# antonbaumann/MIMO-Unet

Hardware: AMD Instinct MI355X
Metric: train images/sec at 256x256, S=2, fbc=30 (higher is better)
Workload: dtype f32 (split into 16-bit hi/lo pairs on the MFMA; weight gradient: activation as one fp16 value); 1 GPU; cfg3: SEN12TP-shape synthetic 2->1 ch, 256x256, S=2, fbc=30, laplace_nll, batch 32 global; global_batch=32, per_gpu_batch=32, scaling=strong, labels=U[0,1) (SURVEY 8d); same batch every step, parallelism=dp1, world_size=1, weak_per_gpu_batch=32, strong_global_batch=32, optimizer=adam(lr=1e-3) fused, inputs=resident in HBM

## Files before the change

mimo_unet_amd/csrc/common.h:

```cpp
#pragma once
#include <hip/hip_runtime.h>
#include <stdint.h>

#include "../../include/mimo_hip.h"
#include "tile_sched.h"

namespace mimo {

void set_error(const char* fmt, ...);

#define MIMO_HIP_CHECK(expr)                                                                          \
  do {                                                                                                \
    hipError_t e_ = (expr);                                                                           \
    if (e_ != hipSuccess) {                                                                           \
      ::mimo::set_error("%s failed: %s (%s:%d)", #expr, hipGetErrorString(e_), __FILE__, __LINE__);   \
      return MIMO_ERR_HIP;                                                                            \
    }                                                                                                 \
  } while (0)
#define MIMO_KERNEL_CHECK() MIMO_HIP_CHECK(hipGetLastError())
#define MIMO_TRY(expr)            \
  do {                            \
    int rc_ = (expr);             \
    if (rc_ != MIMO_OK) return rc_; \
  } while (0)

static inline int ceil_div(int a, int b) { return (a + b - 1) / b; }
static inline int round_up(int a, int b) { return ceil_div(a, b) * b; }
static inline int64_t ceil_div64(int64_t a, int64_t b) { return (a + b - 1) / b; }

static inline int pad_channels(int c) { return round_up(c, 8); }

constexpr int kWave = 64;

enum StoreType { ST_F32 = 0, ST_BF16 = 1, ST_F16 = 2 };
static inline int store_bytes(int dt) { return dt == ST_F32 ? 4 : 2; }

__device__ __forceinline__ int xcd_virtual_index(int linear, int total) {
  return sched::xcd_virtual_index(linear, total);
}

__host__ __device__ __forceinline__ float w16_scale(unsigned wmax_bits, bool inverse) { return sched::w16_scale(wmax_bits, inverse); }

constexpr int kFinSlack = 32;
struct ConvLaunch {
  const float* x;
  float* y;
  const float* w;
  const void* wpk = nullptr;
  const float* bias;
  float* stats;
  int N, Hi, Wi, ldx, cin_p;
  int Ho, Wo, ldy, cout_pad, cout_store;
  int off;
  const float* ep_scale = nullptr;
  const float* ep_shift = nullptr;
  const float* ep_mask = nullptr;
  int ep_mask_ld = 0;
  int* status = nullptr;
  int pair = 0;
  int wide = 0;
  const float* in_scale = nullptr;
  const float* in_shift = nullptr;
  const unsigned* wmax = nullptr;
  int ksplit = 1;
};
int conv3x3_ksplit(int mode, int N, int cin_p, int cout_pad, int Ho, int Wo);
int conv3x3_bf16x3_launch_k(const ConvLaunch& a, int mode, int* rows, hipStream_t stream, float* kpart, size_t kpart_floats);
size_t conv3x3_ksplit_scratch(int mode, int N, int cin_p, int cout_pad, int Ho, int Wo, int ldy);
int conv3x3_split_fuses_input(int mode, int wide, int Ho, int Wo);
int conv3x3_launch(const ConvLaunch& a, int* rows, hipStream_t stream);
int conv3x3_thin_ok(int cin, int cout_p);
int conv3x3_thin_launch(const ConvLaunch& a, int cin, int* rows, hipStream_t stream);
size_t wgrad_thin_scratch(int cin, int cout_p);
int wgrad_thin_ok(int cin, int cout_p, int N, int H, int W);
int wgrad_thin_launch(const float* x, int ldx, const float* dz, int lddz, int N, int H, int W, int cin, int cout, int cout_p,
                      float* partial, float* dw, hipStream_t stream);
int conv3x3_bf16x3_launch(const ConvLaunch& a, int mode, int* rows, hipStream_t stream);
int pack_weights_bf16x3_launch(const float* w, void* dst, int f16, int cout, int cin, int rows_pad, int cols,
                               const int* row_map, const int* col_map, int transposed, hipStream_t stream, int pair = 0);
int conv3x3_pair_tail(int mode, int cin_p, int Ho, int Wo);
int conv3x3_wide_rows(int mode, int N, int cin_p, int rows, int Ho, int Wo);
size_t conv3x3_wide_weight_elems(int cin_p, int rows_pad);
int conv3x3_wide_stat_rows();
int conv3x3_wide_launch(const ConvLaunch& a, int mode, int* rows, hipStream_t stream);
int pack_weights_wide_launch(const float* w, void* dst, int f16, int cout, int cin, int rows_pad, int cols,
                             const int* row_map, const int* col_map, int nrows_map, int transposed, hipStream_t stream,
                             int single = 0);
int conv3x3_pick_nfrag(int cout);
int conv3x3_cout_pad(int cout);
int conv3x3_stat_rows(int N, int Ho, int Wo);
int conv3x3_ws_stat_rows(int N, int Ho, int Wo);

static __device__ __attribute__((aligned(256))) float kZeroPage[64];

struct WgradLaunch {
  const float* x;
  const float* dz;
  float* partial;
  int N, H, W, ldx, lddz;
  int cin_p, cout_p;
  int cin_pad, cout_pad;
  int splits;
  int np = 3;
  const float* dz_absmax = nullptr;
  int dz_absmax_n = 0;
  int store = 0;
  const float* in_scale = nullptr;
  const float* in_shift = nullptr;
};
constexpr int kDzMaxSlots = 2048 * 2;
__host__ __device__ __forceinline__ float wg_dz_scale(unsigned absmax_bits, bool inverse) { return sched::wg_dz_scale(absmax_bits, inverse); }
#if defined(__HIPCC__)
__device__ __forceinline__ float wg_dz_absmax(const float* __restrict__ slots, int n) {
  float m = 0.f;
  for (int i = (int)(threadIdx.x & 63); i < n; i += 64) m = fmaxf(m, slots[i]);
#pragma unroll
  for (int d = 1; d < 64; d <<= 1) m = fmaxf(m, __shfl_xor(m, d));
  return m;
}
#endif
int wgrad_launch(const WgradLaunch& a, hipStream_t stream);
int wgrad_split_has_np2(int cin_p, int cout_p);
int wgrad_split_fuses_input(int cin_p, int cout_p, int store, int np);
void wgrad_split_tiles(int cin_p, int cout_p, int* CI, int* CO);
int wgrad_split_pick_splits(int N, int H, int W, int cin_pad, int cout_pad, int CI, int CO, int store = 0, int cus = 256);
int wgrad_split_launch(const WgradLaunch& a, hipStream_t stream);
int wgrad_pick_splits(int N, int H, int W, int cin_pad, int cout_pad);
size_t wgrad_reduce_scratch(int splits, int cin_pad, int cout_pad);
int wgrad_reduce_launch(const float* partial, int splits, int cin_pad, int cout_pad, const int* cin_map,
                        int cin_p, int cin, int cout, float* dw, hipStream_t stream, const float* dz_absmax = nullptr,
                        int dz_absmax_n = 0, hipEvent_t done = nullptr);

struct PackJob {
  int64_t w_off, bias_off;
  void* dst;
  float* bias_dst;
  const int *row_map, *col_map;
  int kind, cout, cin, rows_pad, cols, transposed, total, bias_n;
  int pair;
  int map_rows;
  unsigned* wmax;
};
int pack_jobs_launch(const PackJob* jobs_dev, int njobs, int max_total, const float* params, hipStream_t stream);
int wabsmax_jobs_launch(const PackJob* jobs_dev, int njobs, int max_total, const float* params, hipStream_t stream,
                        int* status = nullptr);

int pack_weights_launch(const float* w, float* dst, int cout, int cin, int rows_pad, int cols,
                        const int* row_map, const int* col_map, int transposed, hipStream_t stream);

}
```

mimo_unet_amd/csrc/conv_bf16x3.hip:

```cpp
#include <cstdlib>
#include <type_traits>

#include "common.h"

namespace mimo {

template <bool F16>
struct Elem;
template <>
struct Elem<false> {
  typedef __bf16 T;
  typedef __attribute__((ext_vector_type(8))) __bf16 V8;
  typedef __attribute__((ext_vector_type(4))) __bf16 V4;
};
template <>
struct Elem<true> {
  typedef _Float16 T;
  typedef __attribute__((ext_vector_type(8))) _Float16 V8;
  typedef __attribute__((ext_vector_type(4))) _Float16 V4;
};
typedef float f32x4_ __attribute__((ext_vector_type(4)));
__device__ __forceinline__ f32x4_ mfma16(Elem<false>::V8 a, Elem<false>::V8 b, f32x4_ c) {
  return __builtin_amdgcn_mfma_f32_16x16x32_bf16(a, b, c, 0, 0, 0);
}
// ... 206 lines not shown
            }
            acc[m][nf] = mfma16(ah, bh[nf], acc[m][nf]);
          }
        }
      }
      if (!last) {
        MIMO_STORE_W((r + 1) % 3, buf ^ 1)
      }
      if (r == 2 && c + 1 < nchunks) {
        __syncthreads();
        MIMO_STORE_X()
      }
      __syncthreads();
      buf ^= 1;
    }
  }

  float bv[NF], s1[NF], s2[NF], esc[NF], esh[NF], emk[NF];
#pragma unroll
  for (int nf = 0; nf < NF; ++nf) {
    bv[nf] = a.bias ? a.bias[co0 + nf * 16 + lr] : 0.f;
    s1[nf] = 0.f;
    s2[nf] = 0.f;
    esc[nf] = a.ep_scale ? a.ep_scale[co0 + nf * 16 + lr] : 1.f;
    esh[nf] = a.ep_scale ? a.ep_shift[co0 + nf * 16 + lr] : 0.f;
    emk[nf] = (a.ep_mask && co0 + nf * 16 + lr < a.ep_mask_ld) ? a.ep_mask[(size_t)n * a.ep_mask_ld + co0 + nf * 16 + lr] : 1.f;
  }
  typedef typename std::conditional<OUT16, ET, float>::type OT;
  OT* yimg = reinterpret_cast<OT*>(a.y) + (size_t)n * a.Ho * a.Wo * a.ldy;
  const float winv = !F16 ? 1.f : a.wmax ? w16_scale(*a.wmax, true) : 1.f / kF16WeightScale;
#pragma unroll
  for (int m = 0; m < MF; ++m) {
#pragma unroll
    for (int r4 = 0; r4 < 4; ++r4) {
      const int idx = (wave * MF + m) * 16 + g * 4 + r4;
      const int orow = idx / TC, ocol = idx - orow * TC;
      const int oy = y0 + orow, ox = x0 + ocol;
      if (idx < npix_out && oy < a.Ho && ox < a.Wo) {
        OT* yp = yimg + ((size_t)oy * a.Wo + ox) * a.ldy + co0 + lr;
#pragma unroll
        for (int nf = 0; nf < NF; ++nf) {
          float v = acc[m][nf][r4] * winv + bv[nf];
          if (a.ep_scale) {
            if (a.status && !isfinite(v)) atomicOr(a.status, 1);
            v = fmaxf(fmaf(v, esc[nf], esh[nf]), 0.f) * emk[nf];
          }
          if (co0 + nf * 16 + lr < a.cout_store) yp[nf * 16] = (OT)v;
          s1[nf] += v;
          s2[nf] += v * v;
        }
      }
    }
  }
  if (a.stats) {
#pragma unroll
    for (int nf = 0; nf < NF; ++nf) {
      s1[nf] += __shfl_xor(s1[nf], 16);
      s1[nf] += __shfl_xor(s1[nf], 32);
      s2[nf] += __shfl_xor(s2[nf], 16);
      s2[nf] += __shfl_xor(s2[nf], 32);
    }
    float* red = reinterpret_cast<float*>(ws);
    if (g == 0) {
#pragma unroll
      for (int nf = 0; nf < NF; ++nf) {
        red[(wave * 2 + 0) * NB + nf * 16 + lr] = s1[nf];
        red[(wave * 2 + 1) * NB + nf * 16 + lr] = s2[nf];
      }
    }
    __syncthreads();
    if (tid < 2 * NB) {
      const int which = tid / NB, c = tid - which * NB;
      float v = 0.f;
#pragma unroll
      for (int w = 0; w < 8; ++w) v += red[(w * 2 + which) * NB + c];
      a.stats[((size_t)blockIdx.x * 2 + which) * a.cout_pad + co0 + c] = v;
    }
  }
}

#undef MIMO_LOAD_X
#undef MIMO_STORE_X
#undef MIMO_LOAD_W
#undef MIMO_STORE_W

template <int MF>
struct WsTile {
  static constexpr int NPIX = 64 * MF;
  static constexpr int MAXPIX = MF == 4 ? 360 : 180;
};
constexpr int kWsMaxMF = 4;

template <int NF, int MODE, int MF_, bool PAIR = false, bool FIN = false>
__global__ __launch_bounds__(512, (MF_ == 2 && NF <= 2) ? 4 : 2) void conv3x3_ws_kernel(ConvLaunch a, int TR, int TC,
                                                                                          int tilesY, int tilesX,
                                                                                          int numTiles, int xcd_order,
                                                                                          int gx, int coTiles) {
  MIMO_CONV_MODE_CONSTANTS
  static_assert(!PAIR || (NP == 3 && !IN16), "tap pairing: split16 modes");
  static_assert(!FIN || MODE == 1, "fused input BatchNorm + ReLU: the split16 forward");
  typedef typename Elem<F16>::T ET;
  typedef typename Elem<F16>::V8 bf16x8;
  typedef typename Elem<F16>::V4 bf16x4;
  typedef typename std::conditional<OUT16, ET, float>::type OT;
  constexpr int NB = NF * 16;
  constexpr int MF = MF_;
  constexpr int kWsMaxPix = WsTile<MF>::MAXPIX;
  constexpr int UPP = IN16 ? 4 : 8, UPPS = IN16 ? 2 : 3;
  constexpr int XU = (kWsMaxPix * UPP + 255) / 256;
  constexpr int XP = XU / 3;
  static_assert(XU % 3 == 0, "input tile staged in three equal parts");
  constexpr int WUNITS = 3 * NB * 8;
  constexpr int WU = (WUNITS + 255) / 256;
  constexpr int PITCH = kPitchB;
  constexpr int WPITCH = 128;
  constexpr int XBYTES = kWsMaxPix * PITCH, WROWB = 3 * NB * WPITCH;
  __shared__ __attribute__((aligned(128))) unsigned char xs[2 * XBYTES];
  __shared__ __attribute__((aligned(128))) unsigned char ws[2 * WROWB];

  const int tid = threadIdx.x;
  const int lane = tid & 63, wave = tid >> 6;
  const int TCP = TC + 2, TRP = TR + 2;
  const int npix_lds = TRP * TCP, npix_out = TR * TC;
  const int nchunks = (a.cin_p + 31) / 32;
  const int ksplit = a.ksplit > 1 ? a.ksplit : 1;
  const int v_ = xcd_order ? xcd_virtual_index((int)blockIdx.x, gx * coTiles * ksplit) : (int)blockIdx.x;
  const int vks_ = v_ / coTiles;
  const int vbx = vks_ / ksplit, ks = vks_ - vbx * ksplit;
  const int co0 = (v_ - vks_ * coTiles) * NB;
  const int cpk_ = (nchunks + ksplit - 1) / ksplit;
  const int ck0 = ks * cpk_, nck = min(cpk_, nchunks - ck0);
  const int ntiles_mine = vbx < numTiles ? (numTiles - 1 - vbx) / gx + 1 : 0;
  const int nstages = ntiles_mine * nck;

  if (wave >= 4) {
    const int ptid = tid - 256;
    f32x4 xreg[XU];
    const unsigned ws_lds = (unsigned)(size_t)(__attribute__((address_space(3))) unsigned char*)ws;
    int wsrc[WU];
#pragma unroll
    for (int k = 0; k < WU; ++k) {
      const int u = min(ptid + k * 256, WUNITS - 1), row = u >> 3;
      wsrc[k] = ((row / NB) * a.cout_pad + row % NB) * 8 + ((u & 7) ^ (row & 7));
    }
    int u_rc[XU], u_off[XU];
#pragma unroll
    for (int k = 0; k < XU; ++k) {
      const int p = min((ptid + k * 256) >> UPPS, npix_lds - 1);
      const int tr = p / TCP, tc = p - tr * TCP;
      u_rc[k] = (tr << 16) | tc;
      u_off[k] = ((tr * a.Wi + tc) * a.ldx + 4 * ((ptid + k * 256) & 7)) * 4;
    }
    const u32x4* wpk = reinterpret_cast<const u32x4*>(a.wpk);
    f32x4 in_sc = f32x4{0.f, 0.f, 0.f, 0.f}, in_sh = in_sc, in_sc_n = in_sc, in_sh_n = in_sc;
#define WS_LOAD_SS(SC, SH, STAGE)                                                                    \
  if (FIN) {                                                                                         \
    const int c_ = (ck0 + (STAGE) % nck) * 32 + 4 * (ptid & 7);                                      \
     \
    SC = *reinterpret_cast<const f32x4*>(a.in_scale + c_);                                           \
    SH = *reinterpret_cast<const f32x4*>(a.in_shift + c_);                                           \
  }
#define WS_LOAD_X(K0, K1, STAGE)                                                                     \
  {                                                                                                  \
    const int st_ = (STAGE);                                                                         \
    const int ti_ = st_ / nck, ck_ = ck0 + st_ - ti_ * nck;                                          \
    int t_ = vbx + ti_ * gx;                                                                         \
    const int tx_ = t_ % tilesX;                                                                     \
    t_ /= tilesX;                                                                                    \
    const int ty_ = t_ % tilesY;                                                                     \
    const int n_ = t_ / tilesY;                                                                      \
    const int y0_ = ty_ * TR - a.off, x0_ = tx_ * TC - a.off;                                        \
    const float* ximg_ = a.x + (size_t)n_ * a.Hi * a.Wi * a.ldx;                                     \
    const unsigned short* ximg16_ = reinterpret_cast<const unsigned short*>(a.x) + (size_t)n_ * a.Hi * a.Wi * a.ldx; \
                                                                         \
    if (!CVT && !IN16 && y0_ >= 0 && y0_ + TRP <= a.Hi && x0_ >= 0 && x0_ + TCP <= a.Wi && ck_ * 32 + 32 <= a.cin_p) { \
      const char* tb_ = reinterpret_cast<const char*>(ximg_ + ((size_t)y0_ * a.Wi + x0_) * a.ldx) + ck_ * 128; \
      _Pragma("unroll") for (int k_ = (K0); k_ < (K1); ++k_)                                         \
        xreg[k_] = *reinterpret_cast<const f32x4*>(tb_ + u_off[k_]);                                 \
    } else {                                                                                         \
    _Pragma("unroll") for (int k_ = (K0); k_ < (K1); ++k_) {                                         \
      int iy_ = y0_ + (u_rc[k_] >> 16), ix_ = x0_ + (u_rc[k_] & 0xffff);                             \
      bool in_ = true;                                                                               \
      if (a.off == 1) {                                                       \
        iy_ = max(iy_, -iy_);                                                                        \
        iy_ = max(min(iy_, 2 * a.Hi - 2 - iy_), 0);                                                  \
        ix_ = max(ix_, -ix_);                                                                        \
        ix_ = max(min(ix_, 2 * a.Wi - 2 - ix_), 0);                                                  \
      } else {                                            \
        in_ = iy_ >= 0 && iy_ < a.Hi && ix_ >= 0 && ix_ < a.Wi;                                      \
      }                                                                                              \
      const int q_ = (ptid + k_ * 256) & (UPP - 1);                                                  \
      const int o_ = in_ ? (iy_ * a.Wi + ix_) * a.ldx : 0;                                           \
      if (IN16) {                          \
        const int rc_ = min(32, a.cin_p - ck_ * 32);                                                 \
        const bool ok_ = in_ && 8 * q_ < rc_;                                                        \
        xreg[k_] = *reinterpret_cast<const f32x4*>(                                                  \
            ok_ ? reinterpret_cast<const float*>(ximg16_ + o_ + ck_ * 32 + 8 * q_) : kZeroPage);     \
      } else if (CVT) {                                                                              \
        const int ch_ = ck_ * 32 + 4 * q_;                                                           \
        const bool ok_ = in_ && ch_ < a.cin_p;                                                       \
        xreg[k_] = *reinterpret_cast<const f32x4*>(ok_ ? ximg_ + o_ + ch_ : kZeroPage);              \
      } else {                                                                                       \
        const int rc_ = min(32, a.cin_p - ck_ * 32);                                                 \
        const bool ok_ = in_ && 8 * (q_ & 3) < rc_;                                                  \
        const unsigned short* s_ = reinterpret_cast<const unsigned short*>(ximg_ + o_) +             \
                                   (ck_ * 64 + (q_ >> 2) * rc_ + 8 * (q_ & 3));                      \
        xreg[k_] = *reinterpret_cast<const f32x4*>(ok_ ? reinterpret_cast<const float*>(s_) : kZeroPage); \
      }                                                                                              \
    }                                                                                                \
    }                                                                                                \
  }
#define WS_STORE_X(K0, K1, BUF)                                                                      \
  _Pragma("unroll") for (int k_ = (K0); k_ < (K1); ++k_) {                                           \
    const int u_ = ptid + k_ * 256;                                                                  \
    const int p_ = u_ >> UPPS, q_ = u_ & (UPP - 1);                                                  \
    if (p_ < npix_lds) {                                                                             \
      f32x4 v_ = xreg[k_];                                                                           \
      if (FIN) {                                                                                     \
        v_[0] = fmaxf(fmaf(v_[0], in_sc[0], in_sh[0]), 0.f);                                         \
        v_[1] = fmaxf(fmaf(v_[1], in_sc[1], in_sh[1]), 0.f);                                         \
        v_[2] = fmaxf(fmaf(v_[2], in_sc[2], in_sh[2]), 0.f);                                         \
        v_[3] = fmaxf(fmaf(v_[3], in_sc[3], in_sh[3]), 0.f);                                         \
      }                                                                                              \
      unsigned char* row_ = xs + (BUF) * XBYTES + p_ * PITCH;                                        \
      const int sx_ = 0;                                                                             \
      if (CVT) {                                                                                     \
        bf16x4 hi_, lo_;                                                                             \
        hi_[0] = (ET)v_[0];                                                                          \
        hi_[1] = (ET)v_[1];                                                                          \
        hi_[2] = (ET)v_[2];                                                                          \
        hi_[3] = (ET)v_[3];                                                                          \
        lo_[0] = (ET)(v_[0] - (float)hi_[0]);                                                        \
        lo_[1] = (ET)(v_[1] - (float)hi_[1]);                                                        \
        lo_[2] = (ET)(v_[2] - (float)hi_[2]);                                                        \
        lo_[3] = (ET)(v_[3] - (float)hi_[3]);                                                        \
        *reinterpret_cast<bf16x4*>(row_ + (((q_ >> 1) ^ sx_) << 4) + (q_ & 1) * 8) = hi_;            \
        if (NP == 3) *reinterpret_cast<bf16x4*>(row_ + ((((q_ >> 1) + 4) ^ sx_) << 4) + (q_ & 1) * 8) = lo_; \
      } else {                                                                                       \
        *reinterpret_cast<f32x4*>(row_ + ((q_ ^ sx_) << 4)) = v_;                                    \
      }                                                                                              \
    }                                                                                                \
  }
#define WS_DMA_W(BUF, PH)                                                                            \
  {                                                                                                  \
    const int phw_ = (PH);                                                                           \
    const int ck_ = ck0 + (phw_ / 3) % nck, r_ = phw_ % 3;                                           \
    const u32x4* src_ = wpk + ((size_t)(ck_ * 9 + r_ * 3) * a.cout_pad + co0) * 8;                   \
    _Pragma("unroll") for (int k_ = 0; k_ < WU; ++k_) {                                              \
      if (ptid + k_ * 256 < WUNITS) {                      \
         \
        const unsigned dst_ = __builtin_amdgcn_readfirstlane(                                        \
            ws_lds + (unsigned)((BUF) * WROWB + (k_ * 256 + (ptid & ~63)) * 16));                    \
        unsigned keep_;                                                                              \
        asm volatile("s_mov_b32 %0, m0\n\ts_mov_b32 m0, %2\n\ts_nop 0\n\tglobal_load_lds_dwordx4 %1, off\n\ts_mov_b32 m0, %0" \
                     : "=&s"(keep_) : "v"(src_ + wsrc[k_]), "s"(dst_) : "memory");                   \
      }                                                                                              \
    }                                                                                                \
  }
#define WS_DMA_WAIT(N) asm volatile("s_waitcnt vmcnt(%0)\n\ts_waitcnt lgkmcnt(0)\n\ts_barrier" ::"n"(N) : "memory");
    const int nphases = 3 * nstages;
    WS_LOAD_SS(in_sc, in_sh, 0)
    WS_LOAD_X(0, XU, 0)
    WS_DMA_W(0, 0)
    WS_STORE_X(0, XU, 0)
    WS_LOAD_SS(in_sc_n, in_sh_n, min(1, nstages - 1))
    WS_LOAD_X(0, XU, min(1, nstages - 1))
    WS_DMA_WAIT(XU)
    for (int j = 0; j < nstages; ++j) {
      const int xb = (j + 1) & 1;
      if (FIN) {
        in_sc = in_sc_n;
        in_sh = in_sh_n;
      }
#define WS_PHASE(R)                                                                                  \
  {                                                                                                  \
          \
    const int ph_ = 3 * j + (R);                                                                     \
    if ((R) == 0) {                                                                                  \
      WS_LOAD_SS(in_sc_n, in_sh_n, min(j + 2, nstages - 1))  \
    }                                                                                                \
    WS_STORE_X((R) * XP, ((R) + 1) * XP, xb)                                                         \
    WS_DMA_W((ph_ + 1) & 1, min(ph_ + 1, nphases - 1))                                               \
    WS_LOAD_X((R) * XP, ((R) + 1) * XP, min(j + 2, nstages - 1))                                     \
    WS_DMA_WAIT(XP)                                                                                  \
  }
      WS_PHASE(0)
      WS_PHASE(1)
      WS_PHASE(2)
#undef WS_PHASE
    }
#undef WS_LOAD_SS
#undef WS_LOAD_X
#undef WS_STORE_X
#undef WS_DMA_W
#undef WS_DMA_WAIT
    if (FWD && a.stats) __syncthreads();
    return;
  }

  const int lr = lane & 15, g = lane >> 4;
  int pbase[kWsMaxMF];
#pragma unroll
  for (int m = 0; m < MF; ++m) {
    int idx = (wave * MF + m) * 16 + lr;
    if (idx >= npix_out) idx = 0;
    const int r = idx / TC, c = idx - r * TC;
    pbase[m] = (r * TCP + c) * PITCH + g * 16;
  }
  const int pair_d = g >= 2 ? TCP * PITCH - 32 : 0, pair_d2 = g >= 2 ? -32 : 0;
  const int wbase = lr * WPITCH + ((g ^ (lr & 7)) << 4);
  const int wlo = (wbase ^ 64) - wbase;
  f32x4 bv[NF];
#pragma unroll
  for (int nf = 0; nf < NF; ++nf)
    bv[nf] = (FWD && a.bias) ? *reinterpret_cast<const f32x4*>(a.bias + co0 + nf * 16 + g * 4) : f32x4{0.f, 0.f, 0.f, 0.f};
  const float winv = !F16 ? 1.f : a.wmax ? w16_scale(*a.wmax, true) : 1.f / kF16WeightScale;
  (void)winv;
  int prc[kWsMaxMF];
#pragma unroll
  for (int m = 0; m < MF; ++m) {
    const int idx = (wave * MF + m) * 16 + lr;
    const int r = idx / TC, c = idx - r * TC;
    prc[m] = idx < npix_out ? (r << 16) | c : (0x4000 << 16);
  }
  const int nphases = 3 * nstages;
  f32x4 s1[NF], s2[NF];
#pragma unroll
  for (int nf = 0; nf < NF; ++nf) {
    s1[nf] = f32x4{0.f, 0.f, 0.f, 0.f};
    s2[nf] = f32x4{0.f, 0.f, 0.f, 0.f};
  }

  f32x4 acc[kWsMaxMF][NF];
#pragma unroll
  for (int m = 0; m < MF; ++m)
#pragma unroll
    for (int nf = 0; nf < NF; ++nf) acc[m][nf] = f32x4{0.f, 0.f, 0.f, 0.f};
  constexpr bool PINNED = !CVT;
  constexpr int RA = NP == 3 ? 2 : 1, RB = NF * RA;
  bf16x8 ah[2], al[2], bh[2][NF], bl[2][NF];

#define C_READ_B(BS, KW)                                                                             \
// ... 38 lines not shown
    }                                                                                                \
    if (!(LAST)) {                                                                                   \
      C_READ_A(0, (KW) + 1, 0)                                                                       \
      C_MFMA(1, BS, MF - 1)                                                                          \
      C_PIN(RA)                                                                                      \
    }                                                                                                \
  }
#define C_EPILOGUE(TI)                                                                               \
  {                                                                                                  \
    int t_ = vbx + (TI) * gx;                                                                        \
    const int tx_ = t_ % tilesX;                                                                     \
    t_ /= tilesX;                                                                                    \
    const int ty_ = t_ % tilesY;                                                                     \
    const int n_ = t_ / tilesY;                                                                      \
    const int y0_ = ty_ * TR, x0_ = tx_ * TC;                                                        \
    OT* yimg = reinterpret_cast<OT*>(a.y) + ((size_t)ks * a.N + n_) * a.Ho * a.Wo * a.ldy + co0 + g * 4; \
    _Pragma("unroll") for (int m = 0; m < MF; ++m) {                                                 \
      const int oy = y0_ + (prc[m] >> 16), ox = x0_ + (prc[m] & 0xffff);                             \
      if (oy < a.Ho && ox < a.Wo) {                                                                  \
        OT* yp = yimg + ((size_t)oy * a.Wo + ox) * a.ldy;                                            \
        _Pragma("unroll") for (int nf = 0; nf < NF; ++nf) {                                          \
                                                   \
          f32x4 v = acc[m][nf];                                                                      \
          if (F16) v = v * winv;                                                                     \
          if (FWD) v = v + bv[nf];                                                                   \
          const int c_ = co0 + nf * 16 + g * 4;                                                      \
          if (FWD && a.ep_scale) {                                                                   \
            if (a.status && !(isfinite(v[0]) && isfinite(v[1]) && isfinite(v[2]) && isfinite(v[3]))) atomicOr(a.status, 1); \
            const f32x4 esc_ = *reinterpret_cast<const f32x4*>(a.ep_scale + c_);                     \
            const f32x4 esh_ = *reinterpret_cast<const f32x4*>(a.ep_shift + c_);                     \
            _Pragma("unroll") for (int i_ = 0; i_ < 4; ++i_) {                                       \
              const float mk_ = (a.ep_mask && c_ + i_ < a.ep_mask_ld)                                \
                                    ? a.ep_mask[(size_t)n_ * a.ep_mask_ld + c_ + i_] : 1.f;          \
              v[i_] = fmaxf(fmaf(v[i_], esc_[i_], esh_[i_]), 0.f) * mk_;                             \
            }                                                                                        \
          }                                                                                          \
          if (c_ < a.cout_store) {                                                                   \
            if (OUT16) {                                                                             \
              bf16x4 o_;                                                                             \
              o_[0] = (ET)v[0];                                                                      \
              o_[1] = (ET)v[1];                                                                      \
              o_[2] = (ET)v[2];                                                                      \
              o_[3] = (ET)v[3];                                                                      \
              *reinterpret_cast<bf16x4*>(yp + nf * 16) = o_;                                         \
            } else {                                                                                 \
              *reinterpret_cast<f32x4*>(yp + nf * 16) = v;                                           \
            }                                                                                        \
          }                                                                                          \
          if (FWD) {                                                                                 \
            s1[nf] += v;                                                                             \
            s2[nf] += v * v;                                                                         \
          }                                                                                          \
        }                                                                                            \
      }                                                                                              \
    }                                                                                                \
    _Pragma("unroll") for (int m = 0; m < MF; ++m)                                                   \
      _Pragma("unroll") for (int nf = 0; nf < NF; ++nf) acc[m][nf] = f32x4{0.f, 0.f, 0.f, 0.f};      \
  }
#define C_PHASE(P, FIRST)                                                                            \
  {                                                                                                  \
    const int j_ = ph / 3, r_ = ph - 3 * j_;                                                         \
    const unsigned char* xb_ = xs + (j_ & 1) * XBYTES;                                               \
    const unsigned char* wb_ = ws + (ph & 1) * WROWB + wbase;                                        \
    const bool pc_ = PAIR && (j_ + 1) % nchunks == 0;        \
    const int ro_ = pc_ ? 2 * r_ : r_;                                                               \
    const int pd_ = pc_ ? (r_ == 0 ? pair_d : pair_d2) : 0;                                          \
    __syncthreads();         \
    C_READ_B((P) ^ 1, 0)                                                                             \
    C_READ_A(0, 0, 0)                                                                                \
    if (!(FIRST)) {                                                                                  \
      C_MFMA(1, P, MF - 1)                                                                           \
      C_PIN(RA + RB)                                                                                 \
      if (tile_done) {                                                                               \
        C_EPILOGUE(ti)                                                                               \
        ++ti;                                                                                        \
      }                                                                                              \
    }                                                                                                \
    C_TAP(0, (P) ^ 1, false)                                                                         \
    C_TAP(1, P, false)                                                                               \
    C_TAP(2, (P) ^ 1, true)                                                                          \
    tile_done = r_ == (PAIR ? 1 : 2) && (j_ + 1) % nck == 0;                                         \
    ++ph;                                                                                            \
    if (PAIR) {                              \
      if (ph < nphases && ph % 3 == 2 && (ph / 3 + 1) % nchunks == 0) {                              \
        __syncthreads();                                                                             \
        ++ph;                                                                                        \
      }                                                                                              \
    }                                                                                                \
  }

  int ph = 0, ti = 0;
  bool tile_done = false;
  C_PHASE(1, true)
  while (ph + (PAIR ? 2 : 1) < nphases) {
    C_PHASE(0, false)
    C_PHASE(1, false)
  }
  if (ph < nphases) {
    C_PHASE(0, false)
    C_MFMA(1, 1, MF - 1)
  } else {
    C_MFMA(1, 0, MF - 1)
  }
  C_EPILOGUE(ti)
  __syncthreads();
  if (FWD && a.stats) {
    float* red = reinterpret_cast<float*>(xs);
#pragma unroll
    for (int nf = 0; nf < NF; ++nf) {
#pragma unroll
      for (int i = 0; i < 4; ++i) {
#pragma unroll
        for (int d = 1; d < 16; d <<= 1) {
          s1[nf][i] += __shfl_xor(s1[nf][i], d);
          s2[nf][i] += __shfl_xor(s2[nf][i], d);
        }
      }
      if (lr == 0) {
        *reinterpret_cast<f32x4*>(red + (wave * 2 + 0) * NB + nf * 16 + g * 4) = s1[nf];
        *reinterpret_cast<f32x4*>(red + (wave * 2 + 1) * NB + nf * 16 + g * 4) = s2[nf];
      }
    }
    __syncthreads();
    if (tid < 2 * NB) {
      const int which = tid / NB, c = tid - which * NB;
      const float v = (red[(0 * 2 + which) * NB + c] + red[(1 * 2 + which) * NB + c]) +
                      (red[(2 * 2 + which) * NB + c] + red[(3 * 2 + which) * NB + c]);
      a.stats[((size_t)vbx * 2 + which) * a.cout_pad + co0 + c] = v;
    }
  }
#undef C_READ_A
#undef C_READ_B
#undef C_TAP
#undef C_MFMA
#undef C_PIN
#undef C_EPILOGUE
#undef C_PHASE
}

static bool conv_ws_enabled() {
  static const bool on = !(getenv("MIMO_CONV_WS") && atoi(getenv("MIMO_CONV_WS")) == 0);
  return on;
}

int conv3x3_ws_stat_rows(int, int, int) { return 512 * 4; }

int conv3x3_pair_tail(int mode, int cin_p, int Ho, int Wo) {
  if (mode < 0 || mode > 1 || !conv_ws_enabled() || Ho * Wo < 256) return 0;
  const int tail = cin_p - 32 * (ceil_div(cin_p, 32) - 1);
  return tail <= 16 ? 1 : 0;
}

template <int NF, int MODE, int MF>
static int launch_ws(const ConvLaunch& a, int* rows, hipStream_t stream) {
  int TR, TC;
  pick_tile_n(a.Ho, a.Wo, WsTile<MF>::NPIX, WsTile<MF>::MAXPIX, &TR, &TC);
  const int tilesY = ceil_div(a.Ho, TR), tilesX = ceil_div(a.Wo, TC);
  const int numTiles = a.N * tilesY * tilesX;
  const int coTiles = a.cout_pad / (NF * 16);
  constexpr int kWgPerCU = (MF == 2 && NF <= 2) ? 2 : 1;
  const int ksplit = a.ksplit > 1 ? a.ksplit : 1;
  if (ksplit > 1) {
    const int nchunks = ceil_div(a.cin_p, 32), cpk = ceil_div(nchunks, ksplit);
    if (MODE > 1 || a.pair || a.bias || a.stats || a.ep_scale || a.cin_p % 32 != 0 || cpk * (ksplit - 1) >= nchunks) {
      set_error("conv3x3 split: K split %d needs a split16 launch without bias / stats / epilogue, whole 32-channel chunks "
                "and at least one chunk per split (cin_p %d)", ksplit, a.cin_p);
      return MIMO_ERR_INVALID;
    }
  }
  int gx = max(1, 256 * kWgPerCU / (coTiles * ksplit));
  if (gx > numTiles) gx = numTiles;
  const int per = ceil_div(numTiles, gx);
  gx = ceil_div(numTiles, per);
  if (rows) *rows = gx;
  dim3 grid(gx * coTiles * ksplit);
  const int xcd = 1;
  if (a.in_scale) {
    if constexpr (MODE == 1) {
      if (a.ep_scale || !a.in_shift || (a.pair && a.pair != conv3x3_pair_tail(MODE, a.cin_p, a.Ho, a.Wo))) {
        set_error("conv3x3 split: the input BatchNorm + ReLU can be fused into the split16 training forward only");
        return MIMO_ERR_INVALID;
      }
      if (a.pair)
        hipLaunchKernelGGL((conv3x3_ws_kernel<NF, MODE, MF, true, true>), grid, dim3(512), 0, stream, a, TR, TC, tilesY, tilesX, numTiles, xcd, gx, coTiles);
      else
        hipLaunchKernelGGL((conv3x3_ws_kernel<NF, MODE, MF, false, true>), grid, dim3(512), 0, stream, a, TR, TC, tilesY, tilesX, numTiles, xcd, gx, coTiles);
      MIMO_KERNEL_CHECK();
      return MIMO_OK;
    } else {
      set_error("conv3x3 split: the input BatchNorm + ReLU can be fused into the split16 forward only");
      return MIMO_ERR_INVALID;
    }
  }
  if (a.pair) {
    if constexpr (MODE <= 1) {
      if (a.pair != conv3x3_pair_tail(MODE, a.cin_p, a.Ho, a.Wo)) {
        set_error("conv3x3 split: weights packed for tap pairing, launch is not");
        return MIMO_ERR_INVALID;
      }
      hipLaunchKernelGGL((conv3x3_ws_kernel<NF, MODE, MF, true>), grid, dim3(512), 0, stream, a, TR, TC, tilesY, tilesX, numTiles, xcd, gx, coTiles);
    } else {
      set_error("conv3x3 split: tap pairing exists for the split16 modes only");
      return MIMO_ERR_INVALID;
    }
  } else
    hipLaunchKernelGGL((conv3x3_ws_kernel<NF, MODE, MF>), grid, dim3(512), 0, stream, a, TR, TC, tilesY, tilesX, numTiles, xcd, gx, coTiles);
  MIMO_KERNEL_CHECK();
  return MIMO_OK;
}

template <int MF, int NF, int MODE>
static int launch_bf16x3(const ConvLaunch& a, int* rows, hipStream_t stream) {
  int TR, TC;
  pick_tile_n(a.Ho, a.Wo, TileCfg<MF>::NPIX, TileCfg<MF>::MAXPIX, &TR, &TC);
  const int tilesY = ceil_div(a.Ho, TR), tilesX = ceil_div(a.Wo, TC);
  if (rows) *rows = a.N * tilesY * tilesX;
  dim3 grid(a.N * tilesY * tilesX, a.cout_pad / (NF * 16));
  hipLaunchKernelGGL((conv3x3_bf16x3_kernel<MF, NF, MODE>), grid, dim3(512), 0, stream, a, TR, TC, tilesY, tilesX);
  MIMO_KERNEL_CHECK();
  return MIMO_OK;
}

static bool use_big_tile(int Ho, int Wo) { return Ho * Wo >= 1024; }

int conv3x3_split_fuses_input(int mode, int wide, int Ho, int Wo) {
  return mode == 1 && (wide != 0 || (conv_ws_enabled() && Ho * Wo >= 256)) ? 1 : 0;
}

template <int MODE>
static int conv3x3_split_dispatch(const ConvLaunch& a, int* rows, hipStream_t stream) {
  if (a.in_scale && !conv3x3_split_fuses_input(MODE, 0, a.Ho, a.Wo)) {
    set_error("conv3x3 split: this launch cannot apply the input BatchNorm + ReLU in its loader (conv3x3_split_fuses_input)");
    return MIMO_ERR_INVALID;
  }
  const int nfr = a.cout_pad / 16;
  int nf = 4;
  while (nfr % nf != 0) --nf;
  if (conv_ws_enabled() && a.Ho * a.Wo >= 256) {
    if (a.ksplit <= 1) {
      int TR, TC;
      pick_tile_n(a.Ho, a.Wo, WsTile<4>::NPIX, WsTile<4>::MAXPIX, &TR, &TC);
      const int numTiles = a.N * ceil_div(a.Ho, TR) * ceil_div(a.Wo, TC);
      long best = -1;
      for (int c = 4; c >= 1; --c) {
        if (nfr % c) continue;
        const int gx = max(1, min(numTiles, 256 / (nfr / c)));
        const long cost = (long)ceil_div(numTiles, gx) * (1 + c);
        if (best < 0 || cost < best) best = cost, nf = c;
      }
    }
    const bool mf2 = (MODE == 1 || MODE == 2 || MODE == 4 || MODE == 6);
    switch (nf) {
      case 4: return launch_ws<4, MODE, 4>(a, rows, stream);
      case 3: return launch_ws<3, MODE, 4>(a, rows, stream);
      case 2: return mf2 ? launch_ws<2, MODE, 2>(a, rows, stream) : launch_ws<2, MODE, 4>(a, rows, stream);
      default: return mf2 ? launch_ws<1, MODE, 2>(a, rows, stream) : launch_ws<1, MODE, 4>(a, rows, stream);
    }
  }
  if (a.pair) {
    set_error("conv3x3 split: weights packed for tap pairing, launch is not");
    return MIMO_ERR_INVALID;
  }
  if (use_big_tile(a.Ho, a.Wo) && nf >= 3) {
    switch (nf) {
      case 4: return launch_bf16x3<4, 4, MODE>(a, rows, stream);
      case 3: return launch_bf16x3<4, 3, MODE>(a, rows, stream);
      case 2: return launch_bf16x3<4, 2, MODE>(a, rows, stream);
      default: return launch_bf16x3<4, 1, MODE>(a, rows, stream);
    }
  }
  switch (nf) {
    case 4: return launch_bf16x3<2, 4, MODE>(a, rows, stream);
    case 3: return launch_bf16x3<2, 3, MODE>(a, rows, stream);
    case 2: return launch_bf16x3<2, 2, MODE>(a, rows, stream);
    default: return launch_bf16x3<2, 1, MODE>(a, rows, stream);
  }
}

constexpr int kKsplitReduceUnits = 14;
int conv3x3_ksplit(int mode, int N, int cin_p, int cout_pad, int Ho, int Wo) {
  static const int force = [] { const char* e = getenv("MIMO_CONV_KSPLIT"); return e ? atoi(e) : -1; }();
  if (force == 0 || (mode != 0 && mode != 1) || !conv_ws_enabled() || Ho * Wo < 256 || cin_p % 32 != 0 ||
      cout_pad % 16 != 0)
    return 1;
  const int nchunks = cin_p / 32;
  if (nchunks < 2) return 1;
  auto legal = [&](int ks) { return ks >= 2 && ceil_div(nchunks, ks) * (ks - 1) < nchunks; };
  if (force >= 2) {
    int ks = min(force, nchunks);
    while (ks >= 2 && !legal(ks)) --ks;
    return ks >= 2 ? ks : 1;
  }
  int TR, TC;
  pick_tile_n(Ho, Wo, WsTile<4>::NPIX, WsTile<4>::MAXPIX, &TR, &TC);
  const int numTiles = N * ceil_div(Ho, TR) * ceil_div(Wo, TC);
  const int nfr = cout_pad / 16;
  long unsplit = -1;
  for (int c = 4; c >= 1; --c) {
    if (nfr % c) continue;
    const int gx = max(1, min(numTiles, 256 / (nfr / c)));
    const long cost = (long)ceil_div(numTiles, gx) * (1 + c) * nchunks * 3;
    if (unsplit < 0 || cost < unsplit) unsplit = cost;
  }
  int nf = 4;
  while (nfr % nf != 0) --nf;
  const int coTiles = nfr / nf;
  int best = 1;
  long best_cost = -1;
  for (int ks = 2; ks <= 8 && ks <= nchunks; ++ks) {
    if (!legal(ks) || coTiles * ks > 256) continue;
    const int gx = max(1, min(numTiles, 256 / (coTiles * ks)));
    const long cost = (long)ceil_div(numTiles, gx) * (1 + nf) * ceil_div(nchunks, ks) * 3 + kKsplitReduceUnits;
    if (best_cost < 0 || cost < best_cost) best_cost = cost, best = ks;
  }
  return (best_cost >= 0 && best_cost * 100 < unsplit * 85) ? best : 1;
}

size_t conv3x3_ksplit_scratch(int mode, int N, int cin_p, int cout_pad, int Ho, int Wo, int ldy) {
  const int ks = conv3x3_ksplit(mode, N, cin_p, cout_pad, Ho, Wo);
  return ks > 1 ? (size_t)ks * N * Ho * Wo * ldy : 0;
}

__global__ __launch_bounds__(256) void conv_ksplit_reduce_kernel(const float* __restrict__ part, int ksplit, int P, int ld, int Cv,
                                                                 const float* __restrict__ bias, float* __restrict__ out,
                                                                 int ldo, float* __restrict__ stats, int cout_pad) {
  __shared__ f32x4 red[2][256];
  const int QB = Cv < 256 ? Cv : 256, PPI = 256 / QB;
  const int ql = threadIdx.x % QB, pl = threadIdx.x / QB;
  const int q = blockIdx.y * QB + ql;
  const bool active = pl < PPI && q < Cv;
  f32x4 s1 = f32x4{0.f, 0.f, 0.f, 0.f}, s2 = s1;
  if (active) {
    const f32x4 b = bias ? *reinterpret_cast<const f32x4*>(bias + 4 * q) : f32x4{0.f, 0.f, 0.f, 0.f};
    const size_t slab = (size_t)P * ld;
    for (int p = blockIdx.x * PPI + pl; p < P; p += gridDim.x * PPI) {
      const float* src = part + (size_t)p * ld + 4 * q;
      f32x4 v = *reinterpret_cast<const f32x4*>(src);
      for (int k = 1; k < ksplit; ++k) v += *reinterpret_cast<const f32x4*>(src + k * slab);
      v += b;
      *reinterpret_cast<f32x4*>(out + (size_t)p * ldo + 4 * q) = v;
      s1 += v;
      s2 += v * v;
    }
  }
  if (!stats) return;
  red[0][threadIdx.x] = s1;
  red[1][threadIdx.x] = s2;
  __syncthreads();
  if (pl == 0 && q < Cv) {
    for (int i = 1; i < PPI; ++i) {
      s1 += red[0][i * QB + ql];
      s2 += red[1][i * QB + ql];
    }
    float* row = stats + (size_t)blockIdx.x * 2 * cout_pad;
    *reinterpret_cast<f32x4*>(row + 4 * q) = s1;
    *reinterpret_cast<f32x4*>(row + cout_pad + 4 * q) = s2;
  }
}

int conv3x3_bf16x3_launch_k(const ConvLaunch& a, int mode, int* rows, hipStream_t stream, float* kpart, size_t kpart_floats) {
  const int ks = (a.wide || a.ep_scale || !kpart) ? 1 : conv3x3_ksplit(mode, a.N, a.cin_p, a.cout_pad, a.Ho, a.Wo);
  const size_t need = (size_t)ks * a.N * a.Ho * a.Wo * a.ldy;
  if (ks <= 1 || a.pair || need > kpart_floats || a.cout_store % 4 != 0 || a.ldy % 4 != 0 || (size_t)a.N * a.Ho * a.Wo > (1u << 30))
    return conv3x3_bf16x3_launch(a, mode, rows, stream);
  ConvLaunch p = a;
  p.y = kpart;
  p.bias = nullptr;
  p.stats = nullptr;
  p.ksplit = ks;
  MIMO_TRY(conv3x3_bf16x3_launch(p, mode, nullptr, stream));
  const int P = a.N * a.Ho * a.Wo, Cv = a.cout_store / 4;
  const int QB = Cv < 256 ? Cv : 256, PPI = 256 / QB;
  const int gx = max(1, min(ceil_div(P, PPI * 2), 256));
  if (rows) *rows = gx;
  hipLaunchKernelGGL(conv_ksplit_reduce_kernel, dim3(gx, ceil_div(Cv, QB)), dim3(256), 0, stream, kpart, ks, P, a.ldy, Cv, a.bias,
                     a.y, a.ldy, a.stats, a.cout_pad);
  MIMO_KERNEL_CHECK();
  return MIMO_OK;
}

int conv3x3_bf16x3_launch(const ConvLaunch& a, int mode, int* rows, hipStream_t stream) {
  if (a.wide) return conv3x3_wide_launch(a, mode, rows, stream);
  if (!a.wpk || a.ldx % 4 != 0 || a.cout_pad % 16 != 0 || a.Hi < 2 || a.Wi < 2 || mode < 0 || mode > 7 ||
      (mode >= 4 && (a.ldx % 8 != 0 || a.cin_p % 8 != 0 || a.ldy % 4 != 0))) {
    set_error("conv3x3 split: bad geometry or mode");
    return MIMO_ERR_INVALID;
  }
  switch (mode) {
    case 0: return conv3x3_split_dispatch<0>(a, rows, stream);
    case 1: return conv3x3_split_dispatch<1>(a, rows, stream);
    case 2: return conv3x3_split_dispatch<2>(a, rows, stream);
    case 3: return conv3x3_split_dispatch<3>(a, rows, stream);
    case 4: return conv3x3_split_dispatch<4>(a, rows, stream);
    case 5: return conv3x3_split_dispatch<5>(a, rows, stream);
    case 6: return conv3x3_split_dispatch<6>(a, rows, stream);
    default: return conv3x3_split_dispatch<7>(a, rows, stream);
  }
}

__device__ __forceinline__ void pair_slot(int tap, int k, int* slot, int* kk) {
  const int row = tap / 3, kw = tap - 3 * row;
  *slot = row == 2 ? 3 + kw : kw;
  *kk = k + (row == 1 ? 16 : 0);
}

template <bool F16>
__global__ void pack_weights_bf16x3_kernel(const float* __restrict__ w, typename Elem<F16>::T* __restrict__ dst, int cout,
                                           int cin, int rows_pad, int cols, int nchunks, const int* __restrict__ row_map,
                                           const int* __restrict__ col_map, int transposed, int pair) {
  typedef typename Elem<F16>::T ET;
  const int total = nchunks * 9 * rows_pad * 32;
  for (int i = blockIdx.x * blockDim.x + threadIdx.x; i < total; i += gridDim.x * blockDim.x) {
    const int k = i & 31;
    int rest = i >> 5;
    const int row = rest % rows_pad;
    rest /= rows_pad;
    const int tap = rest % 9, chunk = rest / 9;
    const int col = chunk * 32 + k;
    float v = 0.f;
    if (col < cols) {
      const int rm = row_map[row], cm = col_map[col];
      if (rm >= 0 && cm >= 0) {
        const int co = transposed ? cm : rm, ci = transposed ? rm : cm;
        const int kh = transposed ? 2 - tap / 3 : tap / 3, kw = transposed ? 2 - tap % 3 : tap % 3;
        v = w[(((size_t)co * cin + ci) * 3 + kh) * 3 + kw];
      }
    }
    if (F16) v *= kF16WeightScale;
    const ET hi = (ET)v;
    const ET lo = (ET)(v - (float)hi);
    int slot = tap, kk = k;
    if (pair && chunk == nchunks - 1) {
      if (k >= 16) continue;
      pair_slot(tap, k, &slot, &kk);
    }
    ET* d = dst + (((size_t)chunk * 9 + slot) * rows_pad + row) * 64;
    d[kk] = hi;
    d[32 + kk] = lo;
  }
}

__global__ void pack_jobs_kernel(const PackJob* __restrict__ jobs, const float* __restrict__ params) {
  const PackJob j = jobs[blockIdx.y];
  const float* w = params + j.w_off;
  const float wscale = j.wmax ? w16_scale(*j.wmax, false) : kF16WeightScale;
  if (blockIdx.x == 0 && j.bias_n > 0)
    for (int i = threadIdx.x; i < j.bias_n; i += blockDim.x) j.bias_dst[i] = params[j.bias_off + i];
  const int per_tap = j.total / 9;
  for (int i = blockIdx.x * blockDim.x + threadIdx.x; i < per_tap; i += gridDim.x * blockDim.x) {
    int row, col, k = 0, chunk = 0;
    if (j.kind == 0) {
      col = i % j.cols;
      row = i / j.cols;
    } else if (j.kind >= 5) {
      k = i & 31;
      const int rest = i >> 5;
      row = rest % j.rows_pad;
      chunk = rest / j.rows_pad;
      col = chunk * 32 + k;
    } else if (j.kind >= 3) {
      k = i & 15;
      const int rest = i >> 4;
      row = rest % j.rows_pad;
      chunk = rest / j.rows_pad;
      col = chunk * 16 + k;
    } else {
      k = i & 31;
      const int rest = i >> 5;
      row = rest % j.rows_pad;
      chunk = rest / j.rows_pad;
      col = chunk * 32 + k;
    }
    float v[9];
#pragma unroll
    for (int t = 0; t < 9; ++t) v[t] = 0.f;
    if (col < j.cols && (j.kind < 3 || row < j.map_rows)) {
      const int rm = j.row_map[row], cm = j.col_map[col];
      if (rm >= 0 && cm >= 0) {
        const int co = j.transposed ? cm : rm, ci = j.transposed ? rm : cm;
        const float* src = w + ((size_t)co * j.cin + ci) * 9;
#pragma unroll
        for (int t = 0; t < 9; ++t) v[t] = src[j.transposed ? 8 - t : t];
      }
    }
    const bool paired = (j.kind == 1 || j.kind == 2) && j.pair && chunk == (j.cols + 31) / 32 - 1;
    if (paired && k >= 16) continue;
#pragma unroll
    for (int tap = 0; tap < 9; ++tap) {
      const float x = v[tap];
      int slot = tap, kk = k;
      if (paired) pair_slot(tap, k, &slot, &kk);
      if (j.kind == 0) {
        reinterpret_cast<float*>(j.dst)[((size_t)tap * j.rows_pad + row) * j.cols + col] = x;
      } else if (j.kind == 5) {
        reinterpret_cast<_Float16*>(j.dst)[(((size_t)chunk * 9 + tap) * j.rows_pad + row) * 32 + k] = (_Float16)(x * wscale);
      } else if (j.kind == 6) {
        reinterpret_cast<__bf16*>(j.dst)[(((size_t)chunk * 9 + tap) * j.rows_pad + row) * 32 + k] = (__bf16)x;
      } else if (j.kind == 3) {
        const float xs = x * wscale;
        const _Float16 hi = (_Float16)xs, lo = (_Float16)(xs - (float)hi);
        _Float16* d = reinterpret_cast<_Float16*>(j.dst) + (((size_t)chunk * 9 + tap) * j.rows_pad + row) * 32;
        d[k] = hi;
        d[16 + k] = lo;
      } else if (j.kind == 4) {
        const __bf16 hi = (__bf16)x, lo = (__bf16)(x - (float)hi);
        __bf16* d = reinterpret_cast<__bf16*>(j.dst) + (((size_t)chunk * 9 + tap) * j.rows_pad + row) * 32;
        d[k] = hi;
        d[16 + k] = lo;
      } else if (j.kind == 1) {
        const float xs = x * wscale;
        const _Float16 hi = (_Float16)xs, lo = (_Float16)(xs - (float)hi);
        _Float16* d = reinterpret_cast<_Float16*>(j.dst) + (((size_t)chunk * 9 + slot) * j.rows_pad + row) * 64;
        d[kk] = hi;
        d[32 + kk] = lo;
// ... 66 lines not shown
```

mimo_unet_amd/csrc/conv_wide.hip:

```cpp
#include <cstdlib>
#include <type_traits>

#include "common.h"
#include "tile_sched.h"

namespace mimo {

namespace {

typedef float f32x4 __attribute__((ext_vector_type(4)));
typedef float f32x2 __attribute__((ext_vector_type(2)));
typedef float f32x16 __attribute__((ext_vector_type(16)));
typedef unsigned int u32x4 __attribute__((ext_vector_type(4)));
typedef __attribute__((ext_vector_type(8))) __bf16 bf16x8_t;
typedef __attribute__((ext_vector_type(8))) _Float16 f16x8_t;
typedef __attribute__((ext_vector_type(4))) _Float16 f16x4_t;

__device__ __forceinline__ f32x16 mfma32(bf16x8_t a, bf16x8_t b, f32x16 c) {
  return __builtin_amdgcn_mfma_f32_32x32x16_bf16(a, b, c, 0, 0, 0);
}
__device__ __forceinline__ f32x16 mfma32(f16x8_t a, f16x8_t b, f32x16 c) {
  return __builtin_amdgcn_mfma_f32_32x32x16_f16(a, b, c, 0, 0, 0);
}
__device__ __forceinline__ float dpp_xor1(float x) {
  return __builtin_bit_cast(float, __builtin_amdgcn_update_dpp(0, __builtin_bit_cast(int, x), 0xB1, 0xF, 0xF, true));
}

constexpr float kWideF16Scale = 256.f;

constexpr int kXPitch = 80;
constexpr int kMaxPix = sched::kWideMaxPix;
constexpr int kXBytes = kMaxPix * kXPitch;

}

template <int NF, int MODE, int TPP, bool EPI, bool FIN = false>
__global__ __launch_bounds__(512, 2) void conv3x3_wide_kernel(ConvLaunch a, int TR, int TC, int tilesY, int tilesX,
                                                                int numTiles, int gx, int coTiles) {
  static_assert(MODE == 0 || MODE == 1 || (MODE >= 4 && MODE <= 7), "split16 and 16-bit storage modes");
  static_assert(!FIN || (MODE == 1 && !EPI), "fused input BatchNorm + ReLU: the split16 forward with statistics");
  static_assert((NF == 2 && TPP == 3) || (NF == 1 && TPP == 9), "instances: 64 channels x tap rows, 32 channels x chunks");
  constexpr bool FWD = MODE == 1 || MODE == 4 || MODE == 6;
  constexpr bool S16 = MODE >= 4;
  constexpr bool F16 = MODE == 1 || MODE >= 6;
  constexpr bool CVT = MODE == 1;
  constexpr int CKC = S16 ? 32 : 16;
  constexpr bool STATS = FWD && !EPI;
  static_assert(FWD || !EPI, "the inference epilogue belongs to the forward");
  typedef typename std::conditional<F16, f16x8_t, bf16x8_t>::type V8;
  typedef typename std::conditional<F16, _Float16, __bf16>::type ET;
  constexpr int NB = NF * 32;
  constexpr int MF = 4;
  constexpr int SM = NF == 1 ? 2 : 1;
  constexpr int NSLOT = MF / SM;
  constexpr int PARTS = 9 / TPP;
  constexpr int XU = 10;
#define XK0(R) (PARTS == 1 ? ((R) <= 0 ? 0 : XU) : ((R) <= 0 ? 0 : (R) == 1 ? 4 : (R) == 2 ? 8 : XU))
#define XKN(R) (XK0((R) + 1) - XK0(R))
  constexpr int WUNITS = TPP * NB * 4;
  constexpr int WU = (WUNITS + 255) / 256;
  constexpr int WPHB = WU * 256 * 16;
  constexpr int NWB = TPP == 3 ? 3 : 2;
  constexpr int EPIB = FWD ? 3 * NB * 4 : 0;
  constexpr bool DEFER = NF == 1 && MODE == 0 && !EPI;
  constexpr int SUMB = (DEFER && FWD) ? 4 * 2 * 256 * 8 : 0;
  static_assert(2 * kXBytes + NWB * WPHB + EPIB + SUMB <= 160 * 1024, "LDS budget");
  __shared__ __attribute__((aligned(1024))) unsigned char lds[2 * kXBytes + NWB * WPHB + EPIB + SUMB];
  unsigned char* const xs = lds;
  unsigned char* const ws = lds + 2 * kXBytes;
  float* const epi = reinterpret_cast<float*>(lds + 2 * kXBytes + NWB * WPHB);

  const int tid = threadIdx.x;
  const int lane = tid & 63, wave = tid >> 6;
  const int TCP = TC + 2, TRP = TR + 2;
  const int npix_lds = TRP * TCP, npix_out = TR * TC;
  const int nchunks = (a.cin_p + CKC - 1) / CKC;
  const int v_ = xcd_virtual_index((int)blockIdx.x, gx * coTiles);
  const int vbx = v_ / coTiles;
  const int co0 = (v_ - vbx * coTiles) * NB;
  const int ntiles_mine = vbx < numTiles ? (numTiles - 1 - vbx) / gx + 1 : 0;
  const int nstages = ntiles_mine * nchunks;
  const int nphases = PARTS * nstages;
  const int rows_pad = coTiles * NB;

  if (FWD) {
    if (tid < NB) {
      const int c = co0 + tid;
      epi[tid] = c < a.cout_pad ? a.bias[c] : 0.f;
      if (EPI) {
        epi[NB + tid] = c < a.cout_store ? a.ep_scale[c] : 0.f;
        epi[2 * NB + tid] = c < a.cout_store ? a.ep_shift[c] : 0.f;
      }
    }
    __syncthreads();
  }

  if (wave >= 4) {
    const int ptid = tid - 256;
    f32x4 xreg[XU];
    const unsigned ws_lds = (unsigned)(size_t)(__attribute__((address_space(3))) unsigned char*)ws;
    int wsrc[WU];
#pragma unroll
    for (int k = 0; k < WU; ++k) {
      const int u = min(ptid + k * 256, WUNITS - 1), row = u >> 2;
      const int tp = row / NB, ch = row - tp * NB;
      wsrc[k] = ((tp * rows_pad + ch) * 4 + ((u & 3) ^ ((ch >> 2) & 3))) * 16;
    }
    const unsigned wdst0 = __builtin_amdgcn_readfirstlane(ws_lds + (unsigned)((ptid & ~63) * 16));
    int u_rc[XU];
    int u_off[XU];
    unsigned u_val = 0;
#pragma unroll
    for (int k = 0; k < XU; ++k) {
      const int p = min((ptid + k * 256) >> 2, npix_lds - 1);
      const int tr = p / TCP, tc = p - tr * TCP;
      u_rc[k] = (tr << 16) | tc;
      u_off[k] = 0;
    }
    const int uq = ptid & 3;
    const int uq_off = (CVT || S16) ? 16 * uq : (uq >> 1) * 64 + (uq & 1) * 16;
    const int esz = S16 ? 2 : 4;
    const char* const wpk = reinterpret_cast<const char*>(a.wpk) + (size_t)co0 * 64;
    const int wph_bytes = TPP * rows_pad * 64;
    int l_stage = 0, l_ck = 0, l_ti = 0;
    const char* l_img = nullptr;
    int l_y0 = 0, l_x0 = 0;
    bool l_new = true;
    f32x4 in_sc = f32x4{0.f, 0.f, 0.f, 0.f}, in_sh = in_sc, in_sc_n = in_sc, in_sh_n = in_sc;
#define WD_LOAD_SS(SC, SH, CK)                                                                       \
  if (FIN) {                                                                                         \
    const int c_ = (CK) * CKC + 4 * uq;                                                              \
     \
    SC = *reinterpret_cast<const f32x4*>(a.in_scale + c_);                                           \
    SH = *reinterpret_cast<const f32x4*>(a.in_shift + c_);                                           \
  }
#define WD_TILE(TI)                                                                                  \
  {                                                                                                  \
    int t_ = vbx + (TI) * gx;                                                                        \
    const int tx_ = t_ % tilesX;                                                                     \
    t_ /= tilesX;                                                                                    \
    const int ty_ = t_ % tilesY;                                                                     \
    const int n_ = t_ / tilesY;                                                                      \
    l_y0 = ty_ * TR - a.off;                                                                         \
    l_x0 = tx_ * TC - a.off;                                                                         \
    l_img = reinterpret_cast<const char*>(a.x) + (size_t)n_ * a.Hi * a.Wi * a.ldx * esz;             \
  }
#define WD_OFFS(K0, K1)                                                                              \
  _Pragma("unroll") for (int k_ = (K0); k_ < (K1); ++k_) {                                           \
    int iy_ = l_y0 + (u_rc[k_] >> 16), ix_ = l_x0 + (u_rc[k_] & 0xffff);                             \
    if (FWD) {                                                                  \
      iy_ = max(iy_, -iy_);                                                                          \
      iy_ = max(min(iy_, 2 * a.Hi - 2 - iy_), 0);                                                    \
      ix_ = max(ix_, -ix_);                                                                          \
      ix_ = max(min(ix_, 2 * a.Wi - 2 - ix_), 0);                                                    \
    } else {                                    \
      const bool in_ = iy_ >= 0 && iy_ < a.Hi && ix_ >= 0 && ix_ < a.Wi;                             \
      u_val = in_ ? u_val | (1u << k_) : u_val & ~(1u << k_);                                        \
      iy_ = in_ ? iy_ : 0;                                                                           \
      ix_ = in_ ? ix_ : 0;                                                                           \
    }                                                                                                \
    u_off[k_] = (iy_ * a.Wi + ix_) * a.ldx * esz + uq_off;                                           \
  }
#define WD_LOAD_X(K0, K1)                                                                            \
  {                                                                                                  \
    if (l_new) {                                                                                     \
      WD_OFFS(K0, K1)                                                                                \
    }                                                                                                \
    const int rc_ = min(32, a.cin_p - (l_ck >> 1) * 32);  \
                                  \
    const bool full_ = (CVT || S16) ? l_ck * CKC + CKC <= a.cin_p : rc_ == 32;                       \
    const char* b_ = l_img + ((CVT || S16) ? l_ck * 64 : (l_ck >> 1) * 128 + (l_ck & 1) * 32);       \
    if (full_) {                                                                                     \
      _Pragma("unroll") for (int k_ = (K0); k_ < (K1); ++k_) {                                       \
        if (FWD)                                                                                     \
          xreg[k_] = *reinterpret_cast<const f32x4*>(b_ + u_off[k_]);                                \
        else                                                                                         \
          xreg[k_] = *reinterpret_cast<const f32x4*>(                                                \
              (u_val >> k_) & 1 ? b_ + u_off[k_] : reinterpret_cast<const char*>(kZeroPage));        \
      }                                                                                              \
    } else {                                                                                         \
      _Pragma("unroll") for (int k_ = (K0); k_ < (K1); ++k_) {                                       \
        if (CVT || S16) {                                                                            \
          const bool ok_ = (FWD || ((u_val >> k_) & 1)) && l_ck * CKC + (CKC / 4) * uq < a.cin_p;    \
          xreg[k_] = *reinterpret_cast<const f32x4*>(ok_ ? b_ + u_off[k_] : reinterpret_cast<const char*>(kZeroPage)); \
        } else {  \
          const int e_ = (l_ck & 1) * 16 + (uq & 1) * 8;                                             \
          const bool ok_ = ((u_val >> k_) & 1) && e_ < rc_;                                          \
          xreg[k_] = *reinterpret_cast<const f32x4*>(                                                \
              ok_ ? b_ + u_off[k_] + (uq >> 1) * (rc_ - 32) * 2 : reinterpret_cast<const char*>(kZeroPage)); \
        }                                                                                            \
      }                                                                                              \
    }                                                                                                \
  }
#define WD_NEXT_STAGE()                                                                              \
  {                                                                                                  \
    l_new = false;                                                                                   \
    if (l_stage + 1 < nstages) {                                                                     \
      ++l_stage;                                                                                     \
      if (++l_ck == nchunks) {                                                                       \
        l_ck = 0;                                                                                    \
        ++l_ti;                                                                                      \
        l_new = true;                                                                                \
        WD_TILE(l_ti)                                                                                \
      }                                                                                              \
    }                                                                                                \
  }
#define WD_STORE_X(K0, K1, BUF)                                                                      \
  _Pragma("unroll") for (int k_ = (K0); k_ < (K1); ++k_) {                                           \
    const int p_ = (ptid + k_ * 256) >> 2;                                                           \
                                  \
    {                                                                                                \
      f32x4 v_ = xreg[k_];                                                                           \
      if (FIN) {                                                                                     \
        v_[0] = fmaxf(fmaf(v_[0], in_sc[0], in_sh[0]), 0.f);                                         \
        v_[1] = fmaxf(fmaf(v_[1], in_sc[1], in_sh[1]), 0.f);                                         \
        v_[2] = fmaxf(fmaf(v_[2], in_sc[2], in_sh[2]), 0.f);                                         \
        v_[3] = fmaxf(fmaf(v_[3], in_sc[3], in_sh[3]), 0.f);                                         \
      }                                                                                              \
      unsigned char* row_ = xs + (BUF) * kXBytes + p_ * kXPitch;                                     \
      if (CVT) {                                                                                     \
        f16x4_t hi_, lo_;                                                                            \
        hi_[0] = (_Float16)v_[0];                                                                    \
        hi_[1] = (_Float16)v_[1];                                                                    \
        hi_[2] = (_Float16)v_[2];                                                                    \
        hi_[3] = (_Float16)v_[3];                                                                    \
        lo_[0] = (_Float16)(v_[0] - (float)hi_[0]);                                                  \
        lo_[1] = (_Float16)(v_[1] - (float)hi_[1]);                                                  \
        lo_[2] = (_Float16)(v_[2] - (float)hi_[2]);                                                  \
        lo_[3] = (_Float16)(v_[3] - (float)hi_[3]);                                                  \
        *reinterpret_cast<f16x4_t*>(row_ + uq * 8) = hi_;                                            \
        *reinterpret_cast<f16x4_t*>(row_ + 32 + uq * 8) = lo_;                                       \
      } else {                                                                                       \
        *reinterpret_cast<f32x4*>(row_ + uq * 16) = v_;                                              \
      }                                                                                              \
    }                                                                                                \
  }
    int w_ph = 0, w_pht = 0;
    const char* w_src = wpk;
    const int pht_n = PARTS * nchunks;
#define WD_DMA_W(BUF)                                                                                \
  {                                                                                                  \
    _Pragma("unroll") for (int k_ = 0; k_ < WU; ++k_) {                                              \
      const unsigned dst_ = wdst0 + (unsigned)((BUF) * WPHB + k_ * 4096);                            \
      unsigned keep_;                                                                                \
      asm volatile("s_mov_b32 %0, m0\n\ts_mov_b32 m0, %2\n\ts_nop 0\n\tglobal_load_lds_dwordx4 %1, off\n\ts_mov_b32 m0, %0" \
                   : "=&s"(keep_) : "v"(w_src + wsrc[k_]), "s"(dst_) : "memory");                    \
    }                                                                                                \
    if (w_ph + 1 < nphases) {  \
      ++w_ph;                                                                                        \
      w_src += wph_bytes;                                                                            \
      if (++w_pht == pht_n) {                                                                        \
        w_pht = 0;                                                                                   \
        w_src = wpk;                                                                                 \
      }                                                                                              \
    }                                                                                                \
  }
#define WD_WAIT_BAR(N) asm volatile("s_waitcnt vmcnt(%0)\n\ts_waitcnt lgkmcnt(0)\n\ts_barrier" ::"n"(N) : "memory");

    WD_TILE(0)
    WD_LOAD_SS(in_sc, in_sh, 0)
    WD_LOAD_X(0, XU)
    WD_DMA_W(0)
    if (NWB == 3) {
      WD_DMA_W(1)
    }
    WD_STORE_X(0, XU, 0)
    WD_NEXT_STAGE()
    WD_LOAD_SS(in_sc_n, in_sh_n, l_ck)
    WD_LOAD_X(0, XU)
    _Pragma("unroll") for (int k_ = 0; k_ < XU; ++k_) asm volatile("" ::"v"(xreg[k_]));
    WD_WAIT_BAR(0)
    int wslot = NWB == 3 ? 2 : 1;
    for (int j = 0; j < nstages; ++j) {
      const int xb = (j + 1) & 1;
      if (FIN) {
        in_sc = in_sc_n;
        in_sh = in_sh_n;
      }
      WD_NEXT_STAGE()
#define WD_PHASE(R)                                                                                  \
  {                                                                                                  \
    if ((R) == 0) {                                                                                  \
      WD_LOAD_SS(in_sc_n, in_sh_n, l_ck)           \
    }                                                                                                \
    WD_STORE_X(XK0(R), XK0((R) + 1), xb)                                                             \
    WD_DMA_W(wslot)                                                                                  \
    wslot = wslot + 1 == NWB ? 0 : wslot + 1;                                                        \
    WD_LOAD_X(XK0(R), XK0((R) + 1))                                                                  \
                                \
    WD_WAIT_BAR(NWB == 3 ? XKN(((R) + 2) % 3) + WU + XKN(R) + ((FIN && (R) == 0) ? 2 : 0) : XKN(R))  \
  }
      WD_PHASE(0)
      if (PARTS == 3) {
        WD_PHASE(1)
        WD_PHASE(2)
      }
#undef WD_PHASE
    }
#undef WD_LOAD_SS
#undef WD_TILE
#undef WD_OFFS
#undef WD_NEXT_STAGE
#undef WD_LOAD_X
#undef WD_STORE_X
#undef WD_DMA_W
#undef WD_WAIT_BAR
#undef XK0
#undef XKN
    asm volatile("s_waitcnt vmcnt(0)" ::: "memory");
// ... 199 lines not shown
    __builtin_amdgcn_sched_group_barrier(0x002, 5, 0);                                               \
  }                                                                                                  \
  __builtin_amdgcn_sched_group_barrier(0x040, 1, 0);
#define WC_BODY(P, FIRST, PIECES)                                                                    \
  _Pragma("unroll") for (int t = 0; t < TPP; ++t)                                                    \
    _Pragma("unroll") for (int s = 0; s < NSLOT; ++s) {                                              \
      const int g_ = t * NSLOT + s;                                                                  \
      const int ws_ = (t & 1) ? (P) : ((P) ^ 1);                                                     \
      if (!(t == TPP - 1 && s == NSLOT - 1)) {                                                       \
        if (s + 1 < NSLOT) {                                                                         \
          WC_READ_A((g_ + 1) & 1, t, s + 1)                                                          \
        } else {                                                                                     \
          WC_READ_W(ws_ ^ 1, t + 1)                                                                  \
          WC_READ_A((g_ + 1) & 1, t + 1, 0)                                                          \
        }                                                                                            \
        WC_MFMA_Z(g_ & 1, ws_, s, (PIECES) && t == 0)                                                \
        const bool piece_ = (PIECES) && g_ < 4 * MF;                                                 \
        if (piece_) {                                                                                \
          WC_PIECE(g_)                                                                               \
        }                                                                                            \
                                  \
        if (piece_) {                                                  \
          if (s + 1 < NSLOT) {                                                                       \
            WC_PIN_P(2 * SM + (FWD ? 1 : 0))                                                         \
          } else {                                                                                   \
            WC_PIN_P(2 * NF + 2 * SM + (FWD ? 1 : 0))                                                \
          }                                                                                          \
        } else if ((FIRST) && g_ == 0) {  \
          WC_PIN(2 * NF + 2 * SM + 2 * SM)                                                           \
        } else if (s + 1 < NSLOT) {                                                                  \
          WC_PIN(2 * SM)                                                                             \
        } else {                                                                                     \
          WC_PIN(2 * NF + 2 * SM)                                                                    \
        }                                                                                            \
      }                                                                                              \
    }
#define WC_PHASE(P, FIRST)                                                                           \
  {                                                                                                  \
    const int j_ = ph / PARTS, r_ = ph - PARTS * j_;                                                 \
    const unsigned char* xb_ = xs + (j_ & 1) * kXBytes;                                              \
    const unsigned char* wb_ = ws + wslot * WPHB;                                                    \
    const int ro_ = r_ * row1;                                                                       \
    (void)ro_;                                                                                       \
    __syncthreads();         \
    WC_READ_W((P) ^ 1, 0)                                                                            \
    WC_READ_A(0, 0, 0)                                                                               \
    bool pieces_ = false;                                                                            \
    if (!(FIRST)) {                                                                                  \
      WC_MFMA(1, P, NSLOT - 1)                                                                       \
      WC_PIN(2 * NF + 2 * SM)                                                                        \
      if (tile_done) {                                                                               \
        if (DEFER) {                                                                                 \
          WC_SNAPSHOT(ti)                                                                            \
          pieces_ = true;                                                                            \
        } else {                                                                                     \
          WC_EPILOGUE(ti)                                                                            \
        }                                                                                            \
        ++ti;                                                                                        \
      }                                                                                              \
    }                                                                                                \
    if (DEFER && pieces_) {                                                                          \
      WC_BODY(P, FIRST, true)                                                                        \
    } else {                                                                                         \
      WC_BODY(P, FIRST, false)                                                                       \
    }                                                                                                \
    tile_done = r_ == PARTS - 1 && (j_ + 1) % nchunks == 0;                                          \
    ++ph;                                                                                            \
    wslot = wslot + 1 == NWB ? 0 : wslot + 1;                                                        \
  }
#define WC_FINAL_EPILOGUE(TI)                                                                        \
  if (DEFER) {                                                                                       \
    WC_SNAPSHOT(TI)                                                                                  \
    _Pragma("unroll") for (int k_ = 0; k_ < 4 * MF; ++k_) {                                          \
      WC_PIECE(k_)                                                                                   \
    }                                                                                                \
  } else {                                                                                           \
    WC_EPILOGUE(TI)                                                                                  \
  }

  int ph = 0, ti = 0, wslot = 0;
  bool tile_done = false;
  if (nphases > 0) {
    WC_PHASE(1, true)
    while (ph + 1 < nphases) {
      WC_PHASE(0, false)
      WC_PHASE(1, false)
    }
    if (ph < nphases) {
      WC_PHASE(0, false)
      WC_MFMA(1, 1, NSLOT - 1)
    } else {
      WC_MFMA(1, 0, NSLOT - 1)
    }
    WC_FINAL_EPILOGUE(ti)
  }
  if (SUMB) {
#pragma unroll
    for (int j = 0; j < 4; ++j) {
      s1[0][j] = lsum[(2 * j) * 256];
      s2[0][j] = lsum[(2 * j + 1) * 256];
    }
  }
  __syncthreads();
  if (STATS) {
    float* red = reinterpret_cast<float*>(xs);
#pragma unroll
    for (int nf = 0; nf < NF; ++nf)
#pragma unroll
      for (int j = 0; j < 4; ++j) {
#pragma unroll
        for (int i = 0; i < 2; ++i)
#pragma unroll
          for (int d = 2; d < 32; d <<= 1) {
            s1[nf][j][i] += __shfl_xor(s1[nf][j][i], d);
            s2[nf][j][i] += __shfl_xor(s2[nf][j][i], d);
          }
        if (px < 2) {
          const int c = nf * 32 + 8 * j + 4 * h + 2 * px;
          *reinterpret_cast<f32x2*>(red + (wave * 2 + 0) * NB + c) = s1[nf][j];
          *reinterpret_cast<f32x2*>(red + (wave * 2 + 1) * NB + c) = s2[nf][j];
        }
      }
    __syncthreads();
    if (tid < 2 * NB) {
      const int which = tid / NB, c = tid - which * NB;
      const float v = (red[(0 * 2 + which) * NB + c] + red[(1 * 2 + which) * NB + c]) +
                      (red[(2 * 2 + which) * NB + c] + red[(3 * 2 + which) * NB + c]);
      if (a.stats && co0 + c < a.cout_pad) a.stats[((size_t)vbx * 2 + which) * a.cout_pad + co0 + c] = v;
    }
  }
#undef WC_READ_W
#undef WC_READ_A
#undef WC_MFMA
#undef WC_EPILOGUE
#undef WC_FINAL_EPILOGUE
#undef WC_SNAPSHOT
#undef WC_PIECE
#undef WC_PIN_P
#undef WC_BODY
#undef WC_MFMA_Z
#undef WC_PIN
#undef WC_PHASE
}

static int wide_force() {
  static const int f = [] {
    const char* e = getenv("MIMO_CONV_WIDE");
    const int v = e ? atoi(e) : 1;
    return v == 0 ? -1 : v >= 2 ? 1 : 0;
  }();
  return f;
}

int conv3x3_wide_rows(int mode, int N, int cin_p, int rows, int Ho, int Wo) {
  return sched::wide_config(mode, N, cin_p, rows, Ho, Wo, wide_force()).rows_pad;
}
size_t conv3x3_wide_weight_elems(int cin_p, int rows_pad) { return (size_t)ceil_div(cin_p, 16) * 9 * rows_pad * 32; }
int conv3x3_wide_stat_rows() { return 256; }

int conv3x3_wide_launch(const ConvLaunch& a, int mode, int* rows, hipStream_t stream) {
  const sched::WideCfg c = sched::wide_config(mode, a.N, a.cin_p, a.cout_store, a.Ho, a.Wo, 1);
  if (!a.wpk || c.nf == 0 || c.rows_pad != a.wide || a.ldx % 4 != 0 || a.ldy % 4 != 0 || a.Hi < 2 || a.Wi < 2) {
    set_error("conv3x3 wide: weights packed for %d rows, launch geometry gives %d (nf %d)", a.wide, c.rows_pad, c.nf);
    return MIMO_ERR_INVALID;
  }
  if (mode == 0 && a.cout_store % 8 != 0) {
    set_error("conv3x3 wide data gradient: %d stored channels (a multiple of 8 is needed)", a.cout_store);
    return MIMO_ERR_INVALID;
  }
  if ((int64_t)a.Ho * a.Wo * a.ldy * 4 >= (int64_t)0x7fff0000) {
    set_error("conv3x3 wide: output image of %d x %d x %d exceeds the kernel's 32-bit offsets", a.Ho, a.Wo, a.ldy);
    return MIMO_ERR_INVALID;
  }
  if ((int64_t)a.Hi * a.Wi * a.ldx * 4 > (int64_t)INT32_MAX) {
    set_error("conv3x3 wide: input image of %d x %d x %d exceeds the kernel's 32-bit offsets", a.Hi, a.Wi, a.ldx);
    return MIMO_ERR_INVALID;
  }
  const int tilesY = ceil_div(a.Ho, c.TR), tilesX = ceil_div(a.Wo, c.TC);
  const int numTiles = a.N * tilesY * tilesX;
  const int coTiles = c.rows_pad / (c.nf * 32);
  const int gx = sched::wide_grid_x(numTiles, coTiles);
  if (rows) *rows = gx;
  dim3 grid(gx * coTiles);
#define WIDE_LAUNCH(NF_, MODE_, TPP_, EPI_)                                                                        \
  hipLaunchKernelGGL((conv3x3_wide_kernel<NF_, MODE_, TPP_, EPI_>), grid, dim3(512), 0, stream, a, c.TR, c.TC, tilesY, \
                     tilesX, numTiles, gx, coTiles)
  const bool fwd = mode == 1 || mode == 4 || mode == 6;
  if (fwd && (!a.bias || (a.ep_scale && (a.stats || !a.ep_shift)))) {
    set_error("conv3x3 wide forward: needs the bias; statistics rows and the inference epilogue exclude each other");
    return MIMO_ERR_INVALID;
  }
  if (mode >= 4 && (a.ldx % 8 != 0 || a.cin_p % 8 != 0)) {
    set_error("conv3x3 wide, 16-bit storage: channel counts must be multiples of 8");
    return MIMO_ERR_INVALID;
  }
  if (a.in_scale && (mode != 1 || a.ep_scale || !a.in_shift)) {
    set_error("conv3x3 wide: the input BatchNorm + ReLU can be fused into the split16 training forward only");
    return MIMO_ERR_INVALID;
  }
  if (a.in_scale) {
    if (c.nf == 2)
      hipLaunchKernelGGL((conv3x3_wide_kernel<2, 1, 3, false, true>), grid, dim3(512), 0, stream, a, c.TR, c.TC, tilesY, tilesX,
                         numTiles, gx, coTiles);
    else
      hipLaunchKernelGGL((conv3x3_wide_kernel<1, 1, 9, false, true>), grid, dim3(512), 0, stream, a, c.TR, c.TC, tilesY, tilesX,
                         numTiles, gx, coTiles);
    MIMO_KERNEL_CHECK();
    return MIMO_OK;
  }
#define WIDE_FWD(MODE_)            \
  if (a.ep_scale) {                \
    if (c.nf == 2)                 \
      WIDE_LAUNCH(2, MODE_, 3, true);  \
    else                           \
      WIDE_LAUNCH(1, MODE_, 9, true);  \
  } else {                         \
    if (c.nf == 2)                 \
      WIDE_LAUNCH(2, MODE_, 3, false); \
    else                           \
      WIDE_LAUNCH(1, MODE_, 9, false); \
  }
#define WIDE_DG(MODE_)             \
  if (c.nf == 2)                   \
    WIDE_LAUNCH(2, MODE_, 3, false);   \
  else                             \
    WIDE_LAUNCH(1, MODE_, 9, false);
  switch (mode) {
    case 1: WIDE_FWD(1) break;
    case 4: WIDE_FWD(4) break;
    case 6: WIDE_FWD(6) break;
    case 0: WIDE_DG(0) break;
    case 5: WIDE_DG(5) break;
    default: WIDE_DG(7) break;
  }
#undef WIDE_FWD
#undef WIDE_DG
#undef WIDE_LAUNCH
  MIMO_KERNEL_CHECK();
  return MIMO_OK;
}

template <bool F16, bool SINGLE>
__global__ void pack_weights_wide_kernel(const float* __restrict__ w, void* __restrict__ dstv, int cout, int cin,
                                         int rows_pad, int cols, int nchunks, const int* __restrict__ row_map,
                                         const int* __restrict__ col_map, int nrows_map, int transposed) {
  typedef typename std::conditional<F16, _Float16, __bf16>::type ET;
  constexpr int CK = SINGLE ? 32 : 16;
  ET* dst = reinterpret_cast<ET*>(dstv);
  const int total = nchunks * 9 * rows_pad * CK;
  for (int i = blockIdx.x * blockDim.x + threadIdx.x; i < total; i += gridDim.x * blockDim.x) {
    const int k = i % CK;
    int rest = i / CK;
    const int row = rest % rows_pad;
    rest /= rows_pad;
    const int tap = rest % 9, chunk = rest / 9;
    const int col = chunk * CK + k;
    float v = 0.f;
    if (col < cols && row < nrows_map) {
      const int rm = row_map[row], cm = col_map[col];
      if (rm >= 0 && cm >= 0) {
        const int co = transposed ? cm : rm, ci = transposed ? rm : cm;
        const int kh = transposed ? 2 - tap / 3 : tap / 3, kw = transposed ? 2 - tap % 3 : tap % 3;
        v = w[(((size_t)co * cin + ci) * 3 + kh) * 3 + kw];
      }
    }
    if (F16) v *= kWideF16Scale;
    const ET hi = (ET)v;
    ET* d = dst + (((size_t)chunk * 9 + tap) * rows_pad + row) * 32;
    d[k] = hi;
    if (!SINGLE) d[16 + k] = (ET)(v - (float)hi);
  }
}

int pack_weights_wide_launch(const float* w, void* dst, int f16, int cout, int cin, int rows_pad, int cols,
                             const int* row_map, const int* col_map, int nrows_map, int transposed, hipStream_t stream,
                             int single) {
  const int nchunks = ceil_div(cols, single ? 32 : 16);
  const int total = nchunks * 9 * rows_pad * (single ? 32 : 16);
  const int blocks = min(ceil_div(total, 256), 4096);
#define PW_LAUNCH(F_, S_)                                                                                              \
  hipLaunchKernelGGL((pack_weights_wide_kernel<F_, S_>), dim3(blocks), dim3(256), 0, stream, w, dst, cout, cin, rows_pad, \
                     cols, nchunks, row_map, col_map, nrows_map, transposed)
  if (f16) {
    if (single)
      PW_LAUNCH(true, true);
    else
      PW_LAUNCH(true, false);
  } else {
    if (single)
      PW_LAUNCH(false, true);
    else
      PW_LAUNCH(false, false);
  }
#undef PW_LAUNCH
  MIMO_KERNEL_CHECK();
  return MIMO_OK;
}

}
```

mimo_unet_amd/csrc/ops_api.hip:

```cpp
#include <algorithm>
#include <vector>

#include "elementwise.h"

using namespace mimo;

namespace {

struct Temp {
  std::vector<void*> ptrs;
  ~Temp() {
    for (void* p : ptrs) (void)hipFree(p);
  }
  template <typename T>
  T* get(size_t count) {
    void* q = nullptr;
    if (hipMalloc(&q, std::max<size_t>(count, 1) * sizeof(T)) != hipSuccess) return nullptr;
    (void)hipMemset(q, 0, std::max<size_t>(count, 1) * sizeof(T));
    ptrs.push_back(q);
    return static_cast<T*>(q);
  }
  int* ints(const std::vector<int>& v) {
    int* p = get<int>(v.size());
    if (p) (void)hipMemcpy(p, v.data(), v.size() * sizeof(int), hipMemcpyHostToDevice);
// ... 19 lines not shown
    __syncthreads();
  }
  if (threadIdx.x == 0 && c < C) out[c] = (float)red[0];
}

__global__ void sums_to_stats_kernel(const double* __restrict__ sums, int chunks, int cout_pad, int cout,
                                     double* __restrict__ stats) {
  const int c = blockIdx.x * blockDim.x + threadIdx.x;
  if (c >= cout) return;
  double s1 = 0.0, s2 = 0.0;
  for (int k = 0; k < chunks; ++k) {
    s1 += sums[(size_t)k * 2 * cout_pad + c];
    s2 += sums[(size_t)k * 2 * cout_pad + cout_pad + c];
  }
  stats[c] = s1;
  stats[cout + c] = s2;
}

template <typename T>
__global__ void to16_kernel(const float* __restrict__ s, T* __restrict__ d, int64_t n) {
  for (int64_t i = (int64_t)blockIdx.x * blockDim.x + threadIdx.x; i < n; i += (int64_t)gridDim.x * blockDim.x) d[i] = (T)s[i];
}
template <typename T>
__global__ void from16_kernel(const T* __restrict__ s, float* __restrict__ d, int64_t n) {
  for (int64_t i = (int64_t)blockIdx.x * blockDim.x + threadIdx.x; i < n; i += (int64_t)gridDim.x * blockDim.x) d[i] = (float)s[i];
}
int to16(const float* s, void* d, int64_t n, bool f16, hipStream_t st) {
  const int blocks = (int)std::min<int64_t>((n + 255) / 256, 4096);
  if (f16)
    hipLaunchKernelGGL(to16_kernel<_Float16>, dim3(blocks), dim3(256), 0, st, s, (_Float16*)d, n);
  else
    hipLaunchKernelGGL(to16_kernel<__bf16>, dim3(blocks), dim3(256), 0, st, s, (__bf16*)d, n);
  MIMO_KERNEL_CHECK();
  return MIMO_OK;
}
int from16(const void* s, float* d, int64_t n, bool f16, hipStream_t st) {
  const int blocks = (int)std::min<int64_t>((n + 255) / 256, 4096);
  if (f16)
    hipLaunchKernelGGL(from16_kernel<_Float16>, dim3(blocks), dim3(256), 0, st, (const _Float16*)s, d, n);
  else
    hipLaunchKernelGGL(from16_kernel<__bf16>, dim3(blocks), dim3(256), 0, st, (const __bf16*)s, d, n);
  MIMO_KERNEL_CHECK();
  return MIMO_OK;
}
bool is_mixed(int precision) { return precision == MIMO_PREC_BF16_MIXED || precision == MIMO_PREC_FP16_MIXED; }

}

extern "C" {

int mimo_op_conv3x3_forward(const float* x, const float* w, const float* bias, float* z, double* stats, int32_t n,
                            int32_t h, int32_t wd, int32_t cin, int32_t cin_p, int32_t cout, int32_t cout_p,
                            int32_t precision, mimo_stream stream) {
  hipStream_t st = (hipStream_t)stream;
  Temp t;
  const int cout_pad = conv3x3_cout_pad(cout);
  const bool mixed = is_mixed(precision), f16s = precision == MIMO_PREC_FP16_MIXED;
  const bool split = precision == MIMO_PREC_SPLIT16 || precision == MIMO_PREC_BF16 || mixed;
  const bool bf16 = precision == MIMO_PREC_BF16 || precision == MIMO_PREC_BF16_MIXED;
  float* wf = t.get<float>((size_t)9 * cout_pad * cin_p);
  void* wpk = t.get<uint16_t>((size_t)ceil_div(cin_p, 32) * 9 * cout_pad * 64);
  float* bp = t.get<float>(cout_pad);
  int* rm = t.ints(ident_map(cout_pad, cout));
  int* cm = t.ints(ident_map(cin_p, cin));
  const int rows_cap = std::max(std::max(conv3x3_stat_rows(n, h, wd), conv3x3_ws_stat_rows(n, h, wd)), 2048);
  float* partial = t.get<float>((size_t)rows_cap * 2 * cout_pad);
  double* sums = t.get<double>((size_t)kMaxChunks * 2 * cout_pad);
  if (!wf || !bp || !rm || !cm || !partial || !sums) {
    set_error("mimo_op_conv3x3_forward: allocation failed");
    return MIMO_ERR_HIP;
  }
  MIMO_TRY(pack_weights_launch(w, wf, cout, cin, cout_pad, cin_p, rm, cm, 0, st));
  const int fmode = mixed ? (f16s ? 6 : 4) : (bf16 ? 2 : 1);
  const int wide = (precision == MIMO_PREC_SPLIT16 || mixed) ? conv3x3_wide_rows(fmode, n, cin_p, cout_p, h, wd) : 0;
  const int pair = (split && !wide) ? conv3x3_pair_tail(fmode, cin_p, h, wd) : 0;
  if (wide) {
    wpk = t.get<uint16_t>(conv3x3_wide_weight_elems(cin_p, wide));
    if (!wpk) {
      set_error("mimo_op_conv3x3_forward: allocation failed");
      return MIMO_ERR_HIP;
    }
    MIMO_TRY(pack_weights_wide_launch(w, wpk, bf16 ? 0 : 1, cout, cin, wide, cin_p, rm, cm, cout_pad, 0, st, mixed ? 1 : 0));
  } else if (split)
    MIMO_TRY(pack_weights_bf16x3_launch(w, wpk, bf16 ? 0 : 1, cout, cin, cout_pad, cin_p, rm, cm, 0, st, pair));
  if (bias) MIMO_HIP_CHECK(hipMemcpyAsync(bp, bias, cout * sizeof(float), hipMemcpyDeviceToDevice, st));
  const int64_t nx = (int64_t)n * h * wd * cin_p, nz = (int64_t)n * h * wd * cout_p;
  uint16_t *x16 = nullptr, *z16 = nullptr;
  if (mixed) {
    x16 = t.get<uint16_t>(nx);
    z16 = t.get<uint16_t>(nz);
    if (!x16 || !z16) {
      set_error("mimo_op_conv3x3_forward: allocation failed");
      return MIMO_ERR_HIP;
    }
    MIMO_TRY(to16(x, x16, nx, f16s, st));
  }
  ConvLaunch a;
  a.x = mixed ? reinterpret_cast<const float*>(x16) : x;
  a.y = mixed ? reinterpret_cast<float*>(z16) : z;
  a.w = wf;
  a.bias = bp;
  a.stats = stats ? partial : nullptr;
  a.N = n;
  a.Hi = a.Ho = h;
  a.Wi = a.Wo = wd;
  a.ldx = cin_p;
  a.cin_p = cin_p;
  a.ldy = cout_p;
  a.cout_pad = cout_pad;
  a.cout_store = cout_p;
  a.off = 1;
  a.wpk = wpk;
  a.pair = pair;
  a.wide = wide;
  int rows = 0;
  if (!mixed && cin_p < 16 && conv3x3_thin_ok(cin, cout_p))
    MIMO_TRY(conv3x3_thin_launch(a, cin, &rows, st));
  else if (split) {
    const size_t kfl = (mixed || wide) ? 0 : conv3x3_ksplit_scratch(fmode, n, cin_p, cout_pad, h, wd, cout_p);
    float* kpart = kfl ? t.get<float>(kfl) : nullptr;
    MIMO_TRY(conv3x3_bf16x3_launch_k(a, fmode, &rows, st, kpart, kfl));
  } else
    MIMO_TRY(conv3x3_launch(a, &rows, st));
  if (mixed) MIMO_TRY(from16(z16, z, nz, f16s, st));
  if (stats) {
    int chunks = 0;
    MIMO_TRY(rowsum_launch(partial, rows, 2 * cout_pad, sums, &chunks, st));
    hipLaunchKernelGGL(sums_to_stats_kernel, dim3(ceil_div(cout, 64)), dim3(64), 0, st, sums, chunks, cout_pad, cout, stats);
    MIMO_KERNEL_CHECK();
  }
  MIMO_HIP_CHECK(hipStreamSynchronize(st));
  return MIMO_OK;
}

int mimo_op_conv3x3_dgrad(const float* dz, const float* w, float* dx, int32_t n, int32_t h, int32_t wd, int32_t cin,
                          int32_t cin_p, int32_t cout, int32_t cout_p, int32_t precision, mimo_stream stream) {
  hipStream_t st = (hipStream_t)stream;
  Temp t;
  const int rows_pad = conv3x3_cout_pad(cin_p);
  const bool mixed = is_mixed(precision), f16s = precision == MIMO_PREC_FP16_MIXED;
  const bool split = precision == MIMO_PREC_SPLIT16 || precision == MIMO_PREC_BF16 || mixed;
  const bool bf16 = precision == MIMO_PREC_BF16;
  float* wdp = t.get<float>((size_t)9 * rows_pad * cout_p);
  void* wpk = t.get<uint16_t>((size_t)ceil_div(cout_p, 32) * 9 * rows_pad * 64);
  int* rm = t.ints(ident_map(rows_pad, cin));
  int* cm = t.ints(ident_map(cout_p, cout));
  float* dxpad = t.get<float>((size_t)n * (h + 2) * (wd + 2) * cin_p);
  if (!wdp || !rm || !cm || !dxpad) {
    set_error("mimo_op_conv3x3_dgrad: allocation failed");
    return MIMO_ERR_HIP;
  }
  MIMO_TRY(pack_weights_launch(w, wdp, cout, cin, rows_pad, cout_p, rm, cm, 1, st));
  const int dmode = mixed ? (f16s ? 7 : 5) : (bf16 ? 3 : 0);
  const int wide = (precision == MIMO_PREC_SPLIT16 || mixed) ? conv3x3_wide_rows(dmode, n, cout_p, cin_p, h + 2, wd + 2) : 0;
  const int pair = (split && !wide) ? conv3x3_pair_tail(dmode, cout_p, h + 2, wd + 2) : 0;
  if (wide) {
    wpk = t.get<uint16_t>(conv3x3_wide_weight_elems(cout_p, wide));
    if (!wpk) {
      set_error("mimo_op_conv3x3_dgrad: allocation failed");
      return MIMO_ERR_HIP;
    }
    MIMO_TRY(pack_weights_wide_launch(w, wpk, f16s ? 1 : 0, cout, cin, wide, cout_p, rm, cm, rows_pad, 1, st, mixed ? 1 : 0));
  } else if (split)
    MIMO_TRY(pack_weights_bf16x3_launch(w, wpk, f16s ? 1 : 0, cout, cin, rows_pad, cout_p, rm, cm, 1, st, pair));
  const float* dz_in = dz;
  const int64_t ndz = (int64_t)n * h * wd * cout_p, ndx = (int64_t)n * h * wd * cin_p;
  uint16_t* dx16 = nullptr;
  if (mixed) {
    uint16_t* dz16 = t.get<uint16_t>(ndz);
    dx16 = t.get<uint16_t>(ndx);
    if (!dz16 || !dx16) {
      set_error("mimo_op_conv3x3_dgrad: allocation failed");
      return MIMO_ERR_HIP;
    }
    MIMO_TRY(to16(dz, dz16, ndz, f16s, st));
    dz_in = reinterpret_cast<const float*>(dz16);
  } else if (split) {
    float* dzs = t.get<float>((size_t)n * h * wd * cout_p);
    if (!dzs) {
      set_error("mimo_op_conv3x3_dgrad: allocation failed");
      return MIMO_ERR_HIP;
    }
    MIMO_TRY(split_pairs_launch(dz, dzs, (int64_t)n * h * wd, cout_p, st));
    dz_in = dzs;
  }
  ConvLaunch a;
  a.x = dz_in;
  a.y = dxpad;
  a.w = wdp;
  a.bias = nullptr;
  a.stats = nullptr;
  a.N = n;
  a.Hi = h;
  a.Wi = wd;
  a.ldx = cout_p;
  a.cin_p = cout_p;
  a.Ho = h + 2;
  a.Wo = wd + 2;
  a.ldy = cin_p;
  a.cout_pad = rows_pad;
  a.cout_store = cin_p;
  a.off = 2;
  a.wpk = wpk;
  a.pair = pair;
  a.wide = wide;
  if (split) {
    const size_t kfl = (mixed || wide) ? 0 : conv3x3_ksplit_scratch(dmode, n, cout_p, rows_pad, h + 2, wd + 2, cin_p);
    float* kpart = kfl ? t.get<float>(kfl) : nullptr;
    MIMO_TRY(conv3x3_bf16x3_launch_k(a, dmode, nullptr, st, kpart, kfl));
  } else
    MIMO_TRY(conv3x3_launch(a, nullptr, st));
  if (mixed) {
    MIMO_TRY(fold_slice_launch(dxpad, f16s ? ST_F16 : ST_BF16, cin_p, 0, dx16, cin_p, n, h, wd, cin_p, 0, st));
    MIMO_TRY(from16(dx16, dx, ndx, f16s, st));
  } else {
    MIMO_TRY(fold_slice_launch(dxpad, ST_F32, cin_p, 0, dx, cin_p, n, h, wd, cin_p, 0, st));
  }
  MIMO_HIP_CHECK(hipStreamSynchronize(st));
  return MIMO_OK;
}

int mimo_op_conv3x3_wgrad(const float* x, const float* dz, float* dw, float* dbias, int32_t n, int32_t h, int32_t wd,
                          int32_t cin, int32_t cin_p, int32_t cout, int32_t cout_p, int32_t precision,
                          mimo_stream stream) {
  hipStream_t st = (hipStream_t)stream;
  Temp t;
  const bool mixed = is_mixed(precision), f16s = precision == MIMO_PREC_FP16_MIXED;
  const bool split = precision == MIMO_PREC_SPLIT16 || precision == MIMO_PREC_BF16 || mixed;
  const bool bf16 = precision == MIMO_PREC_BF16;
  if (!mixed && cin_p < 16 && wgrad_thin_ok(cin, cout_p, n, h, wd)) {
    float* part = t.get<float>(wgrad_thin_scratch(cin, cout_p));
    if (!part) {
      set_error("mimo_op_conv3x3_wgrad: allocation failed");
      return MIMO_ERR_HIP;
    }
    MIMO_TRY(wgrad_thin_launch(x, cin_p, dz, cout_p, n, h, wd, cin, cout, cout_p, part, dw, st));
    if (dbias) {
      hipLaunchKernelGGL(colsum_naive_kernel, dim3(cout), dim3(256), 0, st, dz, (int64_t)n * h * wd, cout_p, cout, dbias);
      MIMO_KERNEL_CHECK();
    }
    MIMO_HIP_CHECK(hipStreamSynchronize(st));
    return MIMO_OK;
  }
  WgradLaunch a;
  a.x = x;
  a.dz = dz;
  a.N = n;
  a.H = h;
  a.W = wd;
  a.ldx = cin_p;
  a.lddz = cout_p;
  a.cin_p = cin_p;
  a.cout_p = cout_p;
  if (split) {
    int CI, CO;
    wgrad_split_tiles(cin_p, cout_p, &CI, &CO);
    a.cin_pad = round_up(cin_p, CI);
    a.cout_pad = round_up(cout_p, CO);
    a.splits = wgrad_split_pick_splits(n, h, wd, a.cin_pad, a.cout_pad, CI, CO, mixed ? (f16s ? 2 : 1) : 0);
  } else {
    a.cin_pad = round_up(cin_p, 32);
    a.cout_pad = round_up(cout_p, 32);
    a.splits = wgrad_pick_splits(n, h, wd, a.cin_pad, a.cout_pad);
  }
  a.partial = t.get<float>((size_t)(a.splits + a.splits / 8 + 2) * 9 * a.cin_pad * a.cout_pad);
  int* cm = t.ints(ident_map(cin_p, cin));
  if (!a.partial || !cm) {
    set_error("mimo_op_conv3x3_wgrad: allocation failed");
    return MIMO_ERR_HIP;
  }
  if (mixed) {
    const int64_t nx = (int64_t)n * h * wd * cin_p, ndz = (int64_t)n * h * wd * cout_p;
    uint16_t *x16 = t.get<uint16_t>(nx), *dz16 = t.get<uint16_t>(ndz);
    if (!x16 || !dz16) {
      set_error("mimo_op_conv3x3_wgrad: allocation failed");
      return MIMO_ERR_HIP;
    }
    MIMO_TRY(to16(x, x16, nx, f16s, st));
    MIMO_TRY(to16(dz, dz16, ndz, f16s, st));
    a.x = reinterpret_cast<const float*>(x16);
    a.dz = reinterpret_cast<const float*>(dz16);
    a.np = 1;
    a.store = f16s ? 2 : 1;
    MIMO_TRY(wgrad_split_launch(a, st));
  } else if (split) {
    float* dzs = t.get<float>((size_t)n * h * wd * cout_p);
    if (!dzs) {
      set_error("mimo_op_conv3x3_wgrad: allocation failed");
      return MIMO_ERR_HIP;
    }
    float* amax = (!bf16 && wgrad_split_has_np2(cin_p, cout_p)) ? t.get<float>(kDzMaxSlots) : nullptr;
    int amax_n = 0;
    MIMO_TRY(split_pairs_launch(dz, dzs, (int64_t)n * h * wd, cout_p, st, amax, &amax_n));
    a.dz = dzs;
    a.np = bf16 ? 1 : amax ? 2 : 3;
    a.dz_absmax = amax;
    a.dz_absmax_n = amax_n;
    MIMO_TRY(wgrad_split_launch(a, st));
  } else {
    MIMO_TRY(wgrad_launch(a, st));
  }
  MIMO_TRY(wgrad_reduce_launch(a.partial, a.splits, a.cin_pad, a.cout_pad, cm, cin_p, cin, cout, dw, st, a.dz_absmax, a.dz_absmax_n));
  if (dbias) {
    hipLaunchKernelGGL(colsum_naive_kernel, dim3(cout), dim3(256), 0, st, dz, (int64_t)n * h * wd, cout_p, cout, dbias);
    MIMO_KERNEL_CHECK();
  }
  MIMO_HIP_CHECK(hipStreamSynchronize(st));
  return MIMO_OK;
}

int mimo_op_maxpool2x2(const float* x, float* y, int32_t n, int32_t h, int32_t w, int32_t c_p, mimo_stream stream) {
  MIMO_TRY(maxpool_fwd_launch(x, ST_F32, c_p, n, h, w, c_p, y, c_p, (hipStream_t)stream));
  return MIMO_OK;
}

int mimo_op_upsample_cat(const float* skip, const float* low, float* out, int32_t n, int32_t hs, int32_t ws, int32_t cs_p,
                         int32_t hl, int32_t wl, int32_t cl_p, mimo_stream stream) {
  MIMO_TRY(upcat_fwd_launch(skip, ST_F32, cs_p, cs_p, low, cl_p, cl_p, n, hs, ws, hl, wl, out, (hipStream_t)stream));
  return MIMO_OK;
}

}
```

mimo_unet_amd/csrc/plan.hip:

```cpp
#include <algorithm>
#include <cstdarg>
#include <cstdio>
#include <cstdlib>
#include <cstring>
#include <memory>
#include <string>
#include <vector>

#include "elementwise.h"

namespace mimo {

static thread_local char g_error[512] = "";
void set_error(const char* fmt, ...) {
  va_list ap;
  va_start(ap, fmt);
  vsnprintf(g_error, sizeof(g_error), fmt, ap);
  va_end(ap);
}
const char* last_error() { return g_error; }

namespace {

struct TensorInfo {
  std::string name;
  int ndim;
  int64_t shape[4];
  int kind;
  int64_t offset;
};

struct Act {
  float* a = nullptr;
  int ld = 0;
  float* da = nullptr;
  int ldda = 0;
  int Cp = 0, C = 0;
  int N = 0, H = 0, W = 0;
  std::vector<int> chmap;
  int grad_writes = 0;
  const float* skipgrad = nullptr;
  int skipgrad_ld = 0;
  const float* poolgrad = nullptr;
  int poolgrad_ld = 0;
  Act* parent = nullptr;
  int parent_choff = 0;
  const float *z = nullptr, *z_scale = nullptr, *z_shift = nullptr;
  int z_ld = 0;
  bool z_live = false;
};

struct ConvBN {
  std::string conv_name, bn_name;
  int Cin = 0, Cout = 0, cin_p = 0, cout_p = 0;
  int cout_pad = 0;
  int dg_rows = 0;
  int wg_cin_pad = 0, wg_cout_pad = 0, wg_splits = 1;
  int N = 0, H = 0, W = 0;
  int64_t off_w = 0, off_b = 0, off_gamma = 0, off_beta = 0, off_rm = 0, off_rv = 0;
  float *wf = nullptr, *wd = nullptr, *bias_p = nullptr;
  void *wf16 = nullptr, *wd16 = nullptr;
  bool fwd_split = false, dg_split = false, wg_split = false;
  unsigned* wmax = nullptr;
  bool wg_np2 = false;
  bool thin = false;
  int fwd_wide = 0, dg_wide = 0;
  int *cin_map = nullptr, *fwd_row_map = nullptr, *dg_row_map = nullptr, *dg_col_map = nullptr;
  float* z = nullptr;
  int dtz = ST_F32;
  float *mean = nullptr, *invstd = nullptr, *scale = nullptr, *shift = nullptr, *c1 = nullptr, *c2 = nullptr;
  const float* in = nullptr;
  int ld_in = 0;
  float* a = nullptr;
  int ld_a = 0;
  float* pool_out = nullptr;
  int pool_ld = 0;
  bool fuse_in = false, act_elided = false;
  const float* in_z = nullptr;
  int ld_in_z = 0;
  const float *in_scale = nullptr, *in_shift = nullptr;
};

enum InputKind { IN_IMAGE = 0, IN_POOL = 1, IN_UPCAT = 2 };

struct DoubleConv {
  std::string prefix;
  ConvBN c1, c2;
  InputKind kind = IN_IMAGE;
  int subnet = -1;
  Act* src0 = nullptr;
  Act* src1 = nullptr;
  float* in_buf = nullptr;
  int in_ld = 0;
  bool pool_fused = false;
  float* dxpad_own = nullptr;
  float* mid = nullptr;
  Act out;
  float drop_p = 0.f;
  const float* mask = nullptr;
  int64_t p_begin = 0, p_end = 0;
};

struct Head {
  int s = 0;
  int64_t off_w = 0, off_b = 0;
};

}
}

using namespace mimo;

struct mimo_plan {
  mimo_config cfg;
  int S, f, N, H, W, Ci, Co, Ci_p;
  bool mixed = false, f16 = false;
  int st = ST_F32, esz = 4;
  float* eoff(float* p, size_t elems) const { return reinterpret_cast<float*>(reinterpret_cast<char*>(p) + elems * esz); }
  int alloc_act(float** p, size_t elems, int dt) {
    return dalloc(p, (elems * store_bytes(dt) + 3) / 4);
  }
  int fwd_mode() const {
    return cfg.precision == MIMO_PREC_BF16 ? 2 : cfg.precision == MIMO_PREC_BF16_MIXED ? 4 : cfg.precision == MIMO_PREC_FP16_MIXED ? 6 : 1;
  }
  int dgrad_mode() const {
    return cfg.precision == MIMO_PREC_BF16 ? 3 : cfg.precision == MIMO_PREC_BF16_MIXED ? 5 : cfg.precision == MIMO_PREC_FP16_MIXED ? 7 : 0;
  }
  std::vector<TensorInfo> tensors;
  int64_t param_floats = 0, buffer_floats = 0;
  float *params = nullptr, *grads = nullptr, *bnbuf = nullptr;
  std::vector<void*> allocs;
  size_t bytes = 0;

  std::vector<std::unique_ptr<DoubleConv>> dcs;
  std::vector<DoubleConv*> enc_in, down1, up4;
  DoubleConv *down2 = nullptr, *down3 = nullptr, *down4 = nullptr, *up1 = nullptr, *up2 = nullptr, *up3 = nullptr;
  Act x2cat;
  std::vector<Head> heads;

  float *s_dz = nullptr, *s_dxpadA = nullptr, *s_dxpadB = nullptr, *s_wslab = nullptr,
        *s_partial = nullptr, *s_losspart = nullptr;
  float* s_headpart = nullptr;
  int head_rows = 0;
  double* s_sums = nullptr;
  int* s_tickets = nullptr;
  ColsumScratch colsum() const { return ColsumScratch{s_sums, s_tickets, d_status}; }
  int* d_status = nullptr;
  size_t cap_act = 0, cap_pad = 0, cap_slab = 0, cap_partial = 0, cap_sums = 0;
  float* s_kpart = nullptr;
  size_t cap_kpart = 0;

  bool wg_async = false;
  int wg_cus = 256;
  int wg_delay_us = 0;
  bool fuse_bwd_src = false;
  bool fuse_bwd_pool = false, fuse_bwd_head = false;
  hipStream_t wg_stream = nullptr;
#ifndef MIMO_DZ_BUFS
#define MIMO_DZ_BUFS 4
#endif
  static constexpr int kDzBufs = MIMO_DZ_BUFS;
  static constexpr int wg_bufs = kDzBufs;
  hipEvent_t ev_dz[kDzBufs] = {}, ev_wg[kDzBufs] = {}, ev_join = nullptr, ev_stage = nullptr;
  bool wg_pending[kDzBufs] = {};
  float* s_dz2[kDzBufs] = {};
  float* s_dzmax2[kDzBufs] = {};
  float* s_dzs2[kDzBufs] = {};
  bool any_mixed_dz = false;
  int dz_idx = 0;

  struct ProfRec {
    hipEvent_t a, b;
    int kind, tier;
  };
  int cur_tier = 0;
  double prof_kind_tier_ms[MIMO_PROF_KINDS][5] = {};
  bool prof_on = false;
  std::vector<ProfRec> prof_recs;
  std::vector<std::pair<hipEvent_t, hipEvent_t>> prof_pool;
  double prof_ms[MIMO_PROF_KINDS] = {}, prof_flops[MIMO_PROF_KINDS] = {}, prof_bytes[MIMO_PROF_KINDS] = {};
  int64_t prof_launches[MIMO_PROF_KINDS] = {};

  static constexpr int kProfTierBase = 100, kProfTiers = 5;
  double prof_tier_ms[2 * kProfTiers] = {};
  int tier_of(int h) const {
    int t = 0, hh = H;
    while (t < kProfTiers - 1 && hh > h) {
      hh /= 2;
      ++t;
    }
    return t;
  }
  int prof_begin(int kind, hipStream_t st) {
    if (!prof_on) return -1;
    ProfRec r;
    if (!prof_pool.empty()) {
      r.a = prof_pool.back().first;
      r.b = prof_pool.back().second;
      prof_pool.pop_back();
    } else {
      (void)hipEventCreate(&r.a);
      (void)hipEventCreate(&r.b);
    }
    r.kind = kind;
    if (kind >= kProfTierBase) cur_tier = (kind - kProfTierBase) / 2;
    r.tier = cur_tier;
    (void)hipEventRecord(r.a, st);
    prof_recs.push_back(r);
    return (int)prof_recs.size() - 1;
  }
  void prof_end(int idx, double flops, double bytes, hipStream_t st) {
    if (idx < 0 || !prof_on) return;
    (void)hipEventRecord(prof_recs[idx].b, st);
    const int kind = prof_recs[idx].kind;
    if (kind >= kProfTierBase) return;
    prof_flops[kind] += flops;
    prof_bytes[kind] += bytes;
    prof_launches[kind] += 1;
  }
  int prof_collect() {
    for (auto& r : prof_recs) {
      MIMO_HIP_CHECK(hipEventSynchronize(r.b));
      float ms = 0.f;
      MIMO_HIP_CHECK(hipEventElapsedTime(&ms, r.a, r.b));
      if (r.kind >= kProfTierBase)
        prof_tier_ms[r.kind - kProfTierBase] += ms;
      else {
        prof_ms[r.kind] += ms;
        prof_kind_tier_ms[r.kind][r.tier] += ms;
      }
      prof_pool.emplace_back(r.a, r.b);
    }
    prof_recs.clear();
    return MIMO_OK;
  }

  bool graph_enabled = true;
  hipStream_t cap_stream = nullptr;
  hipGraphExec_t graph_exec = nullptr;
  uint64_t graph_key = 0;
  bool train_graph = false;
  hipGraphExec_t tg_fwd = nullptr;
  uint64_t tg_fwd_key = 0, tg_fwd_seen = 0;
  static constexpr int kBwdGraphs = 9;
  hipGraphExec_t tg_bwd[kBwdGraphs] = {};
  uint64_t tg_bwd_key = 0, tg_bwd_seen = 0;
  bool tg_bwd_live = false;
  static constexpr int kMaxTrainCaptures = 24;
  int tg_captures = 0;
  bool fwd_graphed = false;
  bool loss_staged = false;
  int64_t last_x_rows = 0;
  const int64_t* last_perm_arg = nullptr;
  float *g_label = nullptr, *g_lmask = nullptr, *g_dloss = nullptr;
  int64_t* g_lperm = nullptr;
  void drop_train_graphs() {
    if (tg_fwd) (void)hipGraphExecDestroy(tg_fwd);
    tg_fwd = nullptr;
    tg_fwd_key = tg_fwd_seen = 0;
    for (auto& e : tg_bwd) {
      if (e) (void)hipGraphExecDestroy(e);
      e = nullptr;
    }
    tg_bwd_key = tg_bwd_seen = 0;
  }
  void drop_graphs() {
    if (graph_exec) (void)hipGraphExecDestroy(graph_exec);
    graph_exec = nullptr;
    drop_train_graphs();
  }
  float *g_x = nullptr, *g_out = nullptr;
  int64_t* g_perm = nullptr;
  std::vector<float*> g_masks;
  std::vector<const float*> g_mask_ptrs;
  Dropout2dSite* d_sites = nullptr;
  int max_site_count = 0;
  uint64_t rng_seed = 0, rng_offset = 0;
  std::vector<char> elem_rng_on;
  std::vector<const float*> eff_masks;
  float elem_rate(int j) const { return j == 0 ? cfg.center_dropout_rate : cfg.final_dropout_rate; }
  ElemRng elem_rng(int j) const { return ElemRng{rng_seed, rng_offset, (int)dcs.size() + j, elem_rate(j)}; }

  bool capturing = false;

  static constexpr int kMaxWmaxWords = 128;
  unsigned* wmax_pool = nullptr;
  int wmax_used = 0;
  PackJob* pack_jobs = nullptr;
  int n_fwd_jobs = 0, n_all_jobs = 0, pack_max_total = 0;

  bool fwd_done = false, fwd_training = false, had_perm = false, loss_done = false;
  int bwd_next_stage = 0;
  bool fwd_no_grad = false;
  int64_t derived_version = -1;
  bool derived_dgrad = false;
  bool need_derive = true;
  int64_t encoder_param_floats = 0;
  float* out = nullptr;
  const float *label = nullptr, *lmask = nullptr;
  std::vector<const float*> elem_masks;
  const int64_t* lperm = nullptr;

  ~mimo_plan() {
    for (void* p : allocs) (void)hipFree(p);
    for (auto& r : prof_recs) {
      (void)hipEventDestroy(r.a);
      (void)hipEventDestroy(r.b);
    }
    for (auto& e : prof_pool) {
      (void)hipEventDestroy(e.first);
      (void)hipEventDestroy(e.second);
    }
    drop_graphs();
    if (cap_stream) (void)hipStreamDestroy(cap_stream);
    if (wg_stream) (void)hipStreamDestroy(wg_stream);
    for (int i = 0; i < kDzBufs; ++i)
      for (hipEvent_t e : {ev_dz[i], ev_wg[i]})
        if (e) (void)hipEventDestroy(e);
    if (ev_join) (void)hipEventDestroy(ev_join);
    if (ev_stage) (void)hipEventDestroy(ev_stage);
  }

  template <typename T>
  int dalloc(T** p, size_t count) {
    void* q = nullptr;
    const size_t nbytes = std::max<size_t>(count, 1) * sizeof(T);
    MIMO_HIP_CHECK(hipMalloc(&q, nbytes));
    MIMO_HIP_CHECK(hipMemset(q, 0, nbytes));
    allocs.push_back(q);
    bytes += nbytes;
    *p = static_cast<T*>(q);
    return MIMO_OK;
  }
  int upload_ints(int** p, const std::vector<int>& v) {
    MIMO_TRY(dalloc(p, v.size()));
    MIMO_HIP_CHECK(hipMemcpy(*p, v.data(), v.size() * sizeof(int), hipMemcpyHostToDevice));
    return MIMO_OK;
  }

  int64_t add_tensor(const std::string& name, std::vector<int64_t> shape, int kind) {
    TensorInfo t;
    t.name = name;
    t.ndim = (int)shape.size();
    int64_t n = 1;
    for (int i = 0; i < 4; ++i) {
      t.shape[i] = i < t.ndim ? shape[i] : 1;
      n *= t.shape[i];
    }
    t.kind = kind;
    int64_t& cur = kind == 0 ? param_floats : buffer_floats;
    t.offset = cur;
    cur += (n + 3) / 4 * 4;
    tensors.push_back(t);
    return t.offset;
  }

  int init_convbn(ConvBN& L, const std::string& prefix, int conv_idx, int bn_idx, int Cin, int Cout,
                  const std::vector<int>& in_chmap, int n, int h, int w) {
    L.conv_name = prefix + "." + std::to_string(conv_idx);
    L.bn_name = prefix + "." + std::to_string(bn_idx);
    L.Cin = Cin;
    L.Cout = Cout;
    L.cin_p = (int)in_chmap.size();
    L.cout_p = pad_channels(Cout);
    L.cout_pad = conv3x3_cout_pad(Cout);
    L.dg_rows = conv3x3_cout_pad(L.cin_p);
    L.N = n;
    L.H = h;
    L.W = w;
    const bool mfma16 = cfg.precision != MIMO_PREC_FP32;
    L.wg_split = mfma16;
    if (L.wg_split) {
      int CI, CO;
      wgrad_split_tiles(L.cin_p, L.cout_p, &CI, &CO);
      L.wg_cin_pad = round_up(L.cin_p, CI);
      L.wg_cout_pad = round_up(L.cout_p, CO);
      const int wg_store = !mixed ? 0 : (L.cin_p >= 8 ? (f16 ? 2 : 1) : (f16 ? 4 : 3));
      L.wg_splits = wgrad_split_pick_splits(n, h, w, L.wg_cin_pad, L.wg_cout_pad, CI, CO, wg_store, wg_cus);
    } else {
      L.wg_cin_pad = round_up(L.cin_p, 32);
      L.wg_cout_pad = round_up(L.cout_p, 32);
      L.wg_splits = wgrad_pick_splits(n, h, w, L.wg_cin_pad, L.wg_cout_pad);
    }
    L.off_w = add_tensor(L.conv_name + ".weight", {Cout, Cin, 3, 3}, 0);
    L.off_b = add_tensor(L.conv_name + ".bias", {Cout}, 0);
    L.off_gamma = add_tensor(L.bn_name + ".weight", {Cout}, 0);
    L.off_beta = add_tensor(L.bn_name + ".bias", {Cout}, 0);
    L.off_rm = add_tensor(L.bn_name + ".running_mean", {Cout}, 1);
    L.off_rv = add_tensor(L.bn_name + ".running_var", {Cout}, 1);
    const bool train_bufs = !cfg.inference_only;
    MIMO_TRY(dalloc(&L.wf, (size_t)9 * L.cout_pad * L.cin_p));
    if (train_bufs) MIMO_TRY(dalloc(&L.wd, (size_t)9 * L.dg_rows * L.cout_p));
    MIMO_TRY(dalloc(&L.bias_p, L.cout_pad));
    L.fwd_split = mfma16 && L.cin_p >= (mixed ? 8 : 16);
    L.dg_split = mfma16 && (mixed || L.cout_p >= 16);
    L.dtz = L.fwd_split ? st : ST_F32;
    {
      bool ident = true;
      for (int i = 0; i < Cin; ++i) ident = ident && i < (int)in_chmap.size() && in_chmap[i] == i;
      L.thin = !L.fwd_split && ident && conv3x3_thin_ok(Cin, L.cout_p);
      if (L.thin && train_bufs) cap_slab = std::max(cap_slab, wgrad_thin_scratch(Cin, L.cout_p));
    }
    if (L.wg_split && !L.dg_split) any_mixed_dz = true;
    L.wg_np2 = cfg.precision == MIMO_PREC_SPLIT16 && L.wg_split && train_bufs && L.fwd_split && wgrad_split_has_np2(L.cin_p, L.cout_p) &&
               2048 * ceil_div(L.cout_p / 4, 256) <= kDzMaxSlots;
    if (cfg.precision == MIMO_PREC_SPLIT16 || mixed) {
      if (L.fwd_split) L.fwd_wide = conv3x3_wide_rows(fwd_mode(), n, L.cin_p, L.cout_p, h, w);
      if (L.dg_split) L.dg_wide = conv3x3_wide_rows(dgrad_mode(), n, L.cout_p, L.cin_p, h + 2, w + 2);
    }
    if (cfg.precision == MIMO_PREC_SPLIT16) {
      if (L.fwd_split && !L.fwd_wide && !cfg.inference_only)
        cap_kpart = std::max(cap_kpart, conv3x3_ksplit_scratch(fwd_mode(), n, L.cin_p, L.cout_pad, h, w, L.cout_p));
      if (L.dg_split && !L.dg_wide && train_bufs)
        cap_kpart = std::max(cap_kpart, conv3x3_ksplit_scratch(dgrad_mode(), n, L.cout_p, L.dg_rows, h + 2, w + 2, L.cin_p));
    }
    if (L.fwd_split && (cfg.precision == MIMO_PREC_SPLIT16 || cfg.precision == MIMO_PREC_FP16_MIXED)) {
      if (!wmax_pool) MIMO_TRY(dalloc(&wmax_pool, kMaxWmaxWords));
      if (wmax_used >= kMaxWmaxWords) {
        set_error("too many convolution layers (%d) for the fp16 weight-scale words", wmax_used + 1);
        return MIMO_ERR_INVALID;
      }
      L.wmax = wmax_pool + wmax_used++;
    }
    if (L.fwd_split) {
      uint16_t* q = nullptr;
      MIMO_TRY(dalloc(&q, L.fwd_wide ? conv3x3_wide_weight_elems(L.cin_p, L.fwd_wide)
                                     : (size_t)ceil_div(L.cin_p, 32) * 9 * L.cout_pad * 64));
      L.wf16 = q;
    }
    if (L.dg_split && train_bufs) {
      uint16_t* q = nullptr;
      MIMO_TRY(dalloc(&q, L.dg_wide ? conv3x3_wide_weight_elems(L.cout_p, L.dg_wide)
                                    : (size_t)ceil_div(L.cout_p, 32) * 9 * L.dg_rows * 64));
      L.wd16 = q;
    }
    MIMO_TRY(upload_ints(&L.cin_map, in_chmap));
    std::vector<int> frm(L.cout_pad), drm(L.dg_rows), dcm(L.cout_p);
    for (int i = 0; i < L.cout_pad; ++i) frm[i] = i < Cout ? i : -1;
    for (int i = 0; i < L.dg_rows; ++i) drm[i] = i < L.cin_p ? in_chmap[i] : -1;
    for (int i = 0; i < L.cout_p; ++i) dcm[i] = i < Cout ? i : -1;
    MIMO_TRY(upload_ints(&L.fwd_row_map, frm));
    MIMO_TRY(upload_ints(&L.dg_row_map, drm));
    MIMO_TRY(upload_ints(&L.dg_col_map, dcm));
    if (train_bufs || (mixed && !L.fwd_split)) MIMO_TRY(alloc_act(&L.z, (size_t)n * h * w * L.cout_p, L.dtz));
    MIMO_TRY(dalloc(&L.mean, L.cout_p));
    MIMO_TRY(dalloc(&L.invstd, L.cout_p));
    MIMO_TRY(dalloc(&L.scale, L.cout_p + kFinSlack));
    MIMO_TRY(dalloc(&L.shift, L.cout_p + kFinSlack));
    MIMO_TRY(dalloc(&L.c1, L.cout_p));
    MIMO_TRY(dalloc(&L.c2, L.cout_p));
    const size_t act = (size_t)n * h * w * L.cout_p;
    const size_t padv = (size_t)n * (h + 2) * (w + 2) * L.cin_p;
    cap_act = std::max(cap_act, act);
    cap_pad = std::max(cap_pad, padv);
    cap_slab = std::max(cap_slab, (size_t)(L.wg_splits + L.wg_splits / 8 + 2) * 9 * L.wg_cin_pad * L.wg_cout_pad);
    const size_t stat_rows = std::max(conv3x3_stat_rows(n, h, w), conv3x3_ws_stat_rows(n, h, w));
    cap_partial = std::max(cap_partial, stat_rows * 2 * L.cout_pad);
    cap_partial = std::max(cap_partial, (size_t)kBnReduceMaxBlocks * 2 * L.cout_p);
    cap_sums = std::max(cap_sums, (size_t)kMaxChunks * 2 * round_up(std::max(L.cout_pad, L.cout_p), 64));
    return MIMO_OK;
  }

  int make_dc(DoubleConv** outp, const std::string& prefix, const std::vector<int>& in_chmap, int Cin, int Cmid,
              int Cout, int h, int w, float drop_p, float* out_a, int out_ld, float* out_da, int out_ldda) {
    auto dc = std::make_unique<DoubleConv>();
    dc->prefix = prefix;
    dc->drop_p = drop_p;
    dc->p_begin = param_floats;
    MIMO_TRY(init_convbn(dc->c1, prefix, 0, 1, Cin, Cmid, in_chmap, N, h, w));
    std::vector<int> midmap(pad_channels(Cmid));
    for (size_t i = 0; i < midmap.size(); ++i) midmap[i] = (int)i < Cmid ? (int)i : -1;
    MIMO_TRY(init_convbn(dc->c2, prefix, 3, 4, Cmid, Cout, midmap, N, h, w));
    dc->p_end = param_floats;
    MIMO_TRY(alloc_act(&dc->mid, (size_t)N * h * w * dc->c1.cout_p, st));
    Act& o = dc->out;
    o.N = N;
    o.H = h;
    o.W = w;
    o.C = Cout;
    o.Cp = dc->c2.cout_p;
    o.chmap.resize(o.Cp);
    for (int i = 0; i < o.Cp; ++i) o.chmap[i] = i < Cout ? i : -1;
    if (out_a) {
      o.a = out_a;
      o.ld = out_ld;
      o.da = out_da;
      o.ldda = out_ldda;
    } else {
      MIMO_TRY(alloc_act(&o.a, (size_t)N * h * w * o.Cp, st));
      if (!cfg.inference_only) MIMO_TRY(alloc_act(&o.da, (size_t)N * h * w * o.Cp, st));
      o.ld = o.ldda = o.Cp;
    }
    dc->c1.a = dc->mid;
    dc->c1.ld_a = dc->c1.cout_p;
    dc->c2.in = dc->mid;
    dc->c2.ld_in = dc->c1.cout_p;
    {
      const bool on = !(getenv("MIMO_FUSE_BN_IN") && atoi(getenv("MIMO_FUSE_BN_IN")) == 0);
      ConvBN& c2 = dc->c2;
      if (on && cfg.precision == MIMO_PREC_SPLIT16 && !cfg.inference_only && c2.fwd_split && c2.wg_split && dc->c1.dtz == ST_F32 &&
          conv3x3_split_fuses_input(fwd_mode(), c2.fwd_wide, h, w) && wgrad_split_fuses_input(c2.cin_p, c2.cout_p, 0, 3)) {
        c2.fuse_in = true;
        c2.in_z = dc->c1.z;
        c2.ld_in_z = dc->c1.cout_p;
        c2.in_scale = dc->c1.scale;
        c2.in_shift = dc->c1.shift;
        dc->c1.act_elided = true;
      }
    }
    dc->c2.a = o.a;
    dc->c2.ld_a = o.ld;
    *outp = dc.get();
    dcs.push_back(std::move(dc));
    return MIMO_OK;
  }

  void rehome_skip(Act& sk, DoubleConv* up, std::vector<std::pair<DoubleConv*, int>> producers) {
    sk.a = up->in_buf;
    sk.ld = up->in_ld;
    for (auto& pr : producers) {
      DoubleConv* dc = pr.first;
      dc->c2.a = eoff(up->in_buf, pr.second);
      dc->c2.ld_a = up->in_ld;
      dc->out.a = dc->c2.a;
      dc->out.ld = up->in_ld;
    }
  }

  int set_input(DoubleConv* dc, InputKind kind, Act* s0, Act* s1, int in_cp, int h, int w) {
    dc->kind = kind;
    dc->src0 = s0;
    dc->src1 = s1;
    MIMO_TRY(alloc_act(&dc->in_buf, (size_t)N * h * w * in_cp, kind == IN_IMAGE ? ST_F32 : st));
    if (kind == IN_UPCAT && !cfg.inference_only)
      MIMO_TRY(alloc_act(&dc->dxpad_own, (size_t)N * (h + 2) * (w + 2) * in_cp, st));
    if (kind == IN_POOL && fuse_bwd_pool) MIMO_TRY(alloc_act(&dc->dxpad_own, (size_t)N * (h + 2) * (w + 2) * in_cp, st));
    dc->in_ld = in_cp;
    dc->c1.in = dc->in_buf;
    dc->c1.ld_in = in_cp;
    return MIMO_OK;
  }

  static std::vector<int> cat_map(const Act& a, const Act& b) {
    std::vector<int> m = a.chmap;
    for (int v : b.chmap) m.push_back(v < 0 ? -1 : v + a.C);
    return m;
  }

  int build() {
    mixed = cfg.precision == MIMO_PREC_BF16_MIXED || cfg.precision == MIMO_PREC_FP16_MIXED;
    f16 = cfg.precision == MIMO_PREC_FP16_MIXED;
    st = !mixed ? ST_F32 : f16 ? ST_F16 : ST_BF16;
    esz = store_bytes(st);
    {
      const int v = getenv("MIMO_FUSE_BWD_SRC") ? atoi(getenv("MIMO_FUSE_BWD_SRC")) : 1;
      fuse_bwd_src = !mixed && !cfg.inference_only && v != 0;
      fuse_bwd_pool = fuse_bwd_src && v != 3;
      fuse_bwd_head = fuse_bwd_src && v != 2;
    }
    if (cfg.precision < MIMO_PREC_FP32 || cfg.precision > MIMO_PREC_FP16_MIXED) {
      set_error("unknown precision %d", cfg.precision);
      return MIMO_ERR_INVALID;
    }
    if (cfg.norm_kind != MIMO_NORM_BATCH || cfg.act_kind != MIMO_ACT_RELU || cfg.up_kind != MIMO_UP_BILINEAR_ALIGN_CORNERS) {
      set_error("block variant norm %d / act %d / up %d is not implemented: only BatchNorm2d + ReLU + bilinear align_corners "
                "up-sampling, the reference's blocks (components.py:22-30, 77-85)", cfg.norm_kind, cfg.act_kind, cfg.up_kind);
      return MIMO_ERR_INVALID;
    }
    S = cfg.num_subnetworks;
    f = cfg.filter_base_count;
    N = cfg.batch;
    H = cfg.height;
    W = cfg.width;
    Ci = cfg.in_channels;
    Co = cfg.out_channels;
    Ci_p = round_up(Ci, 4);
    {
      const char* e = getenv("MIMO_WGRAD_CUS");
      const int v = e ? atoi(e) : 0;
      wg_cus = (v >= 8 && v <= 256) ? v : sched::wg_side_cus((long)N * H * W, S * f);
      const char* d = getenv("MIMO_DEBUG_WGRAD_DELAY_US");
      wg_delay_us = d ? std::max(0, std::min(atoi(d), 5000)) : 0;
    }
    if (S < 1 || f < 1 || N < 1 || Ci < 1 || Co < 2 || (Co & 1) || Co > kMaxHeadOut || f > 256) {
      set_error("unsupported configuration S=%d f=%d N=%d Ci=%d Co=%d", S, f, N, Ci, Co);
      return MIMO_ERR_INVALID;
    }
    if ((H >> 4) < 2 || (W >> 4) < 2) {
      set_error("input %dx%d too small: reflect padding needs >= 2 pixels at 1/16 resolution", H, W);
      return MIMO_ERR_INVALID;
    }
    const int H1 = H, W1 = W, H2 = H / 2, W2 = W / 2, H3 = H2 / 2, W3 = W2 / 2, H4 = H3 / 2, W4 = W3 / 2, H5 = H4 / 2,
              W5 = W4 / 2;
    std::vector<int> imgmap(Ci_p);
    for (int i = 0; i < Ci_p; ++i) imgmap[i] = i < Ci ? i : -1;

    for (int s = 0; s < S; ++s) {
      DoubleConv* dc;
      MIMO_TRY(make_dc(&dc, "encoder.in_convs." + std::to_string(s) + ".double_conv", imgmap, Ci, f, f, H1, W1,
                       cfg.encoder_dropout_rate, nullptr, 0, nullptr, 0));
      MIMO_TRY(set_input(dc, IN_IMAGE, nullptr, nullptr, Ci_p, H1, W1));
      dc->subnet = s;
      enc_in.push_back(dc);
    }
    const int c2p = pad_channels(2 * f);
    x2cat.N = N;
    x2cat.H = H2;
    x2cat.W = W2;
    x2cat.C = 2 * f * S;
    x2cat.Cp = c2p * S;
    x2cat.ld = x2cat.ldda = x2cat.Cp;
    MIMO_TRY(alloc_act(&x2cat.a, (size_t)N * H2 * W2 * x2cat.Cp, st));
    if (!cfg.inference_only) MIMO_TRY(alloc_act(&x2cat.da, (size_t)N * H2 * W2 * x2cat.Cp, st));
    x2cat.chmap.assign(x2cat.Cp, -1);
    for (int s = 0; s < S; ++s)
      for (int c = 0; c < 2 * f; ++c) x2cat.chmap[s * c2p + c] = s * 2 * f + c;
    for (int s = 0; s < S; ++s) {
      DoubleConv* dc;
      MIMO_TRY(make_dc(&dc, "encoder.down1s." + std::to_string(s) + ".conv.double_conv", enc_in[s]->out.chmap, f, 2 * f,
                       2 * f, H2, W2, cfg.encoder_dropout_rate, eoff(x2cat.a, (size_t)s * c2p), x2cat.Cp,
                       x2cat.da ? eoff(x2cat.da, (size_t)s * c2p) : nullptr, x2cat.Cp));
      MIMO_TRY(set_input(dc, IN_POOL, &enc_in[s]->out, nullptr, enc_in[s]->out.Cp, H2, W2));
      dc->out.parent = &x2cat;
      dc->out.parent_choff = s * c2p;
      down1.push_back(dc);
    }
    encoder_param_floats = param_floats;
    const float pc = cfg.core_dropout_rate;
    MIMO_TRY(make_dc(&down2, "core.down2.conv.double_conv", x2cat.chmap, 2 * f * S, 4 * f * S, 4 * f * S, H3, W3, pc,
                     nullptr, 0, nullptr, 0));
    MIMO_TRY(set_input(down2, IN_POOL, &x2cat, nullptr, x2cat.Cp, H3, W3));
    MIMO_TRY(make_dc(&down3, "core.down3.conv.double_conv", down2->out.chmap, 4 * f * S, 8 * f * S, 8 * f * S, H4, W4, pc,
                     nullptr, 0, nullptr, 0));
    MIMO_TRY(set_input(down3, IN_POOL, &down2->out, nullptr, down2->out.Cp, H4, W4));
    MIMO_TRY(make_dc(&down4, "core.down4.conv.double_conv", down3->out.chmap, 8 * f * S, 8 * f * S, 8 * f * S, H5, W5, pc,
                     nullptr, 0, nullptr, 0));
    MIMO_TRY(set_input(down4, IN_POOL, &down3->out, nullptr, down3->out.Cp, H5, W5));
    {
      std::vector<int> m = cat_map(down3->out, down4->out);
      MIMO_TRY(make_dc(&up1, "core.up1.conv.double_conv", m, 16 * f * S, 8 * f * S, 4 * f * S, H4, W4, pc, nullptr, 0,
                       nullptr, 0));
      MIMO_TRY(set_input(up1, IN_UPCAT, &down3->out, &down4->out, (int)m.size(), H4, W4));
      rehome_skip(down3->out, up1, {{down3, 0}});
    }
    {
      std::vector<int> m = cat_map(down2->out, up1->out);
      MIMO_TRY(make_dc(&up2, "core.up2.conv.double_conv", m, 8 * f * S, 4 * f * S, 2 * f * S, H3, W3, pc, nullptr, 0,
                       nullptr, 0));
      MIMO_TRY(set_input(up2, IN_UPCAT, &down2->out, &up1->out, (int)m.size(), H3, W3));
      rehome_skip(down2->out, up2, {{down2, 0}});
    }
    {
      std::vector<int> m = cat_map(x2cat, up2->out);
      MIMO_TRY(make_dc(&up3, "core.up3.conv.double_conv", m, 4 * f * S, 2 * f * S, f * S, H2, W2, pc, nullptr, 0, nullptr,
                       0));
      MIMO_TRY(set_input(up3, IN_UPCAT, &x2cat, &up2->out, (int)m.size(), H2, W2));
      std::vector<std::pair<DoubleConv*, int>> pr;
      for (int s = 0; s < S; ++s) pr.push_back({down1[s], s * c2p});
      rehome_skip(x2cat, up3, pr);
    }
    elide_output(up1);
    elide_output(up2);
    elide_output(up3);
    {
      auto fuse = [this](DoubleConv* producer, DoubleConv* consumer, int choff) {
        producer->c2.pool_out = eoff(consumer->in_buf, choff);
        producer->c2.pool_ld = consumer->in_ld;
        consumer->pool_fused = true;
      };
      for (int s = 0; s < S; ++s) fuse(enc_in[s], down1[s], 0);
      for (int s = 0; s < S; ++s) fuse(down1[s], down2, s * c2p);
      fuse(down2, down3, 0);
      fuse(down3, down4, 0);
    }
    const int cin_dec = f * S + f;
    for (int s = 0; s < S; ++s) {
      std::vector<int> m = cat_map(enc_in[s]->out, up3->out);
      DoubleConv* dc;
      MIMO_TRY(make_dc(&dc, "decoder.up4s." + std::to_string(s) + ".conv.double_conv", m, cin_dec, cin_dec / 2, f, H1, W1,
                       cfg.decoder_dropout_rate, nullptr, 0, nullptr, 0));
      MIMO_TRY(set_input(dc, IN_UPCAT, &enc_in[s]->out, &up3->out, (int)m.size(), H1, W1));
      rehome_skip(enc_in[s]->out, dc, {{enc_in[s], 0}});
      if (cfg.final_dropout_rate <= 0.f) elide_output(dc);
      up4.push_back(dc);
    }
    for (int s = 0; s < S; ++s) {
      Head h;
      h.s = s;
      const std::string p = "decoder.outcs." + std::to_string(s) + ".conv";
      h.off_w = add_tensor(p + ".weight", {Co, f, 1, 1}, 0);
      h.off_b = add_tensor(p + ".bias", {Co}, 0);
      heads.push_back(h);
    }

    const int fp = pad_channels(f);
    cap_partial = std::max(cap_partial, (size_t)kEwMaxBlocks * (Co * fp + Co));
    cap_sums = std::max(cap_sums, (size_t)kMaxChunks * 2 * round_up(Co * fp + Co, 64));
    if (cfg.inference_only) cap_act = cap_pad = cap_slab = 1;
    MIMO_TRY(alloc_act(&s_dz, cap_act, st));
    {
      const char* we = getenv("MIMO_WGRAD_STREAM");
      wg_async = !(we && atoi(we) == 0) && !cfg.inference_only;
      for (int i = 0; i < kDzBufs; ++i) s_dz2[i] = s_dz;
      if (!cfg.inference_only)
        for (int i = 0; i < kDzBufs; ++i) MIMO_TRY(dalloc(&s_dzmax2[i], kDzMaxSlots));
      if (any_mixed_dz) {
// ... 399 lines not shown
    for (size_t i = 0; i < dcs.size(); ++i) dcs[i]->mask = args->drop_masks ? args->drop_masks[i] : nullptr;
    elem_masks.assign(1 + S, nullptr);
    if (args->elem_masks)
      for (int i = 0; i <= S; ++i) elem_masks[i] = args->elem_masks[i];
    if (need_derive) MIMO_TRY(pack_all(training, st));
    for (int s = 0; s < S; ++s)
      MIMO_TRY(pack_input_launch(args->x, args->stride_n, args->stride_s, args->perm, s, N, Ci, H, W, enc_in[s]->in_buf,
                                 Ci_p, st));
    for (int s = 0; s < S; ++s) {
      MIMO_TRY(dc_forward(enc_in[s], training, st));
      MIMO_TRY(dc_forward(down1[s], training, st));
    }
    MIMO_TRY(dc_forward(down2, training, st));
    MIMO_TRY(dc_forward(down3, training, st));
    MIMO_TRY(dc_forward(down4, training, st));
    if (elem_masks[0] || elem_rng_on[0]) {
      const ElemRng g = elem_rng(0);
      MIMO_TRY(elem_mask_mul_launch(down4->out.a, this->st, down4->out.ld, elem_masks[0], N, down4->out.C, down4->out.Cp,
                                    down4->out.H * down4->out.W, st, elem_masks[0] ? nullptr : &g));
    }
    MIMO_TRY(dc_forward(up1, training, st));
    MIMO_TRY(dc_forward(up2, training, st));
    MIMO_TRY(dc_forward(up3, training, st));
    for (int s = 0; s < S; ++s) {
      MIMO_TRY(dc_forward(up4[s], training, st, elem_masks[1 + s] || elem_rng_on[1 + s]));
      const Act& o = up4[s]->out;
      if (elem_masks[1 + s] || elem_rng_on[1 + s]) {
        const ElemRng g = elem_rng(1 + s);
        MIMO_TRY(elem_mask_mul_launch(o.a, this->st, o.ld, elem_masks[1 + s], N, o.C, o.Cp, H * W, st,
                                      elem_masks[1 + s] ? nullptr : &g));
      }
      const int blk = prof_begin(kProfTierBase, st);
      const int pr = prof_begin(MIMO_PROF_HEAD_FWD, st);
      const bool oz = o.z_live;
      MIMO_TRY(head_fwd_launch(oz ? o.z : o.a, this->st, oz ? o.z_ld : o.ld, params + heads[s].off_w, params + heads[s].off_b, f, Co,
                               N, S, s, H * W, args->out, st, d_status, oz ? o.z_scale : nullptr, oz ? o.z_shift : nullptr));
      prof_end(pr, 0.0, 4.0 * (double)N * H * W * (pad_channels(f) + Co), st);
      prof_end(blk, 0.0, 0.0, st);
    }
    out = args->out;
    fwd_done = true;
    fwd_training = training;
    had_perm = args->perm != nullptr;
    loss_done = false;
    return MIMO_OK;
  }

  int loss_forward(const float* label_, const float* mask_, const int64_t* perm_, float* loss_out, hipStream_t st) {
    if (!fwd_done) {
      set_error("mimo_loss_forward: call mimo_forward first");
      return MIMO_ERR_STATE;
    }
    if (!label_ || !loss_out) {
      set_error("mimo_loss_forward: null argument");
      return MIMO_ERR_INVALID;
    }
    loss_staged = false;
    if (fwd_graphed && train_graph && last_x_rows >= 1 && last_x_rows <= N) {
      const size_t hw = (size_t)H * W;
      MIMO_HIP_CHECK(hipMemcpyAsync(g_label, label_, (size_t)last_x_rows * (Co / 2) * hw * sizeof(float), hipMemcpyDeviceToDevice, st));
      label_ = g_label;
      if (mask_) {
        MIMO_HIP_CHECK(hipMemcpyAsync(g_lmask, mask_, (size_t)last_x_rows * hw * sizeof(float), hipMemcpyDeviceToDevice, st));
        mask_ = g_lmask;
      }
      if (perm_ && perm_ == last_perm_arg) {
        perm_ = g_perm;
      } else if (perm_) {
        MIMO_HIP_CHECK(hipMemcpyAsync(g_lperm, perm_, (size_t)S * N * sizeof(int64_t), hipMemcpyDeviceToDevice, st));
        perm_ = g_lperm;
      }
      loss_staged = true;
    }
    int blocks = 0;
    MIMO_TRY(loss_fwd_launch(out, label_, mask_, perm_, N, S, Co, H * W, cfg.loss_kind, cfg.eps_min, cfg.eps_max,
                             s_losspart, &blocks, st));
    MIMO_TRY(loss_finalize_launch(s_losspart, S, blocks, (double)N * (Co / 2) * H * W, loss_out, st));
    label = label_;
    lmask = mask_;
    lperm = perm_;
    loss_done = true;
    return MIMO_OK;
  }

  static int acc_flag(Act* t) { return t->grad_writes++ > 0 ? 1 : 0; }

  int convbn_backward(ConvBN& L, const GradSrc& src, const float* mask, bool need_dgrad, float* dxpad_out, hipStream_t st) {
    int rows = 0;
    const int64_t P = (int64_t)L.N * L.H * L.W;
    const double src_b = src.kind == GS_POOL ? (1.0 + (src.skip ? 4.0 : 0.0)) : src.kind == GS_HEAD ? 0.5 : 4.0;
    int pr = prof_begin(MIMO_PROF_BN_BWD_REDUCE, st);
    MIMO_TRY(bnrelu_bwd_reduce_launch(src, this->st, L.z, L.dtz, L.cout_p, L.scale, L.shift, L.mean, L.invstd,
                                      mask, L.Cout, L.cout_p, L.N, L.H, L.W, s_partial, &rows, st));
    prof_end(pr, 0.0, (4.0 + src_b) * (double)P * L.cout_p, st);
    if (src.kind == GS_HEAD) head_rows = rows;
    MIMO_TRY(bn_bwd_stats_launch(s_partial, rows, L.Cout, L.cout_p, P, fwd_training ? 1 : 0, L.c1, L.c2,
                                 grads + L.off_gamma, grads + L.off_beta, fwd_training ? grads + L.off_b : nullptr, colsum(), st));
    const bool async = wg_async && !prof_on;
    const int b = dz_idx;
    float* dz = s_dz2[b];
    if (async) {
      dz_idx = (dz_idx + 1) % wg_bufs;
      if (kDzBufs >= 4 && (kDzBufs & 1) == 0) {
        if ((b & 1) == 0) {
          const int w = wg_pending[b + 1] ? b + 1 : b;
          if (wg_pending[w]) MIMO_HIP_CHECK(hipStreamWaitEvent(st, ev_wg[w], 0));
          wg_pending[b] = wg_pending[b + 1] = false;
        } else if (wg_pending[b]) {
          MIMO_HIP_CHECK(hipStreamWaitEvent(st, ev_wg[b], 0));
        }
      } else if (wg_pending[b]) {
        MIMO_HIP_CHECK(hipStreamWaitEvent(st, ev_wg[b], 0));
      }
    }
    const bool thin_wg = L.thin && !mixed && !need_dgrad && wgrad_thin_ok(L.Cin, L.cout_p, L.N, L.H, L.W);
    pr = prof_begin(MIMO_PROF_BN_BWD_APPLY, st);
    int dzmax_n = 0;
    const bool needs_split_copy = L.wg_split && !L.dg_split && !thin_wg;
    const bool ev_on_launch = async && !capturing && !needs_split_copy;
    MIMO_TRY(bn_bwd_apply_launch(src, this->st, L.z, L.dtz, L.cout_p, L.scale, L.shift, L.mean, L.invstd, mask,
                                 L.Cout, L.c1, L.c2, L.cout_p, L.N, L.H, L.W, dz, (L.dg_split && !mixed && !thin_wg) ? 1 : 0,
                                 fwd_training ? nullptr : s_partial, &rows, st, (L.wg_np2 && !thin_wg) ? s_dzmax2[b] : nullptr,
                                 &dzmax_n, ev_on_launch ? ev_dz[b] : nullptr));
    prof_end(pr, 0.0, (8.0 + src_b) * (double)P * L.cout_p, st);
    const float* dz_wg = dz;
    if (needs_split_copy) {
      float* dzs = s_dzs2[b];
      MIMO_TRY(split_pairs_launch(dz, dzs, P, L.cout_p, st));
      dz_wg = dzs;
    }
    if (async && !ev_on_launch) MIMO_HIP_CHECK(hipEventRecord(ev_dz[b], st));
    if (!fwd_training) MIMO_TRY(colsum_vec_launch(s_partial, rows, L.cout_p, L.Cout, grads + L.off_b, colsum(), st));
    if (need_dgrad) {
      ConvLaunch a;
      a.x = dz;
      a.y = dxpad_out;
      a.w = L.wd;
      a.bias = nullptr;
      a.stats = nullptr;
      a.N = L.N;
      a.Hi = L.H;
      a.Wi = L.W;
      a.ldx = L.cout_p;
      a.cin_p = L.cout_p;
      a.Ho = L.H + 2;
      a.Wo = L.W + 2;
      a.ldy = L.cin_p;
      a.cout_pad = L.dg_rows;
      a.cout_store = L.cin_p;
      a.off = 2;
      a.wpk = L.wd16;
      a.pair = (L.dg_split && !L.dg_wide) ? conv3x3_pair_tail(dgrad_mode(), L.cout_p, L.H + 2, L.W + 2) : 0;
      a.wide = L.dg_wide;
      pr = prof_begin(MIMO_PROF_CONV_DGRAD, st);
      if (L.dg_split)
        MIMO_TRY(conv3x3_bf16x3_launch_k(a, dgrad_mode(), nullptr, st, s_kpart, cap_kpart));
      else
        MIMO_TRY(conv3x3_launch(a, nullptr, st));
      prof_end(pr, 18.0 * L.Cin * L.Cout * (double)P, 4.0 * (double)P * (L.Cin + L.Cout), st);
    }
    hipStream_t ws = st;
    if (async) {
      MIMO_HIP_CHECK(hipStreamWaitEvent(wg_stream, ev_dz[b], 0));
      ws = wg_stream;
    }
    WgradLaunch wg;
    wg.x = L.fuse_in ? L.in_z : L.in;
    if (L.fuse_in) {
      wg.in_scale = L.in_scale;
      wg.in_shift = L.in_shift;
    }
    wg.dz = dz_wg;
    wg.partial = s_wslab;
    wg.N = L.N;
    wg.H = L.H;
    wg.W = L.W;
    wg.ldx = L.fuse_in ? L.ld_in_z : L.ld_in;
    wg.lddz = L.cout_p;
    wg.cin_p = L.cin_p;
    wg.cout_p = L.cout_p;
    wg.cin_pad = L.wg_cin_pad;
    wg.cout_pad = L.wg_cout_pad;
    wg.splits = L.wg_splits;
    wg.np = (cfg.precision == MIMO_PREC_BF16 || mixed) ? 1 : 3;
    if (L.wg_np2 && wg.np == 3 && !thin_wg) {
      wg.np = 2;
      wg.dz_absmax = s_dzmax2[b];
      wg.dz_absmax_n = dzmax_n;
    }
    wg.store = !mixed ? 0 : (L.fwd_split ? (f16 ? 2 : 1) : (f16 ? 4 : 3));
    if (wg_delay_us > 0) MIMO_TRY(debug_delay_launch(wg_delay_us, ws));
    pr = prof_begin(MIMO_PROF_CONV_WGRAD, ws);
    if (thin_wg)
      MIMO_TRY(wgrad_thin_launch(L.in, L.ld_in, dz, L.cout_p, L.N, L.H, L.W, L.Cin, L.Cout, L.cout_p, s_wslab, grads + L.off_w, ws));
    else if (L.wg_split)
      MIMO_TRY(wgrad_split_launch(wg, ws));
    else
      MIMO_TRY(wgrad_launch(wg, ws));
    prof_end(pr, 18.0 * L.Cin * L.Cout * (double)P, 4.0 * (double)P * (L.Cin + L.Cout), ws);
    const bool wg_ev_on_launch = async && !capturing && !thin_wg;
    if (!thin_wg)
      MIMO_TRY(wgrad_reduce_launch(s_wslab, L.wg_splits, L.wg_cin_pad, L.wg_cout_pad, L.cin_map, L.cin_p, L.Cin, L.Cout,
                                   grads + L.off_w, ws, wg.dz_absmax, wg.dz_absmax_n, wg_ev_on_launch ? ev_wg[b] : nullptr));
    if (async) {
      if (!wg_ev_on_launch) MIMO_HIP_CHECK(hipEventRecord(ev_wg[b], wg_stream));
      wg_pending[b] = true;
    }
    return MIMO_OK;
  }

  int wg_join(hipStream_t st) {
    bool any = false;
    for (bool p : wg_pending) any |= p;
    if (!wg_async || !any) return MIMO_OK;
    MIMO_HIP_CHECK(hipEventRecord(ev_join, wg_stream));
    MIMO_HIP_CHECK(hipStreamWaitEvent(st, ev_join, 0));
    for (bool& p : wg_pending) p = false;
    return MIMO_OK;
  }

  int dc_backward(DoubleConv* dc, bool need_input_grad, hipStream_t st, const GradSrc* head_src = nullptr) {
    const int blk = prof_begin(kProfTierBase + 2 * tier_of(dc->c1.H) + 1, st);
    const int rc = dc_backward_impl(dc, need_input_grad, st, head_src);
    prof_end(blk, 0.0, 0.0, st);
    return rc;
  }

  int dc_backward_impl(DoubleConv* dc, bool need_input_grad, hipStream_t st, const GradSrc* head_src = nullptr) {
    GradSrc src = GradSrc::plain(dc->out.da, dc->out.ldda);
    {
      const Act* root = dc->out.parent ? dc->out.parent : &dc->out;
      if (head_src) {
        src = *head_src;
      } else if (root->poolgrad) {
        src.kind = GS_POOL;
        src.dxpad = root->poolgrad;
        src.ldp = root->poolgrad_ld;
        src.skip = root->skipgrad;
        src.ldsk = root->skipgrad_ld;
        src.choff = src.skoff = dc->out.parent ? dc->out.parent_choff : 0;
      }
    }
    MIMO_TRY(convbn_backward(dc->c2, src, dc->mask, true, s_dxpadA, st));
    float* dxB = dc->dxpad_own ? dc->dxpad_own : s_dxpadB;
    MIMO_TRY(convbn_backward(dc->c1, GradSrc::fold(s_dxpadA, dc->c1.cout_p), nullptr, need_input_grad, dxB, st));
    if (!need_input_grad) return MIMO_OK;
    const int h = dc->c1.H, w = dc->c1.W, ldp = dc->c1.cin_p;
    if (dc->kind == IN_POOL && fuse_bwd_pool && dc->dxpad_own && dc->src0->grad_writes == 0) {
      Act* s = dc->src0;
      s->poolgrad = dxB;
      s->poolgrad_ld = ldp;
    } else if (dc->kind == IN_POOL) {
      Act* s = dc->src0;
      const int pr = prof_begin(MIMO_PROF_POOL_BWD, st);
      const bool acc = acc_flag(s) != 0;
      MIMO_TRY(pool_bwd_launch(dxB, this->st, ldp, 0, s->a, s->ld, s->da, s->ldda, N, s->H, s->W, s->Cp, acc ? 1 : 0, st, s->skipgrad,
                               s->skipgrad_ld));
      prof_end(pr, 0.0, 4.0 * s->Cp * (double)N * s->H * s->W * (2.25 + (s->skipgrad ? 1.0 : 0.0) + (acc ? 1.0 : 0.0)), st);
      s->skipgrad = nullptr;
    } else if (dc->kind == IN_UPCAT) {
      Act *sk = dc->src0, *lo = dc->src1;
      sk->skipgrad = dxB;
      sk->skipgrad_ld = ldp;
      const int pr = prof_begin(MIMO_PROF_UP_BWD, st);
      MIMO_TRY(up_bwd_launch(dxB, this->st, ldp, sk->Cp, lo->da, lo->ldda, N, h, w, lo->H, lo->W, lo->Cp, acc_flag(lo), st));
      prof_end(pr, 0.0, 4.0 * lo->Cp * ((double)N * (h + 2) * (w + 2) + (double)N * lo->H * lo->W), st);
    }
    return MIMO_OK;
  }

  static constexpr int kBwdStages = 8;
  void stage_range(int stage, int64_t* b, int64_t* e) const {
    DoubleConv* core[6] = {up3, up2, up1, down4, down3, down2};
    if (stage == 0) {
      *b = up4[0]->p_begin;
      *e = param_floats;
    } else if (stage == kBwdStages - 1) {
      *b = 0;
      *e = encoder_param_floats;
    } else {
      *b = core[stage - 1]->p_begin;
      *e = core[stage - 1]->p_end;
    }
  }

  int backward(const float* dout, const float* dloss, float* dx, int stage_first, int stage_last, hipStream_t st,
               hipStream_t* ready = nullptr) {
    if (ready) *ready = st;
    if (!fwd_done) {
      set_error("mimo_backward: call mimo_forward first");
      return MIMO_ERR_STATE;
    }
    if (!grads) {
      set_error("mimo_backward: gradient buffer not bound");
      return MIMO_ERR_STATE;
    }
    if (fwd_no_grad) {
      set_error("mimo_backward: the last forward ran with no_grad (inference epilogue, nothing saved)");
      return MIMO_ERR_STATE;
    }
    if (!dout && !dloss) {
      set_error("mimo_backward: need dout and/or dloss");
      return MIMO_ERR_INVALID;
    }
    if (dloss && !loss_done) {
      set_error("mimo_backward: dloss given but mimo_loss_forward was not called");
// ... 371 lines not shown
```

mimo_unet_amd/csrc/tile_sched.h:

```cpp
#pragma once

#include <cstdint>

#if defined(__HIPCC__)
#define MIMO_SCHED_HD __host__ __device__
#else
#define MIMO_SCHED_HD
#endif

namespace mimo {
namespace sched {

MIMO_SCHED_HD static inline int cdiv(int a, int b) { return (a + b - 1) / b; }
MIMO_SCHED_HD static inline int rup(int a, int b) { return cdiv(a, b) * b; }

MIMO_SCHED_HD static inline int xcd_virtual_index(int linear, int total) {
  const int k = linear & 7, slot = linear >> 3;
  const int base = total >> 3, rem = total & 7;
  return k * base + (k < rem ? k : rem) + slot;
}

static inline void pick_tile_n(int Ho, int Wo, int npix, int maxpix, int* TR, int* TC) {
  double best_eff = -1.0;
  int best_tr = 1, best_tc = 4, best_pix = 1 << 30;
  for (int k = 1; k <= Wo; ++k) {
    int tc = cdiv(Wo, k);
    if (tc > npix) continue;
    int tr = npix / tc;
    if (tr > Ho) tr = Ho;
    while (tr > 1 && (tr + 2) * (tc + 2) > maxpix) --tr;
    if (tr < 1 || (tr + 2) * (tc + 2) > maxpix) continue;
    double eff = double(Ho) * Wo / (double(cdiv(Ho, tr)) * cdiv(Wo, tc) * npix);
    int pix = (tr + 2) * (tc + 2);
    if (eff > best_eff + 1e-9 || (eff > best_eff - 1e-9 && pix < best_pix)) {
      best_eff = eff;
      best_tr = tr;
      best_tc = tc;
      best_pix = pix;
    }
    if (tc <= 4) break;
  }
  *TR = best_tr;
  *TC = best_tc;
}

static inline int conv_pick_nfrag(int cout) {
  const int nfr = cdiv(cout, 16);
  if (nfr <= 1) return 1;
  int best = 2, best_cost = 1 << 30;
  for (int nf = 4; nf >= 2; --nf) {
    const int cost = rup(nfr, nf);
    if (cost < best_cost) {
      best_cost = cost;
      best = nf;
    }
  }
  return best;
}
static inline int conv_cout_pad(int cout) { return rup(cdiv(cout, 16), conv_pick_nfrag(cout)) * 16; }

constexpr int kWgTC = 32;
static inline int wg_pick_ctile(int c_p) {
  if (c_p <= 32) return 32;
  const int p64 = rup(c_p, 64), p48 = rup(c_p, 48);
  return double(p48) <= 0.70 * p64 ? 48 : 64;
}
static inline void wg_tiles(int cin_p, int cout_p, bool ws_enabled, int* CI, int* CO) {
  *CI = wg_pick_ctile(cin_p);
  *CO = wg_pick_ctile(cout_p);
  if (*CI == 64 && ws_enabled && cout_p > 32 && rup(cout_p, 48) <= 0.85 * rup(cout_p, 64)) *CO = 48;
  if (*CI == 64 && ws_enabled && rup(cin_p, 32) <= 0.80 * rup(cin_p, 64)) *CI = 32;
}
static inline bool wg_use_ws(int CI, int CO, bool ws_enabled) {
  return ws_enabled && (CI == 64 || CI == 32) && (CO == 32 || CO == 48 || CO == 64);
}
static inline int wg_ws_tr(int CI, bool s16 = false) { return (CI == 32 || s16) ? 4 : 2; }
static inline int wg_num_tiles(int N, int H, int W, int tr) { return N * cdiv(H, tr) * cdiv(W, kWgTC); }
static inline int wg_pick_splits(int N, int H, int W, int cin_pad, int cout_pad, int CI, int CO, bool ws_enabled,
                                 bool s16 = false, int cus = 256) {
  const int wtiles = (cin_pad / CI) * (cout_pad / CO);
  const bool ws = wg_use_ws(CI, CO, ws_enabled);
  const int tiles = wg_num_tiles(N, H, W, ws ? wg_ws_tr(CI, s16) : 4);
  if (!ws) {
    int splits = cdiv(512, wtiles);
    if (splits > tiles) splits = tiles;
    if (splits > 1024) splits = 1024;
    if (splits < 1) splits = 1;
    return splits;
  }
  const int kCUs = cus;
  const int kFixed = 16 / wg_ws_tr(CI, s16);
  int best = 1;
  long bestCost = -1;
  for (int s = 1; s <= tiles && s <= 1024; ++s) {
    const long rounds = cdiv(wtiles * s, kCUs);
    const long cost = rounds * (cdiv(tiles, s) + kFixed);
    if (bestCost < 0 || cost < bestCost) bestCost = cost, best = s;
  }
  return best;
}

static inline int wg_side_cus(long pixels, int width) {
  const long work = pixels * (long)width, unit = 65536L * 60;
  return work <= 6 * unit ? 128 : work <= 24 * unit ? 192 : 256;
}

MIMO_SCHED_HD static inline float pow2_bits(int k) {
  union { unsigned u; float v; } c;
  c.u = (unsigned)(127 + k) << 23;
  return c.v;
}
MIMO_SCHED_HD static inline float w16_scale(unsigned wmax_bits, bool inverse) {
  const int e = (int)((wmax_bits >> 23) & 0xffu) - 127;
  int k = e < 7 ? 8 : 13 - e;
  k = k < -100 ? -100 : k;
  return pow2_bits(inverse ? -k : k);
}
MIMO_SCHED_HD static inline float wg_dz_scale(unsigned absmax_bits, bool inverse) {
  int e = (int)((absmax_bits >> 23) & 0xffu);
  e = e < 16 ? 16 : e > 254 ? 254 : e;
  const int k = 141 - e;
  return pow2_bits(inverse ? -k : k);
}

constexpr int kWideNPix = 512;
constexpr int kWideMaxPix = 640;

struct WideCfg {
  int nf;
  int rows_pad;
  int TR, TC;
};

static inline int wide_grid_x(int numTiles, int cotiles);

static inline WideCfg wide_config(int mode, int N, int cin_p, int rows, int Ho, int Wo, int force) {
  WideCfg c{0, 0, 0, 0};
  const bool s16 = mode >= 4 && mode <= 7;
  if (force < 0 || !(mode == 0 || mode == 1 || s16) || rows < 1 || cin_p < 16 || Ho < 2 || Wo < 2) return c;
  if (s16 && cin_p % 8 != 0) return c;
  if (mode == 0 && rows % 8 != 0) return c;
  if (int64_t(Ho + 2) * int64_t(Wo + 2) * int64_t(cin_p < rows ? rows : cin_p) * 8 > int64_t(INT32_MAX)) return c;
  int TR, TC;
  pick_tile_n(Ho, Wo, kWideNPix, kWideMaxPix, &TR, &TC);
  if ((TR + 2) * (TC + 2) > kWideMaxPix) return c;
  const int tiles = N * cdiv(Ho, TR) * cdiv(Wo, TC);
  const double eff = double(N) * Ho * Wo / (double(tiles) * kWideNPix);
  const int r32 = cdiv(rows, 32);
  const int nf = (r32 >= 2 && double(rup(r32, 2)) / r32 <= 1.10 + 1e-9) ? 2 : 1;
  const int cotiles = cdiv(r32, nf);
  if (force == 0) {
    const int k16 = rup(cin_p, s16 ? 32 : 16);
    int TRo, TCo;
    pick_tile_n(Ho, Wo, 256, 360, &TRo, &TCo);
    const double eff_o = double(Ho) * Wo / (double(cdiv(Ho, TRo)) * cdiv(Wo, TCo) * 256);
    const int tail = cin_p - 32 * (cdiv(cin_p, 32) - 1);
    const double k_o = 32.0 * (cdiv(cin_p, 32) - 1) + ((tail <= 16 && !s16) ? 64.0 / 3.0 : 32.0);
    double t_w = double(k16) * (cotiles * nf * 32) / eff * (1.0 + (nf == 2 ? 1.2 : 0.2) / (k16 / (s16 ? 32 : 16)));
    double t_o = (s16 ? 1.45 : 1.15) * k_o * rup(rows, 16) / eff_o;
    {
      const int cu_w = wide_grid_x(tiles, cotiles) * cotiles;
      const int nf_o = conv_pick_nfrag(rows);
      const int cot_o = cdiv(cdiv(rows, 16), nf_o);
      const int tiles_o = N * cdiv(Ho, TRo) * cdiv(Wo, TCo);
      int gx_o = 256 / cot_o > 0 ? 256 / cot_o : 1;
      if (gx_o > tiles_o) gx_o = tiles_o;
      const int cu_o = cdiv(tiles_o, cdiv(tiles_o, gx_o)) * cot_o;
      if (cu_w < 192) t_w *= 256.0 / cu_w;
      if (cu_o < 192) t_o *= 256.0 / cu_o;
    }
    const int gx = 256 / cotiles < tiles ? (256 / cotiles > 0 ? 256 / cotiles : 1) : tiles;
    if (tiles * cotiles < 256 || cdiv(tiles, gx) * (k16 / (s16 ? 32 : 16)) < 8 || t_w >= t_o) return c;
  }
  c.nf = nf;
  c.rows_pad = cotiles * nf * 32;
  c.TR = TR;
  c.TC = TC;
  return c;
}

static inline int wide_grid_x(int numTiles, int cotiles) {
  int gx = 256 / cotiles;
  if (gx < 1) gx = 1;
  if (gx > numTiles) gx = numTiles;
  const int per = cdiv(numTiles, gx);
  return cdiv(numTiles, per);
}

}
}
```

Baseline: 1346 images/s.

## Stack batch images vertically into one tall image for dgrad conv tiling

For the data-gradient convolution (mode 0), the batch is treated as one tall image (N*Ho rows) so tiles can span full rows across image boundaries. Per-tap image membership is computed with a magic-number division, and out-of-image rows are masked. This is meant to reduce tile padding waste on small feature maps, where per-image tiling leaves partially empty tiles. In exchange it adds index math in the load path and changes the wide-vs-split heuristics. It is enabled by default through MIMO_CONV_STACK=1.

```diff
diff --git a/mimo_unet_amd/csrc/common.h b/mimo_unet_amd/csrc/common.h
--- a/mimo_unet_amd/csrc/common.h
+++ b/mimo_unet_amd/csrc/common.h
@@ -63,10 +63,14 @@
   const float* in_shift = nullptr;
   const unsigned* wmax = nullptr;
   int ksplit = 1;
+  int stack = 0;
+  int stack_rows = 0, stack_n = 0;
+  unsigned stack_magic = 0;
 };
-int conv3x3_ksplit(int mode, int N, int cin_p, int cout_pad, int Ho, int Wo);
+int conv3x3_stack_switch();
+int conv3x3_ksplit(int mode, int N, int cin_p, int cout_pad, int Ho, int Wo, int stack = 0);
 int conv3x3_bf16x3_launch_k(const ConvLaunch& a, int mode, int* rows, hipStream_t stream, float* kpart, size_t kpart_floats);
-size_t conv3x3_ksplit_scratch(int mode, int N, int cin_p, int cout_pad, int Ho, int Wo, int ldy);
+size_t conv3x3_ksplit_scratch(int mode, int N, int cin_p, int cout_pad, int Ho, int Wo, int ldy, int stack = 0);
 int conv3x3_split_fuses_input(int mode, int wide, int Ho, int Wo);
 int conv3x3_launch(const ConvLaunch& a, int* rows, hipStream_t stream);
 int conv3x3_thin_ok(int cin, int cout_p);
@@ -79,7 +83,7 @@
 int pack_weights_bf16x3_launch(const float* w, void* dst, int f16, int cout, int cin, int rows_pad, int cols,
                                const int* row_map, const int* col_map, int transposed, hipStream_t stream, int pair = 0);
 int conv3x3_pair_tail(int mode, int cin_p, int Ho, int Wo);
-int conv3x3_wide_rows(int mode, int N, int cin_p, int rows, int Ho, int Wo);
+int conv3x3_wide_rows(int mode, int N, int cin_p, int rows, int Ho, int Wo, int stack = 0);
 size_t conv3x3_wide_weight_elems(int cin_p, int rows_pad);
 int conv3x3_wide_stat_rows();
 int conv3x3_wide_launch(const ConvLaunch& a, int mode, int* rows, hipStream_t stream);
diff --git a/mimo_unet_amd/csrc/conv_bf16x3.hip b/mimo_unet_amd/csrc/conv_bf16x3.hip
--- a/mimo_unet_amd/csrc/conv_bf16x3.hip
+++ b/mimo_unet_amd/csrc/conv_bf16x3.hip
@@ -382,6 +382,8 @@
       u_off[k] = ((tr * a.Wi + tc) * a.ldx + 4 * ((ptid + k * 256) & 7)) * 4;
     }
     const u32x4* wpk = reinterpret_cast<const u32x4*>(a.wpk);
+    const int s_rows = a.stack_rows, s_nav = a.stack_n;
+    const unsigned s_magic = a.stack_magic;
     f32x4 in_sc = f32x4{0.f, 0.f, 0.f, 0.f}, in_sh = in_sc, in_sc_n = in_sc, in_sh_n = in_sc;
 #define WS_LOAD_SS(SC, SH, STAGE)                                                                    \
   if (FIN) {                                                                                         \
@@ -403,7 +405,8 @@
     const float* ximg_ = a.x + (size_t)n_ * a.Hi * a.Wi * a.ldx;                                     \
     const unsigned short* ximg16_ = reinterpret_cast<const unsigned short*>(a.x) + (size_t)n_ * a.Hi * a.Wi * a.ldx; \
                                                                          \
-    if (!CVT && !IN16 && y0_ >= 0 && y0_ + TRP <= a.Hi && x0_ >= 0 && x0_ + TCP <= a.Wi && ck_ * 32 + 32 <= a.cin_p) { \
+    if (!CVT && !IN16 && !a.stack_rows && y0_ >= 0 && y0_ + TRP <= a.Hi && x0_ >= 0 && x0_ + TCP <= a.Wi &&       \
+        ck_ * 32 + 32 <= a.cin_p) {                                                                  \
       const char* tb_ = reinterpret_cast<const char*>(ximg_ + ((size_t)y0_ * a.Wi + x0_) * a.ldx) + ck_ * 128; \
       _Pragma("unroll") for (int k_ = (K0); k_ < (K1); ++k_)                                         \
         xreg[k_] = *reinterpret_cast<const f32x4*>(tb_ + u_off[k_]);                                 \
@@ -417,7 +420,15 @@
         ix_ = max(ix_, -ix_);                                                                        \
         ix_ = max(min(ix_, 2 * a.Wi - 2 - ix_), 0);                                                  \
       } else {                                            \
-        in_ = iy_ >= 0 && iy_ < a.Hi && ix_ >= 0 && ix_ < a.Wi;                                      \
+        if (!FWD && a.stack_rows) {                            \
+                             \
+          const int d_ = (int)__umulhi((unsigned)(iy_ + s_rows), s_magic) - 1;                       \
+          iy_ -= d_ * s_rows;                                                                        \
+          in_ = d_ >= 0 && d_ < s_nav && iy_ < a.Hi && ix_ >= 0 && ix_ < a.Wi;                       \
+          iy_ += d_ * a.Hi;                                                                          \
+        } else {                                                                                     \
+          in_ = iy_ >= 0 && iy_ < a.Hi && ix_ >= 0 && ix_ < a.Wi;                                    \
+        }                                                                                            \
       }                                                                                              \
       const int q_ = (ptid + k_ * 256) & (UPP - 1);                                                  \
       const int o_ = in_ ? (iy_ * a.Wi + ix_) * a.ldx : 0;                                           \
@@ -762,9 +773,20 @@
 }
 
 template <int NF, int MODE, int MF>
-static int launch_ws(const ConvLaunch& a, int* rows, hipStream_t stream) {
+static int launch_ws(const ConvLaunch& a_, int* rows, hipStream_t stream) {
   int TR, TC;
-  pick_tile_n(a.Ho, a.Wo, WsTile<MF>::NPIX, WsTile<MF>::MAXPIX, &TR, &TC);
+  ConvLaunch a = a_;
+  if (MODE == 0 && a_.stack > 0 && (int64_t)a_.N * a_.Hi * a_.Wi * a_.ldx <= (int64_t)INT32_MAX &&
+      sched::use_tile_stacked(a_.N, a_.Ho, a_.Wo, WsTile<MF>::NPIX, WsTile<MF>::MAXPIX, ceil_div(a_.cout_pad / 16, 4), a_.stack,
+                              &TR, &TC)) {
+    a.stack_rows = a_.Ho;
+    a.stack_n = a_.N;
+    a.stack_magic = sched::stacked_magic(a_.Ho);
+    a.Ho = a_.N * a_.Ho;
+    a.N = 1;
+  } else {
+    pick_tile_n(a.Ho, a.Wo, WsTile<MF>::NPIX, WsTile<MF>::MAXPIX, &TR, &TC);
+  }
   const int tilesY = ceil_div(a.Ho, TR), tilesX = ceil_div(a.Wo, TC);
   const int numTiles = a.N * tilesY * tilesX;
   const int coTiles = a.cout_pad / (NF * 16);
@@ -787,7 +809,7 @@
   const int xcd = 1;
   if (a.in_scale) {
     if constexpr (MODE == 1) {
-      if (a.ep_scale || !a.in_shift || (a.pair && a.pair != conv3x3_pair_tail(MODE, a.cin_p, a.Ho, a.Wo))) {
+      if (a.ep_scale || !a.in_shift || (a.pair && a.pair != conv3x3_pair_tail(MODE, a.cin_p, a_.Ho, a_.Wo))) {
         set_error("conv3x3 split: the input BatchNorm + ReLU can be fused into the split16 training forward only");
         return MIMO_ERR_INVALID;
       }
@@ -804,7 +826,7 @@
   }
   if (a.pair) {
     if constexpr (MODE <= 1) {
-      if (a.pair != conv3x3_pair_tail(MODE, a.cin_p, a.Ho, a.Wo)) {
+      if (a.pair != conv3x3_pair_tail(MODE, a.cin_p, a_.Ho, a_.Wo)) {
         set_error("conv3x3 split: weights packed for tap pairing, launch is not");
         return MIMO_ERR_INVALID;
       }
@@ -831,6 +853,13 @@
   return MIMO_OK;
 }
 
+static int ws_num_tiles(int mode, int N, int Ho, int Wo, int cout_pad, int stack) {
+  int TR, TC;
+  if (sched::use_tile_stacked(N, Ho, Wo, WsTile<4>::NPIX, WsTile<4>::MAXPIX, ceil_div(cout_pad / 16, 4), mode == 0 ? stack : 0, &TR, &TC))
+    return ceil_div(N * Ho, TR);
+  return N * ceil_div(Ho, TR) * ceil_div(Wo, TC);
+}
+
 static bool use_big_tile(int Ho, int Wo) { return Ho * Wo >= 1024; }
 
 int conv3x3_split_fuses_input(int mode, int wide, int Ho, int Wo) {
@@ -848,9 +877,7 @@
   while (nfr % nf != 0) --nf;
   if (conv_ws_enabled() && a.Ho * a.Wo >= 256) {
     if (a.ksplit <= 1) {
-      int TR, TC;
-      pick_tile_n(a.Ho, a.Wo, WsTile<4>::NPIX, WsTile<4>::MAXPIX, &TR, &TC);
-      const int numTiles = a.N * ceil_div(a.Ho, TR) * ceil_div(a.Wo, TC);
+      const int numTiles = ws_num_tiles(MODE, a.N, a.Ho, a.Wo, a.cout_pad, a.stack);
       long best = -1;
       for (int c = 4; c >= 1; --c) {
         if (nfr % c) continue;
@@ -888,7 +915,7 @@
 }
 
 constexpr int kKsplitReduceUnits = 14;
-int conv3x3_ksplit(int mode, int N, int cin_p, int cout_pad, int Ho, int Wo) {
+int conv3x3_ksplit(int mode, int N, int cin_p, int cout_pad, int Ho, int Wo, int stack) {
   static const int force = [] { const char* e = getenv("MIMO_CONV_KSPLIT"); return e ? atoi(e) : -1; }();
   if (force == 0 || (mode != 0 && mode != 1) || !conv_ws_enabled() || Ho * Wo < 256 || cin_p % 32 != 0 ||
       cout_pad % 16 != 0)
@@ -901,9 +928,7 @@
     while (ks >= 2 && !legal(ks)) --ks;
     return ks >= 2 ? ks : 1;
   }
-  int TR, TC;
-  pick_tile_n(Ho, Wo, WsTile<4>::NPIX, WsTile<4>::MAXPIX, &TR, &TC);
-  const int numTiles = N * ceil_div(Ho, TR) * ceil_div(Wo, TC);
+  const int numTiles = ws_num_tiles(mode, N, Ho, Wo, cout_pad, stack);
   const int nfr = cout_pad / 16;
   long unsplit = -1;
   for (int c = 4; c >= 1; --c) {
@@ -926,8 +951,8 @@
   return (best_cost >= 0 && best_cost * 100 < unsplit * 85) ? best : 1;
 }
 
-size_t conv3x3_ksplit_scratch(int mode, int N, int cin_p, int cout_pad, int Ho, int Wo, int ldy) {
-  const int ks = conv3x3_ksplit(mode, N, cin_p, cout_pad, Ho, Wo);
+size_t conv3x3_ksplit_scratch(int mode, int N, int cin_p, int cout_pad, int Ho, int Wo, int ldy, int stack) {
+  const int ks = conv3x3_ksplit(mode, N, cin_p, cout_pad, Ho, Wo, stack);
   return ks > 1 ? (size_t)ks * N * Ho * Wo * ldy : 0;
 }
 
@@ -969,7 +994,7 @@
 }
 
 int conv3x3_bf16x3_launch_k(const ConvLaunch& a, int mode, int* rows, hipStream_t stream, float* kpart, size_t kpart_floats) {
-  const int ks = (a.wide || a.ep_scale || !kpart) ? 1 : conv3x3_ksplit(mode, a.N, a.cin_p, a.cout_pad, a.Ho, a.Wo);
+  const int ks = (a.wide || a.ep_scale || !kpart) ? 1 : conv3x3_ksplit(mode, a.N, a.cin_p, a.cout_pad, a.Ho, a.Wo, a.stack);
   const size_t need = (size_t)ks * a.N * a.Ho * a.Wo * a.ldy;
   if (ks <= 1 || a.pair || need > kpart_floats || a.cout_store % 4 != 0 || a.ldy % 4 != 0 || (size_t)a.N * a.Ho * a.Wo > (1u << 30))
     return conv3x3_bf16x3_launch(a, mode, rows, stream);
diff --git a/mimo_unet_amd/csrc/conv_wide.hip b/mimo_unet_amd/csrc/conv_wide.hip
--- a/mimo_unet_amd/csrc/conv_wide.hip
+++ b/mimo_unet_amd/csrc/conv_wide.hip
@@ -126,6 +126,10 @@
     const char* l_img = nullptr;
     int l_y0 = 0, l_x0 = 0;
     bool l_new = true;
+    const int s_rows = a.stack_rows;
+    const unsigned s_magic = a.stack_magic;
+    int l_nav = 1;
+    (void)s_rows; (void)s_magic; (void)l_nav;
     f32x4 in_sc = f32x4{0.f, 0.f, 0.f, 0.f}, in_sh = in_sc, in_sc_n = in_sc, in_sh_n = in_sc;
 #define WD_LOAD_SS(SC, SH, CK)                                                                       \
   if (FIN) {                                                                                         \
@@ -143,7 +147,13 @@
     const int n_ = t_ / tilesY;                                                                      \
     l_y0 = ty_ * TR - a.off;                                                                         \
     l_x0 = tx_ * TC - a.off;                                                                         \
-    l_img = reinterpret_cast<const char*>(a.x) + (size_t)n_ * a.Hi * a.Wi * a.ldx * esz;             \
+    int n0_ = n_;                                                                                    \
+    if (!FWD && a.stack_rows) {  \
+      n0_ = (int)((unsigned)max(l_y0, 0) / (unsigned)a.stack_rows);                                  \
+      l_y0 -= n0_ * a.stack_rows;                                                                    \
+      l_nav = a.stack_n - n0_;                                                                       \
+    }                                                                                                \
+    l_img = reinterpret_cast<const char*>(a.x) + (size_t)n0_ * a.Hi * a.Wi * a.ldx * esz;            \
   }
 #define WD_OFFS(K0, K1)                                                                              \
   _Pragma("unroll") for (int k_ = (K0); k_ < (K1); ++k_) {                                           \
@@ -154,7 +164,16 @@
       ix_ = max(ix_, -ix_);                                                                          \
       ix_ = max(min(ix_, 2 * a.Wi - 2 - ix_), 0);                                                    \
     } else {                                    \
-      const bool in_ = iy_ >= 0 && iy_ < a.Hi && ix_ >= 0 && ix_ < a.Wi;                             \
+                                            \
+      bool in_;                                                                                      \
+      if (a.stack_rows) {                        \
+        const int d_ = (int)__umulhi((unsigned)(iy_ + s_rows), s_magic) - 1;                         \
+        iy_ -= d_ * s_rows;                                                                          \
+        in_ = d_ >= 0 && d_ < l_nav && iy_ < a.Hi && ix_ >= 0 && ix_ < a.Wi;                         \
+        iy_ += d_ * a.Hi;                                                                            \
+      } else {                                                                                       \
+        in_ = iy_ >= 0 && iy_ < a.Hi && ix_ >= 0 && ix_ < a.Wi;                                      \
+      }                                                                                              \
       u_val = in_ ? u_val | (1u << k_) : u_val & ~(1u << k_);                                        \
       iy_ = in_ ? iy_ : 0;                                                                           \
       ix_ = in_ ? ix_ : 0;                                                                           \
@@ -660,14 +679,30 @@
   return f;
 }
 
-int conv3x3_wide_rows(int mode, int N, int cin_p, int rows, int Ho, int Wo) {
-  return sched::wide_config(mode, N, cin_p, rows, Ho, Wo, wide_force()).rows_pad;
+int conv3x3_wide_rows(int mode, int N, int cin_p, int rows, int Ho, int Wo, int stack) {
+  return sched::wide_config(mode, N, cin_p, rows, Ho, Wo, wide_force(), stack).rows_pad;
+}
+int conv3x3_stack_switch() {
+  const char* e = getenv("MIMO_CONV_STACK");
+  const int v = e ? atoi(e) : 1;
+  return v <= 0 ? 0 : v >= 2 ? 2 : 1;
 }
 size_t conv3x3_wide_weight_elems(int cin_p, int rows_pad) { return (size_t)ceil_div(cin_p, 16) * 9 * rows_pad * 32; }
 int conv3x3_wide_stat_rows() { return 256; }
 
-int conv3x3_wide_launch(const ConvLaunch& a, int mode, int* rows, hipStream_t stream) {
-  const sched::WideCfg c = sched::wide_config(mode, a.N, a.cin_p, a.cout_store, a.Ho, a.Wo, 1);
+int conv3x3_wide_launch(const ConvLaunch& a_, int mode, int* rows, hipStream_t stream) {
+  sched::WideCfg c = sched::wide_config(mode, a_.N, a_.cin_p, a_.cout_store, a_.Ho, a_.Wo, 1, a_.stack);
+  if (c.stacked && ((int64_t)sched::stacked_span(c.TR, a_.Ho) * a_.Hi * a_.Wi * a_.ldx * 4 > (int64_t)INT32_MAX ||
+                    (int64_t)a_.N * a_.Ho * a_.Wo * a_.ldy * 4 >= (int64_t)0x7fff0000))
+    c = sched::wide_config(mode, a_.N, a_.cin_p, a_.cout_store, a_.Ho, a_.Wo, 1, 0);
+  ConvLaunch a = a_;
+  if (c.stacked) {
+    a.stack_rows = a_.Ho;
+    a.stack_n = a_.N;
+    a.stack_magic = sched::stacked_magic(a_.Ho);
+    a.Ho = a_.N * a_.Ho;
+    a.N = 1;
+  }
   if (!a.wpk || c.nf == 0 || c.rows_pad != a.wide || a.ldx % 4 != 0 || a.ldy % 4 != 0 || a.Hi < 2 || a.Wi < 2) {
     set_error("conv3x3 wide: weights packed for %d rows, launch geometry gives %d (nf %d)", a.wide, c.rows_pad, c.nf);
     return MIMO_ERR_INVALID;
@@ -680,7 +715,7 @@
     set_error("conv3x3 wide: output image of %d x %d x %d exceeds the kernel's 32-bit offsets", a.Ho, a.Wo, a.ldy);
     return MIMO_ERR_INVALID;
   }
-  if ((int64_t)a.Hi * a.Wi * a.ldx * 4 > (int64_t)INT32_MAX) {
+  if (!c.stacked && (int64_t)a.Hi * a.Wi * a.ldx * 4 > (int64_t)INT32_MAX) {
     set_error("conv3x3 wide: input image of %d x %d x %d exceeds the kernel's 32-bit offsets", a.Hi, a.Wi, a.ldx);
     return MIMO_ERR_INVALID;
   }
diff --git a/mimo_unet_amd/csrc/ops_api.hip b/mimo_unet_amd/csrc/ops_api.hip
--- a/mimo_unet_amd/csrc/ops_api.hip
+++ b/mimo_unet_amd/csrc/ops_api.hip
@@ -195,7 +195,8 @@
   }
   MIMO_TRY(pack_weights_launch(w, wdp, cout, cin, rows_pad, cout_p, rm, cm, 1, st));
   const int dmode = mixed ? (f16s ? 7 : 5) : (bf16 ? 3 : 0);
-  const int wide = (precision == MIMO_PREC_SPLIT16 || mixed) ? conv3x3_wide_rows(dmode, n, cout_p, cin_p, h + 2, wd + 2) : 0;
+  const int stack = conv3x3_stack_switch();
+  const int wide = (precision == MIMO_PREC_SPLIT16 || mixed) ? conv3x3_wide_rows(dmode, n, cout_p, cin_p, h + 2, wd + 2, stack) : 0;
   const int pair = (split && !wide) ? conv3x3_pair_tail(dmode, cout_p, h + 2, wd + 2) : 0;
   if (wide) {
     wpk = t.get<uint16_t>(conv3x3_wide_weight_elems(cout_p, wide));
@@ -247,8 +248,9 @@
   a.wpk = wpk;
   a.pair = pair;
   a.wide = wide;
+  a.stack = stack;
   if (split) {
-    const size_t kfl = (mixed || wide) ? 0 : conv3x3_ksplit_scratch(dmode, n, cout_p, rows_pad, h + 2, wd + 2, cin_p);
+    const size_t kfl = (mixed || wide) ? 0 : conv3x3_ksplit_scratch(dmode, n, cout_p, rows_pad, h + 2, wd + 2, cin_p, stack);
     float* kpart = kfl ? t.get<float>(kfl) : nullptr;
     MIMO_TRY(conv3x3_bf16x3_launch_k(a, dmode, nullptr, st, kpart, kfl));
   } else
diff --git a/mimo_unet_amd/csrc/plan.hip b/mimo_unet_amd/csrc/plan.hip
--- a/mimo_unet_amd/csrc/plan.hip
+++ b/mimo_unet_amd/csrc/plan.hip
@@ -149,6 +149,7 @@
   size_t cap_act = 0, cap_pad = 0, cap_slab = 0, cap_partial = 0, cap_sums = 0;
   float* s_kpart = nullptr;
   size_t cap_kpart = 0;
+  int conv_stack = 1;
 
   bool wg_async = false;
   int wg_cus = 256;
@@ -406,13 +407,13 @@
                2048 * ceil_div(L.cout_p / 4, 256) <= kDzMaxSlots;
     if (cfg.precision == MIMO_PREC_SPLIT16 || mixed) {
       if (L.fwd_split) L.fwd_wide = conv3x3_wide_rows(fwd_mode(), n, L.cin_p, L.cout_p, h, w);
-      if (L.dg_split) L.dg_wide = conv3x3_wide_rows(dgrad_mode(), n, L.cout_p, L.cin_p, h + 2, w + 2);
+      if (L.dg_split) L.dg_wide = conv3x3_wide_rows(dgrad_mode(), n, L.cout_p, L.cin_p, h + 2, w + 2, conv_stack);
     }
     if (cfg.precision == MIMO_PREC_SPLIT16) {
       if (L.fwd_split && !L.fwd_wide && !cfg.inference_only)
         cap_kpart = std::max(cap_kpart, conv3x3_ksplit_scratch(fwd_mode(), n, L.cin_p, L.cout_pad, h, w, L.cout_p));
       if (L.dg_split && !L.dg_wide && train_bufs)
-        cap_kpart = std::max(cap_kpart, conv3x3_ksplit_scratch(dgrad_mode(), n, L.cout_p, L.dg_rows, h + 2, w + 2, L.cin_p));
+        cap_kpart = std::max(cap_kpart, conv3x3_ksplit_scratch(dgrad_mode(), n, L.cout_p, L.dg_rows, h + 2, w + 2, L.cin_p, conv_stack));
     }
     if (L.fwd_split && (cfg.precision == MIMO_PREC_SPLIT16 || cfg.precision == MIMO_PREC_FP16_MIXED)) {
       if (!wmax_pool) MIMO_TRY(dalloc(&wmax_pool, kMaxWmaxWords));
@@ -552,6 +553,7 @@
     f16 = cfg.precision == MIMO_PREC_FP16_MIXED;
     st = !mixed ? ST_F32 : f16 ? ST_F16 : ST_BF16;
     esz = store_bytes(st);
+    conv_stack = conv3x3_stack_switch();
     {
       const int v = getenv("MIMO_FUSE_BWD_SRC") ? atoi(getenv("MIMO_FUSE_BWD_SRC")) : 1;
       fuse_bwd_src = !mixed && !cfg.inference_only && v != 0;
@@ -1257,6 +1259,7 @@
       a.wpk = L.wd16;
       a.pair = (L.dg_split && !L.dg_wide) ? conv3x3_pair_tail(dgrad_mode(), L.cout_p, L.H + 2, L.W + 2) : 0;
       a.wide = L.dg_wide;
+      a.stack = conv_stack;
       pr = prof_begin(MIMO_PROF_CONV_DGRAD, st);
       if (L.dg_split)
         MIMO_TRY(conv3x3_bf16x3_launch_k(a, dgrad_mode(), nullptr, st, s_kpart, cap_kpart));
diff --git a/mimo_unet_amd/csrc/tile_sched.h b/mimo_unet_amd/csrc/tile_sched.h
--- a/mimo_unet_amd/csrc/tile_sched.h
+++ b/mimo_unet_amd/csrc/tile_sched.h
@@ -44,6 +44,35 @@
   *TC = best_tc;
 }
 
+static inline double tile_eff(int N, int Ho, int Wo, int TR, int TC, int npix, bool stacked) {
+  const double tiles = stacked ? double(cdiv(N * Ho, TR)) : double(N) * cdiv(Ho, TR) * cdiv(Wo, TC);
+  return double(N) * Ho * Wo / (tiles * npix);
+}
+
+static inline bool pick_tile_stacked(int N, int Ho, int Wo, int npix, int maxpix, int* TR, int* TC, bool force = false) {
+  pick_tile_n(Ho, Wo, npix, maxpix, TR, TC);
+  if (N < 1 || Wo > npix || 3 * (Wo + 2) > maxpix || int64_t(N) * Ho > (1 << 24)) return false;
+  int tr = npix / Wo;
+  if (tr > N * Ho) tr = N * Ho;
+  while (tr > 1 && (tr + 2) * (Wo + 2) > maxpix) --tr;
+  if (!force && tile_eff(N, Ho, Wo, tr, Wo, npix, true) <= tile_eff(N, Ho, Wo, *TR, *TC, npix, false) + 1e-9) return false;
+  *TR = tr;
+  *TC = Wo;
+  return true;
+}
+static inline bool use_tile_stacked(int N, int Ho, int Wo, int npix, int maxpix, int cotiles, int stack, int* TR, int* TC) {
+  if (stack <= 0) {
+    pick_tile_n(Ho, Wo, npix, maxpix, TR, TC);
+    return false;
+  }
+  if (!pick_tile_stacked(N, Ho, Wo, npix, maxpix, TR, TC, stack >= 2)) return false;
+  if (stack >= 2 || cdiv(N * Ho, *TR) * cotiles >= 256) return true;
+  pick_tile_n(Ho, Wo, npix, maxpix, TR, TC);
+  return false;
+}
+static inline int stacked_span(int TR, int Ho) { return (TR + 2 + Ho - 2) / Ho + 1; }
+static inline unsigned stacked_magic(int d) { return (unsigned)(((uint64_t)1 << 32) / (unsigned)d) + 1u; }
+
 static inline int conv_pick_nfrag(int cout) {
   const int nfr = cdiv(cout, 16);
   if (nfr <= 1) return 1;
@@ -130,30 +159,39 @@
   int nf;
   int rows_pad;
   int TR, TC;
+  int stacked;
 };
+constexpr int kWsNPix = 256;
+constexpr int kWsMaxPix = 360;
 
 static inline int wide_grid_x(int numTiles, int cotiles);
 
-static inline WideCfg wide_config(int mode, int N, int cin_p, int rows, int Ho, int Wo, int force) {
-  WideCfg c{0, 0, 0, 0};
+static inline WideCfg wide_config(int mode, int N, int cin_p, int rows, int Ho, int Wo, int force, int stack = 0) {
+  WideCfg c{0, 0, 0, 0, 0};
   const bool s16 = mode >= 4 && mode <= 7;
   if (force < 0 || !(mode == 0 || mode == 1 || s16) || rows < 1 || cin_p < 16 || Ho < 2 || Wo < 2) return c;
   if (s16 && cin_p % 8 != 0) return c;
   if (mode == 0 && rows % 8 != 0) return c;
   if (int64_t(Ho + 2) * int64_t(Wo + 2) * int64_t(cin_p < rows ? rows : cin_p) * 8 > int64_t(INT32_MAX)) return c;
-  int TR, TC;
-  pick_tile_n(Ho, Wo, kWideNPix, kWideMaxPix, &TR, &TC);
-  if ((TR + 2) * (TC + 2) > kWideMaxPix) return c;
-  const int tiles = N * cdiv(Ho, TR) * cdiv(Wo, TC);
-  const double eff = double(N) * Ho * Wo / (double(tiles) * kWideNPix);
   const int r32 = cdiv(rows, 32);
   const int nf = (r32 >= 2 && double(rup(r32, 2)) / r32 <= 1.10 + 1e-9) ? 2 : 1;
   const int cotiles = cdiv(r32, nf);
+  int TR, TC;
+  bool stacked = mode == 0 && use_tile_stacked(N, Ho, Wo, kWideNPix, kWideMaxPix, cotiles, stack, &TR, &TC);
+  if (stacked && (int64_t(stacked_span(TR, Ho)) * Ho * Wo * int64_t(cin_p < rows ? rows : cin_p) * 8 > int64_t(INT32_MAX) ||
+                  int64_t(N) * Ho * Wo * int64_t(cin_p < rows ? rows : cin_p) * 8 >= int64_t(0x7fff0000)))
+    stacked = false;
+  if (!stacked) pick_tile_n(Ho, Wo, kWideNPix, kWideMaxPix, &TR, &TC);
+  if ((TR + 2) * (TC + 2) > kWideMaxPix) return c;
+  const int tiles = stacked ? cdiv(N * Ho, TR) : N * cdiv(Ho, TR) * cdiv(Wo, TC);
+  const double eff = double(N) * Ho * Wo / (double(tiles) * kWideNPix);
   if (force == 0) {
     const int k16 = rup(cin_p, s16 ? 32 : 16);
     int TRo, TCo;
-    pick_tile_n(Ho, Wo, 256, 360, &TRo, &TCo);
-    const double eff_o = double(Ho) * Wo / (double(cdiv(Ho, TRo)) * cdiv(Wo, TCo) * 256);
+    const bool stacked_o =
+        use_tile_stacked(N, Ho, Wo, kWsNPix, kWsMaxPix, cdiv(cdiv(rows, 16), 4), mode == 0 ? stack : 0, &TRo, &TCo);
+    const int tiles_o = stacked_o ? cdiv(N * Ho, TRo) : N * cdiv(Ho, TRo) * cdiv(Wo, TCo);
+    const double eff_o = double(N) * Ho * Wo / (double(tiles_o) * kWsNPix);
     const int tail = cin_p - 32 * (cdiv(cin_p, 32) - 1);
     const double k_o = 32.0 * (cdiv(cin_p, 32) - 1) + ((tail <= 16 && !s16) ? 64.0 / 3.0 : 32.0);
     double t_w = double(k16) * (cotiles * nf * 32) / eff * (1.0 + (nf == 2 ? 1.2 : 0.2) / (k16 / (s16 ? 32 : 16)));
@@ -162,7 +200,6 @@
       const int cu_w = wide_grid_x(tiles, cotiles) * cotiles;
       const int nf_o = conv_pick_nfrag(rows);
       const int cot_o = cdiv(cdiv(rows, 16), nf_o);
-      const int tiles_o = N * cdiv(Ho, TRo) * cdiv(Wo, TCo);
       int gx_o = 256 / cot_o > 0 ? 256 / cot_o : 1;
       if (gx_o > tiles_o) gx_o = tiles_o;
       const int cu_o = cdiv(tiles_o, cdiv(tiles_o, gx_o)) * cot_o;
@@ -176,6 +213,7 @@
   c.rows_pad = cotiles * nf * 32;
   c.TR = TR;
   c.TC = TC;
+  c.stacked = stacked ? 1 : 0;
   return c;
 }
 
```

Result: no change. 1355 images/s, median of 6 (+0.7%).
